# olivesgatech/R3D

Hardware: AMD Instinct MI355X
Metric: training clips/sec (RGB+Depth fusion, DARai) at 1/2/4/8 GPUs; effective-rank match (higher is better)
Workload: dtype f32 (depth products: bf16x3 split on the bf16 matrix cores, fp32 accumulate)

## Files before the change

r3d_amd/csrc/decoder_chain.hip:

```cpp
#include "chain_bf3.h"
#include "mha_small.h"
#include "losses_dev.h"

namespace r3d {

constexpr int kDcBufA = 0;
constexpr int kDcBufB = kDcBufA + kFcRows * kFcP1;
constexpr int kDcBufF = kDcBufB + kFcRows * kFcP1;
constexpr int kDcWl = kDcBufF + kFcRows * kFcP4;
constexpr int kDcWlWave = 128 * kFbWP;
constexpr int kDcRed = kDcWl + 8 * kDcWlWave;
constexpr int kDcLdsFloats = kDcRed + 2 * 2 * 8 * kFcRows;
constexpr int kDcLdsBytes = kDcLdsFloats * 4;
static_assert(16 * kFcWP <= kDcWlWave && mha_small_lds_floats(16, 8) <= kDcWlWave && mha_small_bwd_lds_floats(16, 8) <= kDcWlWave,
              "wave region");
static_assert(kDcLdsBytes + (2 * 8 * (kTLHeads + 8) + 8 * 4 * 128 + 64) * 4 <= 160 * 1024, "LDS (dynamic + the tail's static arrays)");

typedef r3d_decoder_chain_args DcArgs;

__device__ __forceinline__ void dc_stage_rows(float* buf, const float* src, int row0, int tid) {
    const int r = tid >> 5, c4 = tid & 31;
    const f32x4 z = {0.f, 0.f, 0.f, 0.f};
    const f32x4 v = *reinterpret_cast<const f32x4*>(src + (size_t)(row0 + (r & 7)) * kFcH + 4 * c4);
    *reinterpret_cast<f32x4*>(buf + r * kFcP1 + 4 * c4) = r < 8 ? v : z;
}

__device__ __forceinline__ void dc_fwd(const DcArgs& D, const int b, float* lds) {
    const int tid = threadIdx.x, lane = tid & 63, wave = tid >> 6;
    const int li = lane & 15, q = lane >> 4;
    float* bufA = lds + kDcBufA;
    float* bufB = lds + kDcBufB;
    float* bufF = lds + kDcBufF;
    float* wl = lds + kDcWl + wave * kDcWlWave;
    float (*red)[8][kFcRows] = reinterpret_cast<float (*)[8][kFcRows]>(lds + kDcRed);
    constexpr int H = kFcH;
    const int row0 = b * 8;
    const int c = wave * 16 + li;
    const bool live = q < 2;
    const f32x4 zero = {0.f, 0.f, 0.f, 0.f};
    R3D_CHAIN_MARK(D.timeline, b == 0, 0);
    FcW s0, s1;
    fc_wload(s0, D.wo + (size_t)(wave * 16) * H, H, 16, lane);
    fc_wload(s1, D.w1 + (size_t)((4 * wave + 0) * 16) * H, H, 16, lane);
    const FcMaskSrc md2(D.drop_d2, D.g2, H), md3(D.drop_d3, D.g2, H), mff(D.drop_ff, D.g2, 4 * H);
    float t1v[4];
    uint8_t kb2[4], kb3[4], kbf[4][4];
#pragma unroll
    for (int i = 0; i < 4; ++i) {
        const size_t r = (size_t)(row0 + ((4 * q + i) & 7));
        t1v[i] = D.t1[r * H + c];
        kb2[i] = md2.raw(r, c);
        kb3[i] = md3.raw(r, c);
#pragma unroll
        for (int t = 0; t < 4; ++t) kbf[t][i] = mff.raw(r, (4 * wave + t) * 16 + li);
    }
    const float b_o = D.bo[c], g2 = D.g2[c], be2 = D.be2[c], b_2 = D.b2[c];
    float b_1[4];
#pragma unroll
    for (int t = 0; t < 4; ++t) b_1[t] = D.b1[(4 * wave + t) * 16 + li];
    R3D_CHAIN_MARK(D.timeline, b == 0, 1);
    {
        MhaArgs m{};
        m.q = D.caq; m.ldq = H; m.k = D.cakv; m.ldk = 2 * H; m.v = D.cakv + H; m.ldv = 2 * H;
        m.key_label = D.key_label; m.pad_idx = D.pad_idx; m.probs = D.p_ca; m.drop = D.drop_ca; m.drop_scale = D.drop_scale;
        m.o = D.ca_o; m.ldo = H; m.B = D.B; m.heads = 8; m.Lq = 8; m.Lk = D.S; m.dh = 16; m.scale = 0.25f;
        mha_fwd_small_unit<16, 8, false>(m, b * 8 + wave, wl);
    }
    R3D_CHAIN_MARK(D.timeline, b == 0, 2);
    __syncthreads();
    dc_stage_rows(bufA, D.ca_o, row0, tid);
    fc_wstore(s0, wl, lane);
    fc_wload(s0, D.w1 + (size_t)((4 * wave + 1) * 16) * H, H, 16, lane);
    __syncthreads();
    const float* wr = wl + li * kFcWP + 4 * q;
    FcOp a;
    f32x4 acc0 = zero, acc1 = zero;
    R3D_CHAIN_MARK(D.timeline, b == 0, 3);
    fc_opload(a, bufA + li * kFcP1 + 4 * q);
    fc_chunk(a, wr, acc0, acc1);
    __builtin_amdgcn_sched_barrier(0);
    fc_wstore(s1, wl, lane);
    fc_wload(s1, D.w1 + (size_t)((4 * wave + 2) * 16) * H, H, 16, lane);
    __builtin_amdgcn_sched_barrier(0);
    float t2p[4], mean[4], rstd[4], t2v[4];
#pragma unroll
    for (int i = 0; i < 4; ++i) {
        t2p[i] = ((acc0[i] + acc1[i]) + b_o) * md2.keep(kb2[i], D.drop_scale) + t1v[i];
        if (live) D.t2_pre[(size_t)(row0 + 4 * q + i) * H + c] = t2p[i];
    }
    fc_layernorm(t2p, red, wave, li, q, mean, rstd);
#pragma unroll
    for (int i = 0; i < 4; ++i) {
        t2v[i] = (t2p[i] - mean[i]) * rstd[i] * g2 + be2;
        const int r = 4 * q + i;
        if (live) {
            D.t2[(size_t)(row0 + r) * H + c] = t2v[i];
            if (wave == 0 && li == 0) { D.m2[row0 + r] = mean[i]; D.r2[row0 + r] = rstd[i]; }
        }
        bufB[r * kFcP1 + c] = live ? t2v[i] : 0.f;
    }
    __syncthreads();
    R3D_CHAIN_MARK(D.timeline, b == 0, 4);
    fc_opload(a, bufB + li * kFcP1 + 4 * q);
#pragma unroll
    for (int t = 0; t < 4; ++t) {
        acc0 = zero; acc1 = zero;
        fc_chunk(a, wr, acc0, acc1);
        __builtin_amdgcn_sched_barrier(0);
        if (t == 0) { fc_wstore(s0, wl, lane); fc_wload(s0, D.w1 + (size_t)((4 * wave + 3) * 16) * H, H, 16, lane); }
        if (t == 1) { fc_wstore(s1, wl, lane); fc_wload(s1, D.w2 + (size_t)(wave * 16) * (4 * H) + 0, 4 * H, 16, lane); }
        if (t == 2) { fc_wstore(s0, wl, lane); fc_wload(s0, D.w2 + (size_t)(wave * 16) * (4 * H) + 128, 4 * H, 16, lane); }
        if (t == 3) { fc_wstore(s1, wl, lane); fc_wload(s1, D.w2 + (size_t)(wave * 16) * (4 * H) + 256, 4 * H, 16, lane); }
        __builtin_amdgcn_sched_barrier(0);
        const int cu = (4 * wave + t) * 16 + li;
#pragma unroll
        for (int i = 0; i < 4; ++i) {
            const float f = fmaxf((acc0[i] + acc1[i]) + b_1[t], 0.f) * mff.keep(kbf[t][i], D.drop_scale);
            if (live) D.ff1[(size_t)(row0 + 4 * q + i) * (4 * H) + cu] = f;
            bufF[(4 * q + i) * kFcP4 + cu] = live ? f : 0.f;
        }
    }
    __syncthreads();
    R3D_CHAIN_MARK(D.timeline, b == 0, 5);
    acc0 = zero; acc1 = zero;
    const float* ar = bufF + li * kFcP4 + 4 * q;
    fc_opload(a, ar);
    fc_chunk(a, wr, acc0, acc1);
    __builtin_amdgcn_sched_barrier(0);
    fc_wstore(s0, wl, lane);
    fc_wload(s0, D.w2 + (size_t)(wave * 16) * (4 * H) + 384, 4 * H, 16, lane);
    __builtin_amdgcn_sched_barrier(0);
    fc_opload(a, ar + 128);
    fc_chunk(a, wr, acc0, acc1);
    __builtin_amdgcn_sched_barrier(0);
    fc_wstore(s1, wl, lane);
    __builtin_amdgcn_sched_barrier(0);
    fc_opload(a, ar + 256);
    fc_chunk(a, wr, acc0, acc1);
    __builtin_amdgcn_sched_barrier(0);
    fc_wstore(s0, wl, lane);
    __builtin_amdgcn_sched_barrier(0);
    fc_opload(a, ar + 384);
    fc_chunk(a, wr, acc0, acc1);
    if (live) {
#pragma unroll
        for (int i = 0; i < 4; ++i)
            D.t3_pre[(size_t)(row0 + 4 * q + i) * H + c] = ((acc0[i] + acc1[i]) + b_2) * md3.keep(kb3[i], D.drop_scale) + t2v[i];
    }
}

__device__ __forceinline__ void dc_bwd(const DcArgs& D, const int b, float* lds) {
    const int tid = threadIdx.x, lane = tid & 63, wave = tid >> 6;
    const int li = lane & 15, q = lane >> 4;
    float* bufA = lds + kDcBufA;
    float* bufF = lds + kDcBufF;
    float* wl = lds + kDcWl + wave * kDcWlWave;
    float* redA = lds + kDcRed;
    constexpr int H = kFcH;
    const int row0 = b * 8;
    const int c = wave * 16 + li, n0 = wave * 16;
    const bool live = q < 2;
    const f32x4 zero = {0.f, 0.f, 0.f, 0.f};
    R3D_CHAIN_MARK(D.timeline, b == 0, 10);
    FcW s0, s1;
    fb_wload(s0, D.w2 + (4 * wave + 0) * 16, 4 * H, 128, lane);
    fb_wload(s1, D.w2 + (4 * wave + 1) * 16, 4 * H, 128, lane);
    dc_stage_rows(bufA, D.d_ff2, row0, tid);
    const FcMaskSrc md2(D.drop_d2, D.g2, H), mff(D.drop_ff, D.g2, 4 * H);
    float ffv[4][4], res[4], t2pv[4], m2v[4], r2v[4];
    uint8_t kb2[4], kbf[4][4];
#pragma unroll
    for (int i = 0; i < 4; ++i) {
        const size_t r = (size_t)(row0 + ((4 * q + i) & 7));
#pragma unroll
        for (int t = 0; t < 4; ++t) {
            ffv[t][i] = D.ff1[r * (4 * H) + (4 * wave + t) * 16 + li];
            kbf[t][i] = mff.raw(r, (4 * wave + t) * 16 + li);
        }
        res[i] = D.d_t3pre[r * H + c];
        t2pv[i] = D.t2_pre[r * H + c];
        m2v[i] = D.m2[r]; r2v[i] = D.r2[r];
        kb2[i] = md2.raw(r, c);
    }
    const float g2 = D.g2[c];
    __builtin_amdgcn_sched_barrier(0);
    fb_wstore(s0, wl, lane);
    fb_wload(s0, D.w2 + (4 * wave + 2) * 16, 4 * H, 128, lane);
    __syncthreads();
    FcOp a;
    f32x4 acc0, acc1;
    R3D_CHAIN_MARK(D.timeline, b == 0, 11);
    fc_opload(a, bufA + li * kFcP1 + 4 * q);
#pragma unroll
    for (int t = 0; t < 4; ++t) {
        acc0 = zero; acc1 = zero;
        fb_chunk(a, wl, li, q, acc0, acc1);
        __builtin_amdgcn_sched_barrier(0);
        if (t == 0) { fb_wstore(s1, wl, lane); fb_wload(s1, D.w2 + (4 * wave + 3) * 16, 4 * H, 128, lane); }
        if (t == 1) { fb_wstore(s0, wl, lane); fb_wload(s0, D.w1 + n0, H, 128, lane); }
        if (t == 2) { fb_wstore(s1, wl, lane); fb_wload(s1, D.w1 + (size_t)128 * H + n0, H, 128, lane); }
        if (t == 3) { fb_wstore(s0, wl, lane); fb_wload(s0, D.w1 + (size_t)256 * H + n0, H, 128, lane); }
        __builtin_amdgcn_sched_barrier(0);
        const int cu = (4 * wave + t) * 16 + li;
#pragma unroll
        for (int i = 0; i < 4; ++i) {
            const float gv = ffv[t][i] > 0.f ? (acc0[i] + acc1[i]) * mff.keep(kbf[t][i], D.drop_scale) : 0.f;
            if (live) D.d_ff1[(size_t)(row0 + 4 * q + i) * (4 * H) + cu] = gv;
            bufF[(4 * q + i) * kFcP4 + cu] = live ? gv : 0.f;
        }
    }
    __syncthreads();
    R3D_CHAIN_MARK(D.timeline, b == 0, 12);
    acc0 = zero; acc1 = zero;
    const float* ar = bufF + li * kFcP4 + 4 * q;
    fc_opload(a, ar);
    fb_chunk(a, wl, li, q, acc0, acc1);
    __builtin_amdgcn_sched_barrier(0);
    fb_wstore(s1, wl, lane);
    fb_wload(s1, D.w1 + (size_t)384 * H + n0, H, 128, lane);
    __builtin_amdgcn_sched_barrier(0);
    fc_opload(a, ar + 128);
    fb_chunk(a, wl, li, q, acc0, acc1);
    __builtin_amdgcn_sched_barrier(0);
    fb_wstore(s0, wl, lane);
    fb_wload(s0, D.wo + n0, H, 128, lane);
    __builtin_amdgcn_sched_barrier(0);
    fc_opload(a, ar + 256);
    fb_chunk(a, wl, li, q, acc0, acc1);
    __builtin_amdgcn_sched_barrier(0);
    fb_wstore(s1, wl, lane);
    __builtin_amdgcn_sched_barrier(0);
    fc_opload(a, ar + 384);
    fb_chunk(a, wl, li, q, acc0, acc1);
    __builtin_amdgcn_sched_barrier(0);
    fb_wstore(s0, wl, lane);
    __builtin_amdgcn_sched_barrier(0);
    {
        float d[4], xh[4], g[4], gx[4], s1v[4], s2v[4];
#pragma unroll
        for (int i = 0; i < 4; ++i) {
            d[i] = live ? (acc0[i] + acc1[i]) + res[i] : 0.f;
            xh[i] = (t2pv[i] - m2v[i]) * r2v[i];
            g[i] = d[i] * g2;
            gx[i] = g[i] * xh[i];
        }
        if (live) {
            float* pp = D.part_d2 + (size_t)(2 * b + q) * (2 * H);
            pp[c] = (d[0] * xh[0] + d[1] * xh[1]) + (d[2] * xh[2] + d[3] * xh[3]);
            pp[H + c] = (d[0] + d[1]) + (d[2] + d[3]);
        }
        fb_rowsum2<4>(g, gx, redA, wave, li, q, s1v, s2v);
#pragma unroll
        for (int i = 0; i < 4; ++i) {
            const float o = r2v[i] * (g[i] - s1v[i] - xh[i] * s2v[i]);
            const size_t e = (size_t)(row0 + 4 * q + i) * H + c;
            const float ok = o * md2.keep(kb2[i], D.drop_scale);
            if (live) { D.d_t2pre[e] = o; D.d_cap[e] = ok; }
            bufA[(4 * q + i) * kFcP1 + c] = live ? ok : 0.f;
        }
    }
    __syncthreads();
    R3D_CHAIN_MARK(D.timeline, b == 0, 13);
    fc_opload(a, bufA + li * kFcP1 + 4 * q);
    acc0 = zero; acc1 = zero;
    fb_chunk(a, wl, li, q, acc0, acc1);
    if (live) {
#pragma unroll
        for (int i = 0; i < 4; ++i) D.d_cao[(size_t)(row0 + 4 * q + i) * H + c] = acc0[i] + acc1[i];
    }
    R3D_CHAIN_MARK(D.timeline, b == 0, 14);
    __syncthreads();
    {
        MhaArgs m{};
        m.q = D.caq; m.ldq = H; m.k = D.cakv; m.ldk = 2 * H; m.v = D.cakv + H; m.ldv = 2 * H;
        m.probs = D.p_ca; m.drop = D.drop_ca; m.drop_scale = D.drop_scale; m.d_o = D.d_cao; m.lddo = H;
        m.dq = D.d_caq; m.lddq = H; m.dk = D.d_cakv; m.lddk = 2 * H; m.dv = D.d_cakv + H; m.lddv = 2 * H;
        m.B = D.B; m.heads = 8; m.Lq = 8; m.Lk = D.S; m.dh = 16; m.scale = 0.25f;
        mha_bwd_small_unit<16, 8, false>(m, b * 8 + wave, wl);
    }
    R3D_CHAIN_MARK(D.timeline, b == 0, 15);
}

constexpr int kD3P1 = kFcH + 8, kD3P4 = 4 * kFcH + 8;
constexpr int kD3ImgA = 0;
constexpr int kD3ImgB = kD3ImgA + 3 * 16 * kD3P1;
constexpr int kD3ImgF = kD3ImgB + 3 * 16 * kD3P1;
constexpr int kD3ScrBytes = (kD3ImgF + 3 * 16 * kD3P4) * 2;
constexpr int kD3ScrWave = 1856;
constexpr int kD3RedBytes = kD3ScrBytes + 8 * kD3ScrWave * 4;
constexpr int kD3LdsBytes = kD3RedBytes + 2 * 2 * 8 * kFcRows * 4;
static_assert(mha_small_lds_floats(16, 8) <= kD3ScrWave && mha_small_bwd_lds_floats(16, 8) <= kD3ScrWave, "attention scratch");
static_assert(kD3LdsBytes + (2 * 8 * (kTLHeads + 8) + 8 * 4 * 128 + 64) * 4 <= 160 * 1024, "LDS (dynamic + the tail's static arrays)");

__device__ __forceinline__ void dc3_stage_rows(unsigned short* img, const float* src, int row0, int tid) {
    const int r = tid >> 5, c4 = tid & 31;
    const f32x4 z = {0.f, 0.f, 0.f, 0.f};
    const f32x4 v = *reinterpret_cast<const f32x4*>(src + (size_t)(row0 + (r & 7)) * kFcH + 4 * c4);
    bf3_store4(img, kD3P1, r, 4 * c4, r < 8 ? v : z);
}

__device__ __forceinline__ void dc3_fwd(const DcArgs& D, const int b, float* lds) {
    const int tid = threadIdx.x, lane = tid & 63, wave = tid >> 6;
    const int li = lane & 15, q = lane >> 4;
    unsigned short* img = reinterpret_cast<unsigned short*>(lds);
    unsigned short* imgA = img + kD3ImgA;
    unsigned short* imgB = img + kD3ImgB;
    unsigned short* imgF = img + kD3ImgF;
    float* scr = reinterpret_cast<float*>(reinterpret_cast<unsigned char*>(lds) + kD3ScrBytes) + wave * kD3ScrWave;
    float (*red)[8][kFcRows] = reinterpret_cast<float (*)[8][kFcRows]>(reinterpret_cast<unsigned char*>(lds) + kD3RedBytes);
    constexpr int H = kFcH;
    const int row0 = b * 8;
    const int c = wave * 16 + li;
    const bool live = q < 2;
    const f32x4 zero = {0.f, 0.f, 0.f, 0.f};
    R3D_CHAIN_MARK(D.timeline, b == 0, 0);
    Bf3B b0, b1, b2;
    bf3_bload<4>(b0, D.pl_wo, 4, wave, 0, lane);
    bf3_bload<4>(b1, D.pl_w1, 4, 4 * wave + 0, 0, lane);
    bf3_bload<4>(b2, D.pl_w1, 4, 4 * wave + 1, 0, lane);
    const FcMaskSrc md2(D.drop_d2, D.g2, H), md3(D.drop_d3, D.g2, H), mff(D.drop_ff, D.g2, 4 * H);
    float t1v[4];
    uint8_t kb2[4], kb3[4], kbf[4][4];
#pragma unroll
    for (int i = 0; i < 4; ++i) {
        const size_t r = (size_t)(row0 + ((4 * q + i) & 7));
        t1v[i] = D.t1[r * H + c];
        kb2[i] = md2.raw(r, c);
        kb3[i] = md3.raw(r, c);
#pragma unroll
        for (int t = 0; t < 4; ++t) kbf[t][i] = mff.raw(r, (4 * wave + t) * 16 + li);
    }
    const float b_o = D.bo[c], g2 = D.g2[c], be2 = D.be2[c], b_2 = D.b2[c];
    float b_1[4];
#pragma unroll
    for (int t = 0; t < 4; ++t) b_1[t] = D.b1[(4 * wave + t) * 16 + li];
    R3D_CHAIN_MARK(D.timeline, b == 0, 1);
    {
        MhaArgs m{};
        m.q = D.caq; m.ldq = H; m.k = D.cakv; m.ldk = 2 * H; m.v = D.cakv + H; m.ldv = 2 * H;
        m.key_label = D.key_label; m.pad_idx = D.pad_idx; m.probs = D.p_ca; m.drop = D.drop_ca; m.drop_scale = D.drop_scale;
        m.o = D.ca_o; m.ldo = H; m.B = D.B; m.heads = 8; m.Lq = 8; m.Lk = D.S; m.dh = 16; m.scale = 0.25f;
        mha_fwd_small_unit<16, 8, false>(m, b * 8 + wave, scr);
    }
    R3D_CHAIN_MARK(D.timeline, b == 0, 2);
    __syncthreads();
    dc3_stage_rows(imgA, D.ca_o, row0, tid);
    __syncthreads();
    R3D_CHAIN_MARK(D.timeline, b == 0, 3);
    f32x4 acc0 = zero, acc1 = zero;
    bf3_chunk<4>(imgA, kD3P1, li, q, 0, b0, acc0, acc1);
    __builtin_amdgcn_sched_barrier(0);
    bf3_bload<4>(b0, D.pl_w1, 4, 4 * wave + 2, 0, lane);
    __builtin_amdgcn_sched_barrier(0);
    float t2p[4], mean[4], rstd[4], t2v[4];
#pragma unroll
    for (int i = 0; i < 4; ++i) {
        t2p[i] = ((acc0[i] + acc1[i]) + b_o) * md2.keep(kb2[i], D.drop_scale) + t1v[i];
        if (live) D.t2_pre[(size_t)(row0 + 4 * q + i) * H + c] = t2p[i];
    }
    fc_layernorm(t2p, red, wave, li, q, mean, rstd);
#pragma unroll
    for (int i = 0; i < 4; ++i) {
        t2v[i] = (t2p[i] - mean[i]) * rstd[i] * g2 + be2;
        const int r = 4 * q + i;
        if (live) {
            D.t2[(size_t)(row0 + r) * H + c] = t2v[i];
            if (wave == 0 && li == 0) { D.m2[row0 + r] = mean[i]; D.r2[row0 + r] = rstd[i]; }
        }
        bf3_store1(imgB, kD3P1, r, c, live ? t2v[i] : 0.f);
    }
    __syncthreads();
    R3D_CHAIN_MARK(D.timeline, b == 0, 4);
#pragma unroll
    for (int t = 0; t < 4; ++t) {
        acc0 = zero; acc1 = zero;
        if (t == 0) bf3_chunk<4>(imgB, kD3P1, li, q, 0, b1, acc0, acc1);
        if (t == 1) bf3_chunk<4>(imgB, kD3P1, li, q, 0, b2, acc0, acc1);
        if (t == 2) bf3_chunk<4>(imgB, kD3P1, li, q, 0, b0, acc0, acc1);
        if (t == 3) bf3_chunk<4>(imgB, kD3P1, li, q, 0, b1, acc0, acc1);
        __builtin_amdgcn_sched_barrier(0);
        if (t == 0) bf3_bload<4>(b1, D.pl_w1, 4, 4 * wave + 3, 0, lane);
        if (t == 1) bf3_bload<4>(b2, D.pl_w2, 16, wave, 0, lane);
        if (t == 2) bf3_bload<4>(b0, D.pl_w2, 16, wave, 4, lane);
        if (t == 3) bf3_bload<4>(b1, D.pl_w2, 16, wave, 8, lane);
        __builtin_amdgcn_sched_barrier(0);
        const int cu = (4 * wave + t) * 16 + li;
#pragma unroll
        for (int i = 0; i < 4; ++i) {
            const float f = fmaxf((acc0[i] + acc1[i]) + b_1[t], 0.f) * mff.keep(kbf[t][i], D.drop_scale);
            if (live) D.ff1[(size_t)(row0 + 4 * q + i) * (4 * H) + cu] = f;
            bf3_store1(imgF, kD3P4, 4 * q + i, cu, live ? f : 0.f);
        }
    }
    __syncthreads();
    R3D_CHAIN_MARK(D.timeline, b == 0, 5);
    acc0 = zero; acc1 = zero;
    bf3_chunk<4>(imgF, kD3P4, li, q, 0, b2, acc0, acc1);
    __builtin_amdgcn_sched_barrier(0);
    bf3_bload<4>(b2, D.pl_w2, 16, wave, 12, lane);
    __builtin_amdgcn_sched_barrier(0);
    bf3_chunk<4>(imgF, kD3P4, li, q, 4, b0, acc0, acc1);
    bf3_chunk<4>(imgF, kD3P4, li, q, 8, b1, acc0, acc1);
    bf3_chunk<4>(imgF, kD3P4, li, q, 12, b2, acc0, acc1);
    if (live) {
#pragma unroll
        for (int i = 0; i < 4; ++i)
            D.t3_pre[(size_t)(row0 + 4 * q + i) * H + c] =
                ((acc0[i] + acc1[i]) + b_2) * md3.keep(kb3[i], D.drop_scale) + t2v[i];
    }
}

__device__ __forceinline__ void dc3_bwd(const DcArgs& D, const int b, float* lds) {
    const int tid = threadIdx.x, lane = tid & 63, wave = tid >> 6;
    const int li = lane & 15, q = lane >> 4;
    unsigned short* img = reinterpret_cast<unsigned short*>(lds);
    unsigned short* imgA = img + kD3ImgA;
    unsigned short* imgF = img + kD3ImgF;
    float* scr = reinterpret_cast<float*>(reinterpret_cast<unsigned char*>(lds) + kD3ScrBytes) + wave * kD3ScrWave;
    float* redA = reinterpret_cast<float*>(reinterpret_cast<unsigned char*>(lds) + kD3RedBytes);
    constexpr int H = kFcH;
    const int row0 = b * 8;
    const int c = wave * 16 + li;
    const bool live = q < 2;
    const f32x4 zero = {0.f, 0.f, 0.f, 0.f};
    R3D_CHAIN_MARK(D.timeline, b == 0, 10);
    Bf3B b0, b1, b2;
    bf3_bload<4>(b0, D.pl_w2_t, 4, 4 * wave + 0, 0, lane);
    bf3_bload<4>(b1, D.pl_w2_t, 4, 4 * wave + 1, 0, lane);
    bf3_bload<4>(b2, D.pl_w2_t, 4, 4 * wave + 2, 0, lane);
    dc3_stage_rows(imgA, D.d_ff2, row0, tid);
    const FcMaskSrc md2(D.drop_d2, D.g2, H), mff(D.drop_ff, D.g2, 4 * H);
    float ffv[4][4], res[4], t2pv[4], m2v[4], r2v[4];
    uint8_t kb2[4], kbf[4][4];
#pragma unroll
    for (int i = 0; i < 4; ++i) {
        const size_t r = (size_t)(row0 + ((4 * q + i) & 7));
#pragma unroll
        for (int t = 0; t < 4; ++t) {
            ffv[t][i] = D.ff1[r * (4 * H) + (4 * wave + t) * 16 + li];
            kbf[t][i] = mff.raw(r, (4 * wave + t) * 16 + li);
        }
        res[i] = D.d_t3pre[r * H + c];
        t2pv[i] = D.t2_pre[r * H + c];
        m2v[i] = D.m2[r]; r2v[i] = D.r2[r];
        kb2[i] = md2.raw(r, c);
    }
    const float g2 = D.g2[c];
    __syncthreads();
    R3D_CHAIN_MARK(D.timeline, b == 0, 11);
    f32x4 acc0, acc1;
#pragma unroll
    for (int t = 0; t < 4; ++t) {
        acc0 = zero; acc1 = zero;
        if (t == 0) bf3_chunk<4>(imgA, kD3P1, li, q, 0, b0, acc0, acc1);
        if (t == 1) bf3_chunk<4>(imgA, kD3P1, li, q, 0, b1, acc0, acc1);
        if (t == 2) bf3_chunk<4>(imgA, kD3P1, li, q, 0, b2, acc0, acc1);
        if (t == 3) bf3_chunk<4>(imgA, kD3P1, li, q, 0, b0, acc0, acc1);
        __builtin_amdgcn_sched_barrier(0);
        if (t == 0) bf3_bload<4>(b0, D.pl_w2_t, 4, 4 * wave + 3, 0, lane);
        if (t == 1) bf3_bload<4>(b1, D.pl_w1_t, 16, wave, 0, lane);
        if (t == 2) bf3_bload<4>(b2, D.pl_w1_t, 16, wave, 4, lane);
        if (t == 3) bf3_bload<4>(b0, D.pl_w1_t, 16, wave, 8, lane);
        __builtin_amdgcn_sched_barrier(0);
        const int cu = (4 * wave + t) * 16 + li;
#pragma unroll
        for (int i = 0; i < 4; ++i) {
            const float gv = ffv[t][i] > 0.f ? (acc0[i] + acc1[i]) * mff.keep(kbf[t][i], D.drop_scale) : 0.f;
            if (live) D.d_ff1[(size_t)(row0 + 4 * q + i) * (4 * H) + cu] = gv;
            bf3_store1(imgF, kD3P4, 4 * q + i, cu, live ? gv : 0.f);
        }
    }
    __syncthreads();
    R3D_CHAIN_MARK(D.timeline, b == 0, 12);
    acc0 = zero; acc1 = zero;
    bf3_chunk<4>(imgF, kD3P4, li, q, 0, b1, acc0, acc1);
    __builtin_amdgcn_sched_barrier(0);
    bf3_bload<4>(b1, D.pl_w1_t, 16, wave, 12, lane);
    __builtin_amdgcn_sched_barrier(0);
    bf3_chunk<4>(imgF, kD3P4, li, q, 4, b2, acc0, acc1);
    __builtin_amdgcn_sched_barrier(0);
    bf3_bload<4>(b2, D.pl_wo_t, 4, wave, 0, lane);
    __builtin_amdgcn_sched_barrier(0);
    bf3_chunk<4>(imgF, kD3P4, li, q, 8, b0, acc0, acc1);
    bf3_chunk<4>(imgF, kD3P4, li, q, 12, b1, acc0, acc1);
    {
        float d[4], xh[4], g[4], gx[4], s1v[4], s2v[4];
#pragma unroll
        for (int i = 0; i < 4; ++i) {
            d[i] = live ? (acc0[i] + acc1[i]) + res[i] : 0.f;
            xh[i] = (t2pv[i] - m2v[i]) * r2v[i];
            g[i] = d[i] * g2;
            gx[i] = g[i] * xh[i];
        }
        if (live) {
            float* pp = D.part_d2 + (size_t)(2 * b + q) * (2 * H);
            pp[c] = (d[0] * xh[0] + d[1] * xh[1]) + (d[2] * xh[2] + d[3] * xh[3]);
            pp[H + c] = (d[0] + d[1]) + (d[2] + d[3]);
        }
        fb_rowsum2<4>(g, gx, redA, wave, li, q, s1v, s2v);
#pragma unroll
        for (int i = 0; i < 4; ++i) {
            const float o = r2v[i] * (g[i] - s1v[i] - xh[i] * s2v[i]);
            const size_t e = (size_t)(row0 + 4 * q + i) * H + c;
            const float ok = o * md2.keep(kb2[i], D.drop_scale);
            if (live) { D.d_t2pre[e] = o; D.d_cap[e] = ok; }
            bf3_store1(imgA, kD3P1, 4 * q + i, c, live ? ok : 0.f);
        }
    }
    __syncthreads();
    R3D_CHAIN_MARK(D.timeline, b == 0, 13);
    acc0 = zero; acc1 = zero;
    bf3_chunk<4>(imgA, kD3P1, li, q, 0, b2, acc0, acc1);
    if (live) {
#pragma unroll
        for (int i = 0; i < 4; ++i) D.d_cao[(size_t)(row0 + 4 * q + i) * H + c] = acc0[i] + acc1[i];
    }
    R3D_CHAIN_MARK(D.timeline, b == 0, 14);
    __syncthreads();
    {
        MhaArgs m{};
        m.q = D.caq; m.ldq = H; m.k = D.cakv; m.ldk = 2 * H; m.v = D.cakv + H; m.ldv = 2 * H;
        m.probs = D.p_ca; m.drop = D.drop_ca; m.drop_scale = D.drop_scale; m.d_o = D.d_cao; m.lddo = H;
        m.dq = D.d_caq; m.lddq = H; m.dk = D.d_cakv; m.lddk = 2 * H; m.dv = D.d_cakv + H; m.lddv = 2 * H;
        m.B = D.B; m.heads = 8; m.Lq = 8; m.Lk = D.S; m.dh = 16; m.scale = 0.25f;
        mha_bwd_small_unit<16, 8, false>(m, b * 8 + wave, scr);
    }
    R3D_CHAIN_MARK(D.timeline, b == 0, 15);
}

__global__ __launch_bounds__(512) void decoder_chain_bf3_kernel(const DcArgs D, const r3d_tail_losses_args t, const LossArgs a,
                                                                float* part, unsigned* arrivals) {
    extern __shared__ __attribute__((aligned(16))) float lds[];
    __shared__ float lg[8][kTLHeads + 8];
    __shared__ float dl[8][kTLHeads + 8];
    __shared__ float red[8][4][128];
    __shared__ int is_last;
    if (threadIdx.x >= 256) __builtin_amdgcn_s_setprio(0); else __builtin_amdgcn_s_setprio(2);
    const int lane = threadIdx.x & 63, wave = threadIdx.x >> 6;
    if ((int)blockIdx.x < D.B) {
        const int b = (int)blockIdx.x;
        if (D.phases & 1) dc3_fwd(D, b, lds);
        R3D_CHAIN_MARK(D.timeline, b == 0, 6);
        if (D.phases & 2) {
            __syncthreads();
            tail_clip_body(t, a, part, b, lg, dl, red);
        }
        R3D_CHAIN_MARK(D.timeline, b == 0, 7);
        if (D.phases & 4) {
            __syncthreads();
            dc3_bwd(D, b, lds);
        }
    } else if (D.phases & 2) {
        const int u = ((int)blockIdx.x - D.B) * 8 + wave;
        if (u < a.B * a.S) losses_unit(a, part, u, lane);
    }
    if (D.phases & 2) tail_losses_finish(t, a, part, arrivals, &is_last);
}

__global__ __launch_bounds__(512) void decoder_chain_kernel(const DcArgs D, const r3d_tail_losses_args t, const LossArgs a,
                                                            float* part, unsigned* arrivals) {
    extern __shared__ __attribute__((aligned(16))) float lds[];
    if (threadIdx.x >= 256) __builtin_amdgcn_s_setprio(0); else __builtin_amdgcn_s_setprio(2);
    __shared__ float lg[8][kTLHeads + 8];
    __shared__ float dl[8][kTLHeads + 8];
    __shared__ float red[8][4][128];
    __shared__ int is_last;
    const int lane = threadIdx.x & 63, wave = threadIdx.x >> 6;
    if ((int)blockIdx.x < D.B) {
        const int b = (int)blockIdx.x;
        if (D.phases & 1) dc_fwd(D, b, lds);
        R3D_CHAIN_MARK(D.timeline, b == 0, 6);
        if (D.phases & 2) {
            __syncthreads();
            tail_clip_body(t, a, part, b, lg, dl, red);
        }
        R3D_CHAIN_MARK(D.timeline, b == 0, 7);
        if (D.phases & 4) {
            __syncthreads();
            dc_bwd(D, b, lds);
        }
    } else if (D.phases & 2) {
        const int u = ((int)blockIdx.x - D.B) * 8 + wave;
        if (u < a.B * a.S) losses_unit(a, part, u, lane);
    }
    if (D.phases & 2) tail_losses_finish(t, a, part, arrivals, &is_last);
}

}

using namespace r3d;

R3D_EXPORT int r3d_decoder_tail_losses_supported(int H, int n_head, int Q, int rows);

R3D_EXPORT int r3d_decoder_chain_supported(int H, int Q, int heads, int S) {
    return (H == kFcH && Q == 8 && heads == 8 && S > 0 && S <= 64) ? 1 : 0;
}

R3D_EXPORT int r3d_decoder_chain(const r3d_decoder_chain_args* d, const r3d_tail_losses_args* tail, float* ws, void* stream) {
    R3D_REQUIRE(d && (d->phases & 7) && !(d->phases & ~7));
    R3D_REQUIRE(r3d_decoder_chain_supported(d->H, d->Q, d->heads, d->S) && d->B > 0);
    R3D_REQUIRE(d->caq && d->cakv && d->p_ca && d->wo && d->w1 && d->w2 && d->t2_pre && d->m2 && d->r2 && d->g2 && d->ff1);
    if (d->phases & 1)
        R3D_REQUIRE(d->ca_o && d->bo && d->t1 && d->be2 && d->t2 && d->b1 && d->b2 && d->t3_pre);
    if (d->phases & 4)
        R3D_REQUIRE(d->d_t3pre && d->d_ff2 && d->d_ff1 && d->d_t2pre && d->d_cap && d->d_cao && d->d_caq && d->d_cakv && d->part_d2);
    const void* al[] = {d->caq, d->cakv, d->wo, d->w1, d->w2, d->ca_o, d->d_ff2, d->d_cao, d->d_cakv};
    for (const void* p : al)
        if (p && !r3d_aligned16(p)) return R3D_EALIGN;
    r3d_tail_losses_args t{};
    LossArgs a{};
    int grid = d->B;
    unsigned* arrivals = nullptr;
    if (d->phases & 2) {
        R3D_REQUIRE(tail && ws);
        t = *tail;
        R3D_REQUIRE(t.x && t.g3 && t.b3 && t.gF && t.bF && t.w_head && t.b_head && t.t3 && t.m3 && t.r3 && t.tgtF && t.mF && t.rF);
        R3D_REQUIRE(t.out && t.seg && t.past_label && t.target && t.target_dur && t.d_seg && t.d_out && t.loss_out && t.counts);
        R3D_REQUIRE(t.dx && t.dx2 && t.wsF && t.ws3);
        R3D_REQUIRE(t.B == d->B && t.S == d->S && t.Q == d->Q && t.H == d->H && t.K > 0 && t.n_head == t.K + 1);
        R3D_REQUIRE(t.ld_out >= t.n_head && t.ld_dout >= t.n_head && t.ld_seg >= t.K && t.ld_dseg >= t.K);
        if (!r3d_decoder_tail_losses_supported(t.H, t.n_head, t.Q, t.B * t.Q)) return R3D_EINVAL;
        if (!r3d_aligned16(ws)) return R3D_EALIGN;
        if (d->phases & 1) R3D_REQUIRE(t.x == d->t3_pre);
        if (d->phases & 4) R3D_REQUIRE(t.dx == d->d_t3pre && t.dx2 == d->d_ff2);
        a = LossArgs{t.seg, t.ld_seg, t.out, t.ld_out, t.out + t.K, t.ld_out, t.past_label, t.target, t.target_dur, t.B, t.S, t.Q,
                     t.K, t.pad_idx, t.exclude_idx, 0, t.dur_den, t.grad_scale, t.d_seg, t.ld_dseg, t.d_out, t.ld_dout,
                     t.d_out + t.K, t.ld_dout, t.loss_out, t.counts, t.tick_a, t.tick_b};
        const int units = t.B * t.S + t.B * t.Q + t.B;
        grid = t.B + r3d_cdiv(t.B * t.S, 8);
        arrivals = reinterpret_cast<unsigned*>(ws + 4 * (size_t)units);
    }
    if (d->pl_wo) {
        R3D_REQUIRE(d->pl_w1 && d->pl_w2 && d->pl_w2_t && d->pl_w1_t && d->pl_wo_t);
        hipError_t e3 = hipFuncSetAttribute((const void*)decoder_chain_bf3_kernel, hipFuncAttributeMaxDynamicSharedMemorySize,
                                            kD3LdsBytes);
        if (e3 != hipSuccess) return (int)e3;
        hipLaunchKernelGGL(decoder_chain_bf3_kernel, dim3(grid), dim3(512), (size_t)kD3LdsBytes, (hipStream_t)stream, *d, t, a, ws,
                           arrivals);
        R3D_LAUNCH_CHECK();
        return R3D_OK;
    }
    hipError_t e = hipFuncSetAttribute((const void*)decoder_chain_kernel, hipFuncAttributeMaxDynamicSharedMemorySize, kDcLdsBytes);
    if (e != hipSuccess) return (int)e;
    hipLaunchKernelGGL(decoder_chain_kernel, dim3(grid), dim3(512), (size_t)kDcLdsBytes, (hipStream_t)stream, *d, t, a, ws, arrivals);
    R3D_LAUNCH_CHECK();
    return R3D_OK;
}
```

r3d_amd/csrc/fuser_chain.hip:

```cpp
#include "chain_bf3.h"
#include "mha_small.h"
#include "../../include/r3d_hip.h"

namespace r3d {

constexpr int kFcBufH = 0;
constexpr int kFcBufV = kFcBufH + kFcRows * kFcP1;
constexpr int kFcBufF = kFcBufV + kFcRows * kFcP1;
constexpr int kFcWl = kFcBufF + kFcRows * kFcP4;
constexpr int kFcRed = kFcWl + 8 * 16 * kFcWP;
constexpr int kFcLdsFloats = kFcRed + 2 * 8 * kFcRows;
constexpr int kFcLdsBytes = kFcLdsFloats * 4;
static_assert(mha_small_lds_floats(16, 8) <= 16 * kFcWP, "the query role's attention units borrow the wave's weight region");
static_assert(mha_small_bwd_lds_floats(16, 8) <= 16 * kFcWP, "the query role's attention units borrow the wave's weight region");

typedef r3d_fuser_chain_fwd_args FcFwd;

__device__ __forceinline__ void fc_fwd_fuser(const FcFwd& A, const int wg, float* lds) {
    const int tid = threadIdx.x, lane = tid & 63, wave = tid >> 6;
    const int li = lane & 15, q = lane >> 4;
    float* bufH = lds + kFcBufH;
    float* bufV = lds + kFcBufV;
    float* bufF = lds + kFcBufF;
    float* wl = lds + kFcWl + wave * (16 * kFcWP);
    float (*red)[8][kFcRows] = reinterpret_cast<float (*)[8][kFcRows]>(lds + kFcRed);
    const int row0 = wg * kFcRows;
    const int c = wave * 16 + li;
    constexpr int H = kFcH;
    const int nseg_t = (A.K + 15) >> 4;
    R3D_CHAIN_MARK(A.timeline, wg == 0, 0);
    const int nt5 = 16 + nseg_t;

    FcW s0, s1;
    fc_wload(s0, A.wv + (size_t)(wave * 16) * H, H, 16, lane);
    fc_wload(s1, A.wproj + (size_t)(wave * 16) * H, H, 16, lane);
    const f32x4 a_in = *reinterpret_cast<const f32x4*>(A.h1 + (size_t)(row0 + (tid >> 5)) * H + 4 * (tid & 31));
    float x0[4];
#pragma unroll
    for (int i = 0; i < 4; ++i) x0[i] = A.x0[(size_t)(row0 + 4 * q + i) * H + c];
    const float b_proj = A.bproj[c], g2 = A.g2[c], be2 = A.be2[c], b_2 = A.b2[c], gF = A.gf[c], beF = A.bef[c];
    float b_1[4];
#pragma unroll
    for (int t = 0; t < 4; ++t) b_1[t] = A.b1[(4 * wave + t) * 16 + li];
    const int f0 = (row0 >> 1) + 2 * q;
    const float pos0 = A.pos[(size_t)(f0 % A.S) * H + c], pos1 = A.pos[(size_t)((f0 + 1) % A.S) * H + c];
    __builtin_amdgcn_sched_barrier(0);
    *reinterpret_cast<f32x4*>(bufH + (tid >> 5) * kFcP1 + 4 * (tid & 31)) = a_in;
    fc_wstore(s0, wl, lane);
    fc_wload(s0, A.w1 + (size_t)((4 * wave + 0) * 16) * H, H, 16, lane);
    __syncthreads();

    R3D_CHAIN_MARK(A.timeline, wg == 0, 1);
    const float* wr = wl + li * kFcWP + 4 * q;
    FcOp a;
    f32x4 acc0, acc1;
    const f32x4 zero = {0.f, 0.f, 0.f, 0.f};
    fc_opload(a, bufH + li * kFcP1 + 4 * q);
    acc0 = zero; acc1 = zero;
    fc_chunk(a, wr, acc0, acc1);
    __builtin_amdgcn_sched_barrier(0);
    fc_wstore(s1, wl, lane);
    fc_wload(s1, A.w1 + (size_t)((4 * wave + 1) * 16) * H, H, 16, lane);
    __builtin_amdgcn_sched_barrier(0);
#pragma unroll
    for (int i = 0; i < 4; ++i) {
        const float v = acc0[i] + acc1[i];
        const int rs = 4 * q + (i ^ 1);
        A.vsw[(size_t)(row0 + rs) * H + c] = v;
        bufV[rs * kFcP1 + c] = v;
    }
    __syncthreads();
    R3D_CHAIN_MARK(A.timeline, wg == 0, 2);
    fc_opload(a, bufV + li * kFcP1 + 4 * q);
    acc0 = zero; acc1 = zero;
    fc_chunk(a, wr, acc0, acc1);
    __builtin_amdgcn_sched_barrier(0);
    fc_wstore(s0, wl, lane);
    fc_wload(s0, A.w1 + (size_t)((4 * wave + 2) * 16) * H, H, 16, lane);
    __builtin_amdgcn_sched_barrier(0);
    float x1[4], mean[4], rstd[4];
#pragma unroll
    for (int i = 0; i < 4; ++i) {
        x1[i] = (acc0[i] + acc1[i]) + b_proj + x0[i];
        A.x1[(size_t)(row0 + 4 * q + i) * H + c] = x1[i];
    }
    fc_layernorm(x1, red, wave, li, q, mean, rstd);
#pragma unroll
    for (int i = 0; i < 4; ++i) {
        const float h = (x1[i] - mean[i]) * rstd[i] * g2 + be2;
        const int r = 4 * q + i;
        A.h2[(size_t)(row0 + r) * H + c] = h;
        bufH[r * kFcP1 + c] = h;
        if (wave == 0 && li == 0) { A.m2[row0 + r] = mean[i]; A.r2[row0 + r] = rstd[i]; }
    }
    __syncthreads();
    R3D_CHAIN_MARK(A.timeline, wg == 0, 3);
    fc_opload(a, bufH + li * kFcP1 + 4 * q);
#pragma unroll
    for (int t = 0; t < 4; ++t) {
        acc0 = zero; acc1 = zero;
        if (t < 2) R3D_CHAIN_MARK(A.timeline, wg == 0, 8 + 4 * t);
        fc_chunk(a, wr, acc0, acc1);
        __builtin_amdgcn_sched_barrier(0);
        if (t < 2) R3D_CHAIN_MARK(A.timeline, wg == 0, 9 + 4 * t);
#if defined(R3D_FC_PROBE) && (R3D_FC_PROBE & 8)
        if (t == 0) { fc_wstore(s1, wl, lane); }
        if (t == 1) { fc_wstore(s0, wl, lane); }
        if (t == 2) { fc_wstore(s1, wl, lane); }
        if (t == 3) { fc_wstore(s0, wl, lane); }
#elif defined(R3D_FC_PROBE) && (R3D_FC_PROBE & 16)
        if (t == 0) { fc_wload(s1, A.w1 + (size_t)((4 * wave + 3) * 16) * H, H, 16, lane); }
        if (t == 1) { fc_wload(s0, A.w2 + (size_t)(wave * 16) * (4 * H) + 0, 4 * H, 16, lane); }
        if (t == 2) { fc_wload(s1, A.w2 + (size_t)(wave * 16) * (4 * H) + 128, 4 * H, 16, lane); }
        if (t == 3) { fc_wload(s0, A.w2 + (size_t)(wave * 16) * (4 * H) + 256, 4 * H, 16, lane); }
#else
        if (t == 0) { fc_wstore(s1, wl, lane); fc_wload(s1, A.w1 + (size_t)((4 * wave + 3) * 16) * H, H, 16, lane); }
        if (t == 1) { fc_wstore(s0, wl, lane); fc_wload(s0, A.w2 + (size_t)(wave * 16) * (4 * H) + 0, 4 * H, 16, lane); }
        if (t == 2) { fc_wstore(s1, wl, lane); fc_wload(s1, A.w2 + (size_t)(wave * 16) * (4 * H) + 128, 4 * H, 16, lane); }
        if (t == 3) { fc_wstore(s0, wl, lane); fc_wload(s0, A.w2 + (size_t)(wave * 16) * (4 * H) + 256, 4 * H, 16, lane); }
#endif
        __builtin_amdgcn_sched_barrier(0);
        if (t < 2) R3D_CHAIN_MARK(A.timeline, wg == 0, 10 + 4 * t);
        const int cu = (4 * wave + t) * 16 + li;
#pragma unroll
        for (int i = 0; i < 4; ++i) {
            const float u = (acc0[i] + acc1[i]) + b_1[t];
#if defined(R3D_FC_PROBE) && (R3D_FC_PROBE & 4)
            const float f = u;
#else
            const float f = gelu_f(u);
#endif
            const size_t o = (size_t)(row0 + 4 * q + i) * (4 * H) + cu;
#if !(defined(R3D_FC_PROBE) && (R3D_FC_PROBE & 1))
            A.u[o] = u;
            A.f1[o] = f;
#endif
#if !(defined(R3D_FC_PROBE) && (R3D_FC_PROBE & 2))
            bufF[(4 * q + i) * kFcP4 + cu] = f;
#else
            if (u == 123.456f) bufF[(4 * q + i) * kFcP4 + cu] = f;
#endif
        }
        if (t < 2) R3D_CHAIN_MARK(A.timeline, wg == 0, 11 + 4 * t);
    }
    __syncthreads();
    R3D_CHAIN_MARK(A.timeline, wg == 0, 4);
    acc0 = zero; acc1 = zero;
    {
        const float* ar = bufF + li * kFcP4 + 4 * q;
        fc_opload(a, ar);
        fc_chunk(a, wr, acc0, acc1);
        __builtin_amdgcn_sched_barrier(0);
        fc_wstore(s1, wl, lane);
        fc_wload(s1, A.w2 + (size_t)(wave * 16) * (4 * H) + 384, 4 * H, 16, lane);
        __builtin_amdgcn_sched_barrier(0);
        fc_opload(a, ar + 128);
        fc_chunk(a, wr, acc0, acc1);
        __builtin_amdgcn_sched_barrier(0);
        fc_wstore(s0, wl, lane);
        {
            const int t5 = wave;
            fc_wload(s0, A.wkv + (size_t)(t5 * 16) * H, H, 16, lane);
        }
        __builtin_amdgcn_sched_barrier(0);
        fc_opload(a, ar + 256);
        fc_chunk(a, wr, acc0, acc1);
        __builtin_amdgcn_sched_barrier(0);
        fc_wstore(s1, wl, lane);
        {
            const int t5 = wave + 8;
            fc_wload(s1, A.wkv + (size_t)(t5 * 16) * H, H, 16, lane);
        }
        __builtin_amdgcn_sched_barrier(0);
        fc_opload(a, ar + 384);
        fc_chunk(a, wr, acc0, acc1);
        __builtin_amdgcn_sched_barrier(0);
    }
    fc_wstore(s0, wl, lane);
    const int t5c = wave + 16;
    const bool has12 = t5c < nt5;
    {
        const int ts = has12 ? t5c - 16 : 0;
        const int nv = A.K - 16 * ts;
        fc_wload(s0, A.wseg + (size_t)(ts * 16) * H, H, nv < 16 ? nv : 16, lane);
    }
    const float bkv0 = A.bkv[wave * 16 + li], bkv1 = A.bkv[(wave + 8) * 16 + li];
    const int cseg = (has12 ? t5c - 16 : 0) * 16 + li;
    const float bsg = A.bseg[cseg < A.K ? cseg : A.K - 1];
    __builtin_amdgcn_sched_barrier(0);
    R3D_CHAIN_MARK(A.timeline, wg == 0, 5);
    float x3[4];
#pragma unroll
    for (int i = 0; i < 4; ++i) {
        x3[i] = (acc0[i] + acc1[i]) + b_2 + x1[i] + (A.add_xres ? x0[i] : 0.f);
        A.x3[(size_t)(row0 + 4 * q + i) * H + c] = x3[i];
    }
    fc_layernorm(x3, red, wave, li, q, mean, rstd);
    float y[4];
#pragma unroll
    for (int i = 0; i < 4; ++i) {
        y[i] = (x3[i] - mean[i]) * rstd[i] * gF + beF;
        if (A.y) A.y[(size_t)(row0 + 4 * q + i) * H + c] = y[i];
        if (wave == 0 && li == 0) { A.mf[row0 + 4 * q + i] = mean[i]; A.rf[row0 + 4 * q + i] = rstd[i]; }
    }
    {
        const float fu0 = (y[0] + y[1]) * 0.5f, fu1 = (y[2] + y[3]) * 0.5f;
        A.fused[(size_t)f0 * H + c] = fu0;
        A.fused[(size_t)(f0 + 1) * H + c] = fu1;
        bufV[(2 * q) * kFcP1 + c] = fu0;
        bufV[(2 * q + 1) * kFcP1 + c] = fu1;
        bufV[(8 + 2 * q) * kFcP1 + c] = fu0 + pos0;
        bufV[(8 + 2 * q + 1) * kFcP1 + c] = fu1 + pos1;
    }
    __syncthreads();
    R3D_CHAIN_MARK(A.timeline, wg == 0, 6);
    fc_opload(a, bufV + li * kFcP1 + 4 * q);
    const int fr = (row0 >> 1) + ((4 * q) & 7);
    acc0 = zero; acc1 = zero;
    fc_chunk(a, wr, acc0, acc1);
    __builtin_amdgcn_sched_barrier(0);
    fc_wstore(s1, wl, lane);
    __builtin_amdgcn_sched_barrier(0);
    if (q >= 2) {
#pragma unroll
        for (int i = 0; i < 4; ++i) A.cakv[(size_t)(fr + i) * (2 * H) + wave * 16 + li] = (acc0[i] + acc1[i]) + bkv0;
    }
    acc0 = zero; acc1 = zero;
    fc_chunk(a, wr, acc0, acc1);
    __builtin_amdgcn_sched_barrier(0);
    fc_wstore(s0, wl, lane);
    __builtin_amdgcn_sched_barrier(0);
    if (q >= 2) {
#pragma unroll
        for (int i = 0; i < 4; ++i) A.cakv[(size_t)(fr + i) * (2 * H) + (wave + 8) * 16 + li] = (acc0[i] + acc1[i]) + bkv1;
    }
    if (has12) {
        acc0 = zero; acc1 = zero;
        fc_chunk(a, wr, acc0, acc1);
        if (q < 2 && cseg < A.K) {
#pragma unroll
            for (int i = 0; i < 4; ++i) A.seg[(size_t)(fr + i) * A.K + cseg] = (acc0[i] + acc1[i]) + bsg;
        }
    }
    R3D_CHAIN_MARK(A.timeline, wg == 0, 7);
}

__device__ __forceinline__ void fc_fwd_query(const FcFwd& A, const int wgq, float* lds) {
    const int tid = threadIdx.x, lane = tid & 63, wave = tid >> 6;
    const int li = lane & 15, q = lane >> 4;
    float* bufH = lds + kFcBufH;
    float* bufV = lds + kFcBufV;
    float* wl = lds + kFcWl + wave * (16 * kFcWP);
    float (*red)[8][kFcRows] = reinterpret_cast<float (*)[8][kFcRows]>(lds + kFcRed);
    constexpr int H = kFcH;
    const int row0 = wgq * kFcRows;
    const int c = wave * 16 + li;
    R3D_CHAIN_MARK(A.timeline, wgq == 0, 16);
    FcW s0, s1;
    fc_wload(s0, A.w_in + (size_t)(wave * 16) * H, H, 16, lane);
    fc_wload(s1, A.w_in + (size_t)((wave + 8) * 16) * H, H, 16, lane);
    const f32x4 a_in = *reinterpret_cast<const f32x4*>(A.qpos + (size_t)((tid >> 5) & 7) * H + 4 * (tid & 31));
    float b_in[3];
#pragma unroll
    for (int t = 0; t < 3; ++t) b_in[t] = A.b_in[(wave + 8 * t) * 16 + li];
    const float b_out = A.b_out[c], g1 = A.g1[c], be1 = A.be1[c], b_q = A.bq[c];
    const FcMaskSrc md1(A.drop_d1, A.g1, H);
    uint8_t kb[4];
    float qp[4];
#pragma unroll
    for (int i = 0; i < 4; ++i) {
        const int r = row0 + 4 * q + i;
        kb[i] = md1.raw(r, c);
        qp[i] = A.qpos[(size_t)((4 * q + i) & 7) * H + c];
    }
    __builtin_amdgcn_sched_barrier(0);
    *reinterpret_cast<f32x4*>(bufH + (tid >> 5) * kFcP1 + 4 * (tid & 31)) = a_in;
    fc_wstore(s0, wl, lane);
    fc_wload(s0, A.w_in + (size_t)((wave + 16) * 16) * H, H, 16, lane);
    __syncthreads();
    const float* wr = wl + li * kFcWP + 4 * q;
    FcOp a;
    f32x4 acc0, acc1;
    const f32x4 zero = {0.f, 0.f, 0.f, 0.f};
    fc_opload(a, bufH + li * kFcP1 + 4 * q);
#pragma unroll
    for (int t = 0; t < 3; ++t) {
        acc0 = zero; acc1 = zero;
        fc_chunk(a, wr, acc0, acc1);
        __builtin_amdgcn_sched_barrier(0);
        if (t == 0) { fc_wstore(s1, wl, lane); fc_wload(s1, A.w_out + (size_t)(wave * 16) * H, H, 16, lane); }
        if (t == 1) { fc_wstore(s0, wl, lane); fc_wload(s0, A.wq + (size_t)(wave * 16) * H, H, 16, lane); }
        __builtin_amdgcn_sched_barrier(0);
#pragma unroll
        for (int i = 0; i < 4; ++i)
            A.sa_qkv[(size_t)(row0 + 4 * q + i) * (3 * H) + (wave + 8 * t) * 16 + li] = (acc0[i] + acc1[i]) + b_in[t];
    }
    R3D_CHAIN_MARK(A.timeline, wgq == 0, 17);
    __syncthreads();
    {
        MhaArgs m{};
        m.q = A.sa_qkv; m.ldq = 3 * H; m.k = A.sa_qkv + H; m.ldk = 3 * H; m.v = A.sa_qkv + 2 * H; m.ldv = 3 * H;
        m.probs = A.p_sa; m.drop = A.drop_sa; m.drop_scale = A.drop_scale; m.o = A.sa_o; m.ldo = H;
        m.B = A.B; m.heads = 8; m.Lq = 8; m.Lk = 8; m.dh = 16; m.scale = 0.25f;
        mha_fwd_small_unit<16, 8, false>(m, (2 * wgq) * 8 + wave, wl);
        __builtin_amdgcn_wave_barrier();
        mha_fwd_small_unit<16, 8, false>(m, (2 * wgq + 1) * 8 + wave, wl);
    }
    __syncthreads();
    {
        const f32x4 so = *reinterpret_cast<const f32x4*>(A.sa_o + (size_t)(row0 + (tid >> 5)) * H + 4 * (tid & 31));
        *reinterpret_cast<f32x4*>(bufV + (tid >> 5) * kFcP1 + 4 * (tid & 31)) = so;
    }
    R3D_CHAIN_MARK(A.timeline, wgq == 0, 18);
    fc_wstore(s1, wl, lane);
    __syncthreads();
    R3D_CHAIN_MARK(A.timeline, wgq == 0, 19);
    fc_opload(a, bufV + li * kFcP1 + 4 * q);
    acc0 = zero; acc1 = zero;
    fc_chunk(a, wr, acc0, acc1);
    __builtin_amdgcn_sched_barrier(0);
    fc_wstore(s0, wl, lane);
    __builtin_amdgcn_sched_barrier(0);
    float t1p[4], mean[4], rstd[4];
#pragma unroll
    for (int i = 0; i < 4; ++i) {
        t1p[i] = ((acc0[i] + acc1[i]) + b_out) * md1.keep(kb[i], A.drop_scale);
        A.t1_pre[(size_t)(row0 + 4 * q + i) * H + c] = t1p[i];
    }
    fc_layernorm(t1p, red, wave, li, q, mean, rstd);
#pragma unroll
    for (int i = 0; i < 4; ++i) {
        const int r = 4 * q + i;
        const float t1 = (t1p[i] - mean[i]) * rstd[i] * g1 + be1;
        A.t1[(size_t)(row0 + r) * H + c] = t1;
        bufH[r * kFcP1 + c] = t1 + qp[i];
        if (wave == 0 && li == 0) { A.m1[row0 + r] = mean[i]; A.r1[row0 + r] = rstd[i]; }
    }
    __syncthreads();
    R3D_CHAIN_MARK(A.timeline, wgq == 0, 20);
    fc_opload(a, bufH + li * kFcP1 + 4 * q);
    acc0 = zero; acc1 = zero;
    fc_chunk(a, wr, acc0, acc1);
#pragma unroll
    for (int i = 0; i < 4; ++i) A.caq[(size_t)(row0 + 4 * q + i) * H + c] = (acc0[i] + acc1[i]) + b_q;
    R3D_CHAIN_MARK(A.timeline, wgq == 0, 21);
}

constexpr int kF3P1 = kFcH + 8;
constexpr int kF3P4 = 4 * kFcH + 8;
constexpr int kF3ImgH = 0;
constexpr int kF3ImgV = kF3ImgH + 3 * 16 * kF3P1;
constexpr int kF3ImgF = kF3ImgV + 3 * 16 * kF3P1;
constexpr int kF3RedBytes = (kF3ImgF + 3 * 16 * kF3P4) * 2;
constexpr int kF3LdsBytes = kF3RedBytes + 2 * 2 * 8 * kFcRows * 4;

__device__ __forceinline__ void fc3_fwd_fuser(const FcFwd& A, const int wg, float* lds) {
    const int tid = threadIdx.x, lane = tid & 63, wave = tid >> 6;
    const int li = lane & 15, q = lane >> 4;
    unsigned short* img = reinterpret_cast<unsigned short*>(lds);
    unsigned short* imgH = img + kF3ImgH;
    unsigned short* imgV = img + kF3ImgV;
    unsigned short* imgF = img + kF3ImgF;
    float (*red)[8][kFcRows] = reinterpret_cast<float (*)[8][kFcRows]>(reinterpret_cast<unsigned char*>(lds) + kF3RedBytes);
    const int row0 = wg * kFcRows;
    const int c = wave * 16 + li;
    constexpr int H = kFcH;
    const int nseg_t = (A.K + 15) >> 4;
    const bool has12 = wave < nseg_t;
    R3D_CHAIN_MARK(A.timeline, wg == 0, 0);
    Bf3B b0, b1, b2;
    bf3_bload<4>(b0, A.pl_wv, 4, wave, 0, lane);
    bf3_bload<4>(b1, A.pl_wproj, 4, wave, 0, lane);
    bf3_bload<4>(b2, A.pl_w1, 4, 4 * wave + 0, 0, lane);
    const f32x4 a_in = *reinterpret_cast<const f32x4*>(A.h1 + (size_t)(row0 + (tid >> 5)) * H + 4 * (tid & 31));
    float x0[4];
#pragma unroll
    for (int i = 0; i < 4; ++i) x0[i] = A.x0[(size_t)(row0 + 4 * q + i) * H + c];
    const float b_proj = A.bproj[c], g2 = A.g2[c], be2 = A.be2[c], b_2 = A.b2[c], gF = A.gf[c], beF = A.bef[c];
    float b_1[4];
#pragma unroll
    for (int t = 0; t < 4; ++t) b_1[t] = A.b1[(4 * wave + t) * 16 + li];
    const int f0 = (row0 >> 1) + 2 * q;
    const float pos0 = A.pos[(size_t)(f0 % A.S) * H + c], pos1 = A.pos[(size_t)((f0 + 1) % A.S) * H + c];
    const float bkv0 = A.bkv[wave * 16 + li], bkv1 = A.bkv[(wave + 8) * 16 + li];
    const int cseg = (has12 ? wave : 0) * 16 + li;
    const float bsg = A.bseg[cseg < A.K ? cseg : A.K - 1];
    __builtin_amdgcn_sched_barrier(0);
    bf3_stage_tile(imgH, kF3P1, 0, a_in, tid);
    __syncthreads();
    R3D_CHAIN_MARK(A.timeline, wg == 0, 1);
    const f32x4 zero = {0.f, 0.f, 0.f, 0.f};
    f32x4 acc0 = zero, acc1 = zero;
    bf3_chunk<4>(imgH, kF3P1, li, q, 0, b0, acc0, acc1);
    __builtin_amdgcn_sched_barrier(0);
    bf3_bload<4>(b0, A.pl_w1, 4, 4 * wave + 1, 0, lane);
    __builtin_amdgcn_sched_barrier(0);
#pragma unroll
    for (int i = 0; i < 4; ++i) {
        const float v = acc0[i] + acc1[i];
        const int rs = 4 * q + (i ^ 1);
        A.vsw[(size_t)(row0 + rs) * H + c] = v;
        bf3_store1(imgV, kF3P1, rs, c, v);
    }
    __syncthreads();
    R3D_CHAIN_MARK(A.timeline, wg == 0, 2);
    acc0 = zero; acc1 = zero;
    bf3_chunk<4>(imgV, kF3P1, li, q, 0, b1, acc0, acc1);
    __builtin_amdgcn_sched_barrier(0);
    bf3_bload<4>(b1, A.pl_w1, 4, 4 * wave + 2, 0, lane);
    __builtin_amdgcn_sched_barrier(0);
    float x1[4], mean[4], rstd[4];
#pragma unroll
    for (int i = 0; i < 4; ++i) {
        x1[i] = (acc0[i] + acc1[i]) + b_proj + x0[i];
        A.x1[(size_t)(row0 + 4 * q + i) * H + c] = x1[i];
    }
    fc_layernorm(x1, red, wave, li, q, mean, rstd);
#pragma unroll
    for (int i = 0; i < 4; ++i) {
        const float h = (x1[i] - mean[i]) * rstd[i] * g2 + be2;
        const int r = 4 * q + i;
        A.h2[(size_t)(row0 + r) * H + c] = h;
        bf3_store1(imgH, kF3P1, r, c, h);
        if (wave == 0 && li == 0) { A.m2[row0 + r] = mean[i]; A.r2[row0 + r] = rstd[i]; }
    }
    __syncthreads();
    R3D_CHAIN_MARK(A.timeline, wg == 0, 3);
#pragma unroll
    for (int t = 0; t < 4; ++t) {
        acc0 = zero; acc1 = zero;
        if (t == 0) bf3_chunk<4>(imgH, kF3P1, li, q, 0, b2, acc0, acc1);
        if (t == 1) bf3_chunk<4>(imgH, kF3P1, li, q, 0, b0, acc0, acc1);
        if (t == 2) bf3_chunk<4>(imgH, kF3P1, li, q, 0, b1, acc0, acc1);
        if (t == 3) bf3_chunk<4>(imgH, kF3P1, li, q, 0, b2, acc0, acc1);
        __builtin_amdgcn_sched_barrier(0);
        if (t == 0) bf3_bload<4>(b2, A.pl_w1, 4, 4 * wave + 3, 0, lane);
        if (t == 1) bf3_bload<4>(b0, A.pl_w2, 16, wave, 0, lane);
        if (t == 2) bf3_bload<4>(b1, A.pl_w2, 16, wave, 4, lane);
        if (t == 3) bf3_bload<4>(b2, A.pl_w2, 16, wave, 8, lane);
        __builtin_amdgcn_sched_barrier(0);
        const int cu = (4 * wave + t) * 16 + li;
#pragma unroll
        for (int i = 0; i < 4; ++i) {
            const float u = (acc0[i] + acc1[i]) + b_1[t];
            const float f = gelu_f(u);
            const size_t o = (size_t)(row0 + 4 * q + i) * (4 * H) + cu;
            A.u[o] = u;
            A.f1[o] = f;
            bf3_store1(imgF, kF3P4, 4 * q + i, cu, f);
        }
    }
    __syncthreads();
    R3D_CHAIN_MARK(A.timeline, wg == 0, 4);
    acc0 = zero; acc1 = zero;
    bf3_chunk<4>(imgF, kF3P4, li, q, 0, b0, acc0, acc1);
    __builtin_amdgcn_sched_barrier(0);
    bf3_bload<4>(b0, A.pl_w2, 16, wave, 12, lane);
    __builtin_amdgcn_sched_barrier(0);
    bf3_chunk<4>(imgF, kF3P4, li, q, 4, b1, acc0, acc1);
    __builtin_amdgcn_sched_barrier(0);
    bf3_bload<4>(b1, A.pl_wkv, 4, wave, 0, lane);
    __builtin_amdgcn_sched_barrier(0);
    bf3_chunk<4>(imgF, kF3P4, li, q, 8, b2, acc0, acc1);
    __builtin_amdgcn_sched_barrier(0);
    bf3_bload<4>(b2, A.pl_wkv, 4, wave + 8, 0, lane);
    __builtin_amdgcn_sched_barrier(0);
    bf3_chunk<4>(imgF, kF3P4, li, q, 12, b0, acc0, acc1);
    __builtin_amdgcn_sched_barrier(0);
    bf3_bload<4>(b0, A.pl_wseg, 4, has12 ? wave : 0, 0, lane);
    __builtin_amdgcn_sched_barrier(0);
    R3D_CHAIN_MARK(A.timeline, wg == 0, 5);
    float x3[4];
#pragma unroll
    for (int i = 0; i < 4; ++i) {
        x3[i] = (acc0[i] + acc1[i]) + b_2 + x1[i] + (A.add_xres ? x0[i] : 0.f);
        A.x3[(size_t)(row0 + 4 * q + i) * H + c] = x3[i];
    }
    fc_layernorm(x3, red, wave, li, q, mean, rstd);
    float y[4];
#pragma unroll
    for (int i = 0; i < 4; ++i) {
        y[i] = (x3[i] - mean[i]) * rstd[i] * gF + beF;
        if (A.y) A.y[(size_t)(row0 + 4 * q + i) * H + c] = y[i];
        if (wave == 0 && li == 0) { A.mf[row0 + 4 * q + i] = mean[i]; A.rf[row0 + 4 * q + i] = rstd[i]; }
    }
    {
        const float fu0 = (y[0] + y[1]) * 0.5f, fu1 = (y[2] + y[3]) * 0.5f;
        A.fused[(size_t)f0 * H + c] = fu0;
        A.fused[(size_t)(f0 + 1) * H + c] = fu1;
        bf3_store1(imgV, kF3P1, 2 * q, c, fu0);
        bf3_store1(imgV, kF3P1, 2 * q + 1, c, fu1);
        bf3_store1(imgV, kF3P1, 8 + 2 * q, c, fu0 + pos0);
        bf3_store1(imgV, kF3P1, 8 + 2 * q + 1, c, fu1 + pos1);
    }
    __syncthreads();
    R3D_CHAIN_MARK(A.timeline, wg == 0, 6);
    const int fr = (row0 >> 1) + ((4 * q) & 7);
    acc0 = zero; acc1 = zero;
    bf3_chunk<4>(imgV, kF3P1, li, q, 0, b1, acc0, acc1);
    if (q >= 2) {
#pragma unroll
        for (int i = 0; i < 4; ++i) A.cakv[(size_t)(fr + i) * (2 * H) + wave * 16 + li] = (acc0[i] + acc1[i]) + bkv0;
    }
    acc0 = zero; acc1 = zero;
    bf3_chunk<4>(imgV, kF3P1, li, q, 0, b2, acc0, acc1);
    if (q >= 2) {
#pragma unroll
        for (int i = 0; i < 4; ++i) A.cakv[(size_t)(fr + i) * (2 * H) + (wave + 8) * 16 + li] = (acc0[i] + acc1[i]) + bkv1;
    }
    if (has12) {
        acc0 = zero; acc1 = zero;
        bf3_chunk<4>(imgV, kF3P1, li, q, 0, b0, acc0, acc1);
        if (q < 2 && cseg < A.K) {
#pragma unroll
            for (int i = 0; i < 4; ++i) A.seg[(size_t)(fr + i) * A.K + cseg] = (acc0[i] + acc1[i]) + bsg;
        }
    }
    R3D_CHAIN_MARK(A.timeline, wg == 0, 7);
}

__global__ __launch_bounds__(512) void fuser_chain_fwd_bf3_kernel(const FcFwd A) {
    extern __shared__ __attribute__((aligned(16))) float lds[];
    if (threadIdx.x >= 256) __builtin_amdgcn_s_setprio(0); else __builtin_amdgcn_s_setprio(2);
    const int nf = (2 * A.N) / kFcRows;
    if ((int)blockIdx.x < nf) fc3_fwd_fuser(A, (int)blockIdx.x, lds);
    else fc_fwd_query(A, (int)blockIdx.x - nf, lds);
}

__global__ __launch_bounds__(256) void weight_planes_kernel(const r3d_plane_job* __restrict__ jobs, int njobs, int total) {
    weight_planes_block(jobs, njobs, total, (int)blockIdx.x * 4 + (threadIdx.x >> 6), threadIdx.x & 63);
}

__global__ __launch_bounds__(512) void fuser_chain_fwd_kernel(const FcFwd A) {
    extern __shared__ __attribute__((aligned(16))) float lds[];
    if (threadIdx.x >= 256) __builtin_amdgcn_s_setprio(0); else __builtin_amdgcn_s_setprio(2);
    const int nf = (2 * A.N) / kFcRows;
    if ((int)blockIdx.x < nf) fc_fwd_fuser(A, (int)blockIdx.x, lds);
    else fc_fwd_query(A, (int)blockIdx.x - nf, lds);
}


constexpr int kFbWl = kFcBufF + kFcRows * kFcP4;
constexpr int kFbRed = kFbWl + 8 * 128 * kFbWP;
constexpr int kFbLdsFloats = kFbRed + 2 * 2 * 8 * kFcRows;
constexpr int kFbLdsBytes = kFbLdsFloats * 4;
static_assert(mha_small_bwd_lds_floats(16, 8) <= 128 * kFbWP, "attention units borrow the wave's weight region");
static_assert(kFbLdsBytes <= 160 * 1024, "LDS");

typedef r3d_fuser_chain_bwd_args FcBwd;

__device__ __forceinline__ void fc_bwd_fuser(const FcBwd& A, const int wg, float* lds) {
    const int tid = threadIdx.x, lane = tid & 63, wave = tid >> 6;
    const int li = lane & 15, q = lane >> 4;
    float* bufH = lds + kFcBufH;
    float* bufV = lds + kFcBufV;
    float* bufF = lds + kFcBufF;
    float* wl = lds + kFbWl + wave * (128 * kFbWP);
    float* redA = lds + kFbRed;
    float* redB = redA + 2 * 8 * kFcRows;
    constexpr int H = kFcH;
    const int row0 = wg * kFcRows;
    const int c = wave * 16 + li;
    const int n0 = wave * 16;
    const int f0 = (row0 >> 1) + 2 * q;
    const f32x4 zero = {0.f, 0.f, 0.f, 0.f};

    R3D_CHAIN_MARK(A.timeline, wg == 0, 0);
    FcW s0, s1;
    fb_wload(s0, A.wkv + n0, H, 128, lane);
    fb_wload(s1, A.wkv + (size_t)128 * H + n0, H, 128, lane);
    {
        const int r = tid >> 5, c4 = tid & 31, fr = (row0 >> 1) + (r >> 1);
        const f32x4 v0 = *reinterpret_cast<const f32x4*>(A.d_cakv + (size_t)fr * (2 * H) + 4 * c4);
        const f32x4 v1 = *reinterpret_cast<const f32x4*>(A.d_cakv + (size_t)fr * (2 * H) + 128 + 4 * c4);
        f32x4 v2;
#pragma unroll
        for (int e = 0; e < 4; ++e) {
            const int k = 4 * c4 + e;
            const float t = A.d_seg[(size_t)fr * A.K + (k < A.K ? k : A.K - 1)];
            v2[e] = k < A.K ? t : 0.f;
        }
        float* dst = bufF + r * kFcP4 + 4 * c4;
        *reinterpret_cast<f32x4*>(dst) = v0;
        *reinterpret_cast<f32x4*>(dst + 128) = v1;
        *reinterpret_cast<f32x4*>(dst + 256) = v2;
    }
    float x3v[4], mfv[4], rfv[4], dex[2];
#pragma unroll
    for (int i = 0; i < 4; ++i) {
        const int r = row0 + 4 * q + i;
        x3v[i] = A.x3[(size_t)r * H + c]; mfv[i] = A.mf[r]; rfv[i] = A.rf[r];
    }
    const float gF = A.gf[c];
    {
        const float* ex = A.d_extra ? A.d_extra : A.gf;
        const int ld = A.d_extra ? H : 0;
        dex[0] = ex[(size_t)f0 * ld + c]; dex[1] = ex[(size_t)(f0 + 1) * ld + c];
        if (!A.d_extra) { dex[0] = 0.f; dex[1] = 0.f; }
    }
    __builtin_amdgcn_sched_barrier(0);
    fb_wstore(s0, wl, lane);
    fb_wload(s0, A.wseg + n0, H, A.K, lane);
    __syncthreads();
    FcOp a;
    f32x4 acc0 = zero, acc1 = zero;
    const float* ar = bufF + li * kFcP4 + 4 * q;
    R3D_CHAIN_MARK(A.timeline, wg == 0, 1);
    fc_opload(a, ar);
    fb_chunk(a, wl, li, q, acc0, acc1);
    __builtin_amdgcn_sched_barrier(0);
    fb_wstore(s1, wl, lane);
    fb_wload(s1, A.w2 + (4 * wave + 0) * 16, 4 * H, 128, lane);
    __builtin_amdgcn_sched_barrier(0);
    fc_opload(a, ar + 128);
    fb_chunk(a, wl, li, q, acc0, acc1);
    __builtin_amdgcn_sched_barrier(0);
    fb_wstore(s0, wl, lane);
    fb_wload(s0, A.w2 + (4 * wave + 1) * 16, 4 * H, 128, lane);
    __builtin_amdgcn_sched_barrier(0);
    A.d_fused[(size_t)f0 * H + c] = acc0[0] + acc1[0];
    A.d_fused[(size_t)(f0 + 1) * H + c] = acc0[2] + acc1[2];
    fc_opload(a, ar + 256);
    fb_chunk(a, wl, li, q, acc0, acc1);
    __builtin_amdgcn_sched_barrier(0);
    fb_wstore(s1, wl, lane);
    fb_wload(s1, A.w2 + (4 * wave + 2) * 16, 4 * H, 128, lane);
    __builtin_amdgcn_sched_barrier(0);
    R3D_CHAIN_MARK(A.timeline, wg == 0, 2);
    float dx3[4];
    {
        float d[4], xh[4], g[4], gx[4], s1v[4], s2v[4];
#pragma unroll
        for (int i = 0; i < 4; ++i) {
            d[i] = 0.5f * ((acc0[i] + acc1[i]) + dex[i >> 1]);
            xh[i] = (x3v[i] - mfv[i]) * rfv[i];
            g[i] = d[i] * gF;
            gx[i] = g[i] * xh[i];
        }
        float* pp = A.part_nf + (size_t)(wg * 4 + q) * (2 * H);
        pp[c] = (d[0] * xh[0] + d[1] * xh[1]) + (d[2] * xh[2] + d[3] * xh[3]);
        pp[H + c] = (d[0] + d[1]) + (d[2] + d[3]);
        fb_rowsum2<4>(g, gx, redA, wave, li, q, s1v, s2v);
#pragma unroll
        for (int i = 0; i < 4; ++i) {
            dx3[i] = rfv[i] * (g[i] - s1v[i] - xh[i] * s2v[i]);
            A.d_x3[(size_t)(row0 + 4 * q + i) * H + c] = dx3[i];
            bufH[(4 * q + i) * kFcP1 + c] = dx3[i];
        }
    }
    float uv[4][4];
#pragma unroll
    for (int t = 0; t < 4; ++t) {
#pragma unroll
        for (int i = 0; i < 4; ++i) uv[t][i] = A.u[(size_t)(row0 + 4 * q + i) * (4 * H) + (4 * wave + t) * 16 + li];
    }
    __syncthreads();
    R3D_CHAIN_MARK(A.timeline, wg == 0, 3);
    fc_opload(a, bufH + li * kFcP1 + 4 * q);
#pragma unroll
    for (int t = 0; t < 4; ++t) {
        acc0 = zero; acc1 = zero;
        fb_chunk(a, wl, li, q, acc0, acc1);
        __builtin_amdgcn_sched_barrier(0);
        if (t == 0) { fb_wstore(s0, wl, lane); fb_wload(s0, A.w2 + (4 * wave + 3) * 16, 4 * H, 128, lane); }
        if (t == 1) { fb_wstore(s1, wl, lane); fb_wload(s1, A.w1 + n0, H, 128, lane); }
        if (t == 2) { fb_wstore(s0, wl, lane); fb_wload(s0, A.w1 + (size_t)128 * H + n0, H, 128, lane); }
        if (t == 3) { fb_wstore(s1, wl, lane); fb_wload(s1, A.w1 + (size_t)256 * H + n0, H, 128, lane); }
        __builtin_amdgcn_sched_barrier(0);
        const int cu = (4 * wave + t) * 16 + li;
#pragma unroll
        for (int i = 0; i < 4; ++i) {
            const float du = (acc0[i] + acc1[i]) * gelu_grad_f(uv[t][i]);
            A.d_u[(size_t)(row0 + 4 * q + i) * (4 * H) + cu] = du;
            bufF[(4 * q + i) * kFcP4 + cu] = du;
        }
    }
    float x1v[4], m2v[4], r2v[4];
#pragma unroll
    for (int i = 0; i < 4; ++i) {
        const int r = row0 + 4 * q + i;
        x1v[i] = A.x1[(size_t)r * H + c]; m2v[i] = A.m2[r]; r2v[i] = A.r2[r];
    }
    const float g2 = A.g2[c];
    __syncthreads();
    R3D_CHAIN_MARK(A.timeline, wg == 0, 4);
    acc0 = zero; acc1 = zero;
    fc_opload(a, ar);
    fb_chunk(a, wl, li, q, acc0, acc1);
    __builtin_amdgcn_sched_barrier(0);
    fb_wstore(s0, wl, lane);
    fb_wload(s0, A.w1 + (size_t)384 * H + n0, H, 128, lane);
    __builtin_amdgcn_sched_barrier(0);
    fc_opload(a, ar + 128);
    fb_chunk(a, wl, li, q, acc0, acc1);
    __builtin_amdgcn_sched_barrier(0);
    fb_wstore(s1, wl, lane);
    fb_wload(s1, A.wproj + n0, H, 128, lane);
    __builtin_amdgcn_sched_barrier(0);
    fc_opload(a, ar + 256);
    fb_chunk(a, wl, li, q, acc0, acc1);
    __builtin_amdgcn_sched_barrier(0);
    fb_wstore(s0, wl, lane);
    fb_wload(s0, A.wv + n0, H, 128, lane);
    __builtin_amdgcn_sched_barrier(0);
    fc_opload(a, ar + 384);
    fb_chunk(a, wl, li, q, acc0, acc1);
    __builtin_amdgcn_sched_barrier(0);
    fb_wstore(s1, wl, lane);
    __builtin_amdgcn_sched_barrier(0);
    float dx1[4];
    {
        float d[4], xh[4], g[4], gx[4], s1v[4], s2v[4];
#pragma unroll
        for (int i = 0; i < 4; ++i) {
            d[i] = acc0[i] + acc1[i];
            if (A.d_h2) A.d_h2[(size_t)(row0 + 4 * q + i) * H + c] = d[i];
            xh[i] = (x1v[i] - m2v[i]) * r2v[i];
            g[i] = d[i] * g2;
            gx[i] = g[i] * xh[i];
        }
        float* pp = A.part_n2 + (size_t)(wg * 4 + q) * (2 * H);
        pp[c] = (d[0] * xh[0] + d[1] * xh[1]) + (d[2] * xh[2] + d[3] * xh[3]);
        pp[H + c] = (d[0] + d[1]) + (d[2] + d[3]);
        fb_rowsum2<4>(g, gx, redB, wave, li, q, s1v, s2v);
#pragma unroll
        for (int i = 0; i < 4; ++i) {
            dx1[i] = r2v[i] * (g[i] - s1v[i] - xh[i] * s2v[i]) + dx3[i];
            A.d_x1[(size_t)(row0 + 4 * q + i) * H + c] = dx1[i];
            bufV[(4 * q + i) * kFcP1 + c] = dx1[i];
        }
    }
    const FcMaskSrc mx0(A.drop_x0, A.g1n, H);
    float x0v[4], m1v[4], r1v[4];
    uint8_t kb[4];
#pragma unroll
    for (int i = 0; i < 4; ++i) {
        const int r = row0 + 4 * q + i;
        x0v[i] = A.x0[(size_t)r * H + c]; m1v[i] = A.m1[r]; r1v[i] = A.r1[r];
        kb[i] = mx0.raw(r, c);
    }
    const float g1n = A.g1n[c], mr = A.m_rgb[c], md = A.m_dep[c], gd = A.lnd_g[c], bd = A.lnd_b[c];
    float rgbv[2], dpv[2], mdv[2], rdv[2];
#pragma unroll
    for (int j = 0; j < 2; ++j) {
        rgbv[j] = A.rgb[(size_t)(f0 + j) * H + c]; dpv[j] = A.dep_pre[(size_t)(f0 + j) * H + c];
        mdv[j] = A.mean_d[f0 + j]; rdv[j] = A.rstd_d[f0 + j];
    }
    __syncthreads();
    R3D_CHAIN_MARK(A.timeline, wg == 0, 5);
    fc_opload(a, bufV + li * kFcP1 + 4 * q);
    acc0 = zero; acc1 = zero;
    fb_chunk(a, wl, li, q, acc0, acc1);
    __builtin_amdgcn_sched_barrier(0);
    fb_wstore(s0, wl, lane);
    __builtin_amdgcn_sched_barrier(0);
#pragma unroll
    for (int i = 0; i < 4; ++i) {
        const float v = acc0[i] + acc1[i];
        const int rs = 4 * q + (i ^ 1);
        A.d_v[(size_t)(row0 + rs) * H + c] = v;
        bufH[rs * kFcP1 + c] = v;
    }
    __syncthreads();
    R3D_CHAIN_MARK(A.timeline, wg == 0, 6);
    fc_opload(a, bufH + li * kFcP1 + 4 * q);
    acc0 = zero; acc1 = zero;
    fb_chunk(a, wl, li, q, acc0, acc1);
    float gx0[4];
    {
        float d[4], xh[4], g[4], gx[4], s1v[4], s2v[4];
#pragma unroll
        for (int i = 0; i < 4; ++i) {
            d[i] = acc0[i] + acc1[i];
            if (A.d_h1) A.d_h1[(size_t)(row0 + 4 * q + i) * H + c] = d[i];
            xh[i] = (x0v[i] - m1v[i]) * r1v[i];
            g[i] = d[i] * g1n;
            gx[i] = g[i] * xh[i];
        }
#pragma unroll
        for (int j = 0; j < 2; ++j) {
            float* pp = A.part_n1 + (size_t)(f0 + j) * (2 * H);
            pp[c] = d[2 * j] * xh[2 * j] + d[2 * j + 1] * xh[2 * j + 1];
            pp[H + c] = d[2 * j] + d[2 * j + 1];
        }
        fb_rowsum2<4>(g, gx, redA, wave, li, q, s1v, s2v);
#pragma unroll
        for (int i = 0; i < 4; ++i)
            gx0[i] = (r1v[i] * (g[i] - s1v[i] - xh[i] * s2v[i]) + dx1[i] + (A.add_xres ? dx3[i] : 0.f)) *
                     mx0.keep(kb[i], A.drop_scale);
    }
    {
        float g[2], gx[2], xh[2], s1v[2], s2v[2];
#pragma unroll
        for (int j = 0; j < 2; ++j) {
            const float g0 = gx0[2 * j], g1 = gx0[2 * j + 1];
            const float drgb = ((mr != 0.f ? 0.f : g0) + (md != 0.f ? g1 : 0.f)) * (rgbv[j] > 0.f ? 1.f : 0.f);
            A.d_rgb_pre[(size_t)(f0 + j) * H + c] = drgb;
            float dd = (mr != 0.f ? g0 : 0.f) + (md != 0.f ? 0.f : g1);
            xh[j] = (dpv[j] - mdv[j]) * rdv[j];
            if (!(xh[j] * gd + bd > 0.f)) dd = 0.f;
            float* pp = A.part_dep + (size_t)(f0 + j) * (2 * H);
            pp[c] = dd * xh[j];
            pp[H + c] = dd;
            g[j] = dd * gd;
            gx[j] = g[j] * xh[j];
        }
        fb_rowsum2<2>(g, gx, redB, wave, li, q, s1v, s2v);
#pragma unroll
        for (int j = 0; j < 2; ++j)
            A.d_dep_pre[(size_t)(f0 + j) * H + c] = rdv[j] * (g[j] - s1v[j] - xh[j] * s2v[j]);
    }
    R3D_CHAIN_MARK(A.timeline, wg == 0, 7);
}

__device__ __forceinline__ void fc_bwd_query(const FcBwd& A, const int wgq, float* lds) {
    const int tid = threadIdx.x, lane = tid & 63, wave = tid >> 6;
    const int li = lane & 15, q = lane >> 4;
    float* bufH = lds + kFcBufH;
    float* bufV = lds + kFcBufV;
    float* bufF = lds + kFcBufF;
    float* wl = lds + kFbWl + wave * (128 * kFbWP);
    float* redA = lds + kFbRed;
    constexpr int H = kFcH;
    const int row0 = wgq * kFcRows;
    const int c = wave * 16 + li, n0 = wave * 16;
    const f32x4 zero = {0.f, 0.f, 0.f, 0.f};
    FcW s0, s1;
    fb_wload(s0, A.wq + n0, H, 128, lane);
    fb_wload(s1, A.w_out + n0, H, 128, lane);
    const f32x4 a_in = *reinterpret_cast<const f32x4*>(A.d_caq + (size_t)(row0 + (tid >> 5)) * H + 4 * (tid & 31));
    const FcMaskSrc md1(A.drop_d1, A.g1d, H);
    float t2p[4], tpre[4], m1v[4], r1v[4];
    uint8_t kb[4];
#pragma unroll
    for (int i = 0; i < 4; ++i) {
        const int r = row0 + 4 * q + i;
        t2p[i] = A.d_t1_res[(size_t)r * H + c];
        tpre[i] = A.t1_pre[(size_t)r * H + c];
        m1v[i] = A.m1d[r]; r1v[i] = A.r1d[r];
        kb[i] = md1.raw(r, c);
    }
    const float g1 = A.g1d[c];
    __builtin_amdgcn_sched_barrier(0);
    *reinterpret_cast<f32x4*>(bufH + (tid >> 5) * kFcP1 + 4 * (tid & 31)) = a_in;
    fb_wstore(s0, wl, lane);
    fb_wload(s0, A.w_in + n0, H, 128, lane);
    __syncthreads();
    FcOp a;
    f32x4 acc0 = zero, acc1 = zero;
    fc_opload(a, bufH + li * kFcP1 + 4 * q);
    fb_chunk(a, wl, li, q, acc0, acc1);
    __builtin_amdgcn_sched_barrier(0);
    fb_wstore(s1, wl, lane);
    fb_wload(s1, A.w_in + (size_t)128 * H + n0, H, 128, lane);
    __builtin_amdgcn_sched_barrier(0);
    {
        float d[4], xh[4], g[4], gx[4], s1v[4], s2v[4];
#pragma unroll
        for (int i = 0; i < 4; ++i) {
            const float cq = acc0[i] + acc1[i];
            A.caqin[(size_t)(row0 + 4 * q + i) * H + c] = cq;
            d[i] = cq + t2p[i];
            xh[i] = (tpre[i] - m1v[i]) * r1v[i];
            g[i] = d[i] * g1;
            gx[i] = g[i] * xh[i];
        }
        float* pp = A.part_d1 + (size_t)(wgq * 4 + q) * (2 * H);
        pp[c] = (d[0] * xh[0] + d[1] * xh[1]) + (d[2] * xh[2] + d[3] * xh[3]);
        pp[H + c] = (d[0] + d[1]) + (d[2] + d[3]);
        fb_rowsum2<4>(g, gx, redA, wave, li, q, s1v, s2v);
#pragma unroll
        for (int i = 0; i < 4; ++i) {
            const float o = r1v[i] * (g[i] - s1v[i] - xh[i] * s2v[i]);
            const size_t e = (size_t)(row0 + 4 * q + i) * H + c;
            const float ok = o * md1.keep(kb[i], A.drop_scale);
            if (A.t1pre_out) A.t1pre_out[e] = o;
            A.sap[e] = ok;
            bufV[(4 * q + i) * kFcP1 + c] = ok;
        }
    }
    __syncthreads();
    fc_opload(a, bufV + li * kFcP1 + 4 * q);
    acc0 = zero; acc1 = zero;
    fb_chunk(a, wl, li, q, acc0, acc1);
#pragma unroll
    for (int i = 0; i < 4; ++i) A.sao[(size_t)(row0 + 4 * q + i) * H + c] = acc0[i] + acc1[i];
    __syncthreads();
    {
        MhaArgs m{};
        m.q = A.sa_qkv; m.ldq = 3 * H; m.k = A.sa_qkv + H; m.ldk = 3 * H; m.v = A.sa_qkv + 2 * H; m.ldv = 3 * H;
        m.probs = const_cast<float*>(A.p_sa); m.drop = A.drop_sa; m.drop_scale = A.drop_scale; m.d_o = A.sao; m.lddo = H;
        m.dq = A.saqkv; m.lddq = 3 * H; m.dk = A.saqkv + H; m.lddk = 3 * H; m.dv = A.saqkv + 2 * H; m.lddv = 3 * H;
        m.B = A.B; m.heads = 8; m.Lq = 8; m.Lk = 8; m.dh = 16; m.scale = 0.25f;
        mha_bwd_small_unit<16, 8, false>(m, (2 * wgq) * 8 + wave, wl);
        __builtin_amdgcn_wave_barrier();
        mha_bwd_small_unit<16, 8, false>(m, (2 * wgq + 1) * 8 + wave, wl);
    }
    __syncthreads();
    {
        const int r = tid >> 5, c4 = tid & 31;
        const float* src = A.saqkv + (size_t)(row0 + r) * (3 * H) + 4 * c4;
        const f32x4 v0 = *reinterpret_cast<const f32x4*>(src), v1 = *reinterpret_cast<const f32x4*>(src + 128),
                    v2 = *reinterpret_cast<const f32x4*>(src + 256);
        float* dst = bufF + r * kFcP4 + 4 * c4;
        *reinterpret_cast<f32x4*>(dst) = v0;
        *reinterpret_cast<f32x4*>(dst + 128) = v1;
        *reinterpret_cast<f32x4*>(dst + 256) = v2;
    }
    fb_wstore(s0, wl, lane);
    fb_wload(s0, A.w_in + (size_t)256 * H + n0, H, 128, lane);
    __syncthreads();
    const float* ar = bufF + li * kFcP4 + 4 * q;
    acc0 = zero; acc1 = zero;
    fc_opload(a, ar);
    fb_chunk(a, wl, li, q, acc0, acc1);
    __builtin_amdgcn_sched_barrier(0);
    fb_wstore(s1, wl, lane);
    __builtin_amdgcn_sched_barrier(0);
    fc_opload(a, ar + 128);
    fb_chunk(a, wl, li, q, acc0, acc1);
    __builtin_amdgcn_sched_barrier(0);
    fb_wstore(s0, wl, lane);
    __builtin_amdgcn_sched_barrier(0);
    fc_opload(a, ar + 256);
    fb_chunk(a, wl, li, q, acc0, acc1);
#pragma unroll
    for (int i = 0; i < 4; ++i) A.sain[(size_t)(row0 + 4 * q + i) * H + c] = acc0[i] + acc1[i];
}

__device__ __forceinline__ void fc3_bwd_fuser(const FcBwd& A, const int wg, float* lds) {
    const int tid = threadIdx.x, lane = tid & 63, wave = tid >> 6;
    const int li = lane & 15, q = lane >> 4;
    unsigned short* img = reinterpret_cast<unsigned short*>(lds);
    unsigned short* imgH = img + kF3ImgH;
    unsigned short* imgV = img + kF3ImgV;
    unsigned short* imgF = img + kF3ImgF;
    float* redA = reinterpret_cast<float*>(reinterpret_cast<unsigned char*>(lds) + kF3RedBytes);
    float* redB = redA + 2 * 8 * kFcRows;
    constexpr int H = kFcH;
    const int row0 = wg * kFcRows;
    const int c = wave * 16 + li;
    const int f0 = (row0 >> 1) + 2 * q;
    const f32x4 zero = {0.f, 0.f, 0.f, 0.f};
    R3D_CHAIN_MARK(A.timeline, wg == 0, 0);
    Bf3B b0, b1, b2;
    bf3_bload<4>(b0, A.pl_wkv_t, 8, wave, 0, lane);
    bf3_bload<4>(b1, A.pl_wkv_t, 8, wave, 4, lane);
    bf3_bload<1>(b2, A.pl_wseg_t, 1, wave, 0, lane);
    {
        const int r = tid >> 5, c4 = tid & 31, fr = (row0 >> 1) + (r >> 1);
        const f32x4 v0 = *reinterpret_cast<const f32x4*>(A.d_cakv + (size_t)fr * (2 * H) + 4 * c4);
        const f32x4 v1 = *reinterpret_cast<const f32x4*>(A.d_cakv + (size_t)fr * (2 * H) + 128 + 4 * c4);
        f32x4 v2;
#pragma unroll
        for (int e = 0; e < 4; ++e) {
            const int k = 4 * (c4 & 7) + e;
            const float t = A.d_seg[(size_t)fr * A.K + (k < A.K ? k : A.K - 1)];
            v2[e] = k < A.K ? t : 0.f;
        }
        bf3_store4(imgF, kF3P4, r, 4 * c4, v0);
        bf3_store4(imgF, kF3P4, r, 128 + 4 * c4, v1);
        if (c4 < 8) bf3_store4(imgF, kF3P4, r, 256 + 4 * c4, v2);
    }
    float x3v[4], mfv[4], rfv[4], dex[2];
#pragma unroll
    for (int i = 0; i < 4; ++i) {
        const int r = row0 + 4 * q + i;
        x3v[i] = A.x3[(size_t)r * H + c]; mfv[i] = A.mf[r]; rfv[i] = A.rf[r];
    }
    const float gF = A.gf[c];
    {
        const float* ex = A.d_extra ? A.d_extra : A.gf;
        const int ld = A.d_extra ? H : 0;
        dex[0] = ex[(size_t)f0 * ld + c]; dex[1] = ex[(size_t)(f0 + 1) * ld + c];
        if (!A.d_extra) { dex[0] = 0.f; dex[1] = 0.f; }
    }
    __syncthreads();
    R3D_CHAIN_MARK(A.timeline, wg == 0, 1);
    f32x4 acc0 = zero, acc1 = zero;
    bf3_chunk<4>(imgF, kF3P4, li, q, 0, b0, acc0, acc1);
    __builtin_amdgcn_sched_barrier(0);
    bf3_bload<4>(b0, A.pl_w2_t, 4, 4 * wave + 0, 0, lane);
    __builtin_amdgcn_sched_barrier(0);
    bf3_chunk<4>(imgF, kF3P4, li, q, 4, b1, acc0, acc1);
    __builtin_amdgcn_sched_barrier(0);
    bf3_bload<4>(b1, A.pl_w2_t, 4, 4 * wave + 1, 0, lane);
    __builtin_amdgcn_sched_barrier(0);
    A.d_fused[(size_t)f0 * H + c] = acc0[0] + acc1[0];
    A.d_fused[(size_t)(f0 + 1) * H + c] = acc0[2] + acc1[2];
    bf3_chunk<1>(imgF, kF3P4, li, q, 8, b2, acc0, acc1);
    __builtin_amdgcn_sched_barrier(0);
    bf3_bload<4>(b2, A.pl_w2_t, 4, 4 * wave + 2, 0, lane);
    __builtin_amdgcn_sched_barrier(0);
    R3D_CHAIN_MARK(A.timeline, wg == 0, 2);
    float dx3[4];
    {
        float d[4], xh[4], g[4], gx[4], s1v[4], s2v[4];
#pragma unroll
        for (int i = 0; i < 4; ++i) {
            d[i] = 0.5f * ((acc0[i] + acc1[i]) + dex[i >> 1]);
            xh[i] = (x3v[i] - mfv[i]) * rfv[i];
            g[i] = d[i] * gF;
            gx[i] = g[i] * xh[i];
        }
        float* pp = A.part_nf + (size_t)(wg * 4 + q) * (2 * H);
        pp[c] = (d[0] * xh[0] + d[1] * xh[1]) + (d[2] * xh[2] + d[3] * xh[3]);
        pp[H + c] = (d[0] + d[1]) + (d[2] + d[3]);
        fb_rowsum2<4>(g, gx, redA, wave, li, q, s1v, s2v);
#pragma unroll
        for (int i = 0; i < 4; ++i) {
            dx3[i] = rfv[i] * (g[i] - s1v[i] - xh[i] * s2v[i]);
            A.d_x3[(size_t)(row0 + 4 * q + i) * H + c] = dx3[i];
            bf3_store1(imgH, kF3P1, 4 * q + i, c, dx3[i]);
        }
    }
    float uv[4][4];
#pragma unroll
    for (int t = 0; t < 4; ++t) {
#pragma unroll
        for (int i = 0; i < 4; ++i) uv[t][i] = A.u[(size_t)(row0 + 4 * q + i) * (4 * H) + (4 * wave + t) * 16 + li];
    }
    __syncthreads();
    R3D_CHAIN_MARK(A.timeline, wg == 0, 3);
#pragma unroll
    for (int t = 0; t < 4; ++t) {
        acc0 = zero; acc1 = zero;
        if (t == 0) bf3_chunk<4>(imgH, kF3P1, li, q, 0, b0, acc0, acc1);
        if (t == 1) bf3_chunk<4>(imgH, kF3P1, li, q, 0, b1, acc0, acc1);
        if (t == 2) bf3_chunk<4>(imgH, kF3P1, li, q, 0, b2, acc0, acc1);
        if (t == 3) bf3_chunk<4>(imgH, kF3P1, li, q, 0, b0, acc0, acc1);
        __builtin_amdgcn_sched_barrier(0);
        if (t == 0) bf3_bload<4>(b0, A.pl_w2_t, 4, 4 * wave + 3, 0, lane);
        if (t == 1) bf3_bload<4>(b1, A.pl_w1_t, 16, wave, 0, lane);
        if (t == 2) bf3_bload<4>(b2, A.pl_w1_t, 16, wave, 4, lane);
        if (t == 3) bf3_bload<4>(b0, A.pl_w1_t, 16, wave, 8, lane);
        __builtin_amdgcn_sched_barrier(0);
        const int cu = (4 * wave + t) * 16 + li;
#pragma unroll
        for (int i = 0; i < 4; ++i) {
            const float du = (acc0[i] + acc1[i]) * gelu_grad_f(uv[t][i]);
            A.d_u[(size_t)(row0 + 4 * q + i) * (4 * H) + cu] = du;
            bf3_store1(imgF, kF3P4, 4 * q + i, cu, du);
        }
    }
    float x1v[4], m2v[4], r2v[4];
#pragma unroll
    for (int i = 0; i < 4; ++i) {
        const int r = row0 + 4 * q + i;
        x1v[i] = A.x1[(size_t)r * H + c]; m2v[i] = A.m2[r]; r2v[i] = A.r2[r];
    }
    const float g2 = A.g2[c];
    __syncthreads();
    R3D_CHAIN_MARK(A.timeline, wg == 0, 4);
    acc0 = zero; acc1 = zero;
    bf3_chunk<4>(imgF, kF3P4, li, q, 0, b1, acc0, acc1);
    __builtin_amdgcn_sched_barrier(0);
    bf3_bload<4>(b1, A.pl_w1_t, 16, wave, 12, lane);
    __builtin_amdgcn_sched_barrier(0);
    bf3_chunk<4>(imgF, kF3P4, li, q, 4, b2, acc0, acc1);
    __builtin_amdgcn_sched_barrier(0);
    bf3_bload<4>(b2, A.pl_wproj_t, 4, wave, 0, lane);
    __builtin_amdgcn_sched_barrier(0);
    bf3_chunk<4>(imgF, kF3P4, li, q, 8, b0, acc0, acc1);
    __builtin_amdgcn_sched_barrier(0);
    bf3_bload<4>(b0, A.pl_wv_t, 4, wave, 0, lane);
    __builtin_amdgcn_sched_barrier(0);
    bf3_chunk<4>(imgF, kF3P4, li, q, 12, b1, acc0, acc1);
    __builtin_amdgcn_sched_barrier(0);
    float dx1[4];
    {
        float d[4], xh[4], g[4], gx[4], s1v[4], s2v[4];
#pragma unroll
        for (int i = 0; i < 4; ++i) {
            d[i] = acc0[i] + acc1[i];
            if (A.d_h2) A.d_h2[(size_t)(row0 + 4 * q + i) * H + c] = d[i];
            xh[i] = (x1v[i] - m2v[i]) * r2v[i];
            g[i] = d[i] * g2;
            gx[i] = g[i] * xh[i];
        }
        float* pp = A.part_n2 + (size_t)(wg * 4 + q) * (2 * H);
        pp[c] = (d[0] * xh[0] + d[1] * xh[1]) + (d[2] * xh[2] + d[3] * xh[3]);
        pp[H + c] = (d[0] + d[1]) + (d[2] + d[3]);
        fb_rowsum2<4>(g, gx, redB, wave, li, q, s1v, s2v);
#pragma unroll
        for (int i = 0; i < 4; ++i) {
            dx1[i] = r2v[i] * (g[i] - s1v[i] - xh[i] * s2v[i]) + dx3[i];
            A.d_x1[(size_t)(row0 + 4 * q + i) * H + c] = dx1[i];
            bf3_store1(imgV, kF3P1, 4 * q + i, c, dx1[i]);
        }
    }
    const FcMaskSrc mx0(A.drop_x0, A.g1n, H);
    float x0v[4], m1v[4], r1v[4];
    uint8_t kb[4];
#pragma unroll
    for (int i = 0; i < 4; ++i) {
        const int r = row0 + 4 * q + i;
        x0v[i] = A.x0[(size_t)r * H + c]; m1v[i] = A.m1[r]; r1v[i] = A.r1[r];
        kb[i] = mx0.raw(r, c);
    }
    const float g1n = A.g1n[c], mr = A.m_rgb[c], md = A.m_dep[c], gd = A.lnd_g[c], bd = A.lnd_b[c];
    float rgbv[2], dpv[2], mdv[2], rdv[2];
#pragma unroll
    for (int j = 0; j < 2; ++j) {
        rgbv[j] = A.rgb[(size_t)(f0 + j) * H + c]; dpv[j] = A.dep_pre[(size_t)(f0 + j) * H + c];
        mdv[j] = A.mean_d[f0 + j]; rdv[j] = A.rstd_d[f0 + j];
    }
    __syncthreads();
    R3D_CHAIN_MARK(A.timeline, wg == 0, 5);
    acc0 = zero; acc1 = zero;
    bf3_chunk<4>(imgV, kF3P1, li, q, 0, b2, acc0, acc1);
#pragma unroll
    for (int i = 0; i < 4; ++i) {
        const float v = acc0[i] + acc1[i];
        const int rs = 4 * q + (i ^ 1);
        A.d_v[(size_t)(row0 + rs) * H + c] = v;
        bf3_store1(imgH, kF3P1, rs, c, v);
    }
    __syncthreads();
    R3D_CHAIN_MARK(A.timeline, wg == 0, 6);
    acc0 = zero; acc1 = zero;
    bf3_chunk<4>(imgH, kF3P1, li, q, 0, b0, acc0, acc1);
    float gx0[4];
    {
        float d[4], xh[4], g[4], gx[4], s1v[4], s2v[4];
#pragma unroll
        for (int i = 0; i < 4; ++i) {
            d[i] = acc0[i] + acc1[i];
            if (A.d_h1) A.d_h1[(size_t)(row0 + 4 * q + i) * H + c] = d[i];
            xh[i] = (x0v[i] - m1v[i]) * r1v[i];
            g[i] = d[i] * g1n;
            gx[i] = g[i] * xh[i];
        }
#pragma unroll
        for (int j = 0; j < 2; ++j) {
            float* pp = A.part_n1 + (size_t)(f0 + j) * (2 * H);
            pp[c] = d[2 * j] * xh[2 * j] + d[2 * j + 1] * xh[2 * j + 1];
            pp[H + c] = d[2 * j] + d[2 * j + 1];
        }
        fb_rowsum2<4>(g, gx, redA, wave, li, q, s1v, s2v);
#pragma unroll
        for (int i = 0; i < 4; ++i)
            gx0[i] = (r1v[i] * (g[i] - s1v[i] - xh[i] * s2v[i]) + dx1[i] + (A.add_xres ? dx3[i] : 0.f)) *
                     mx0.keep(kb[i], A.drop_scale);
    }
    {
        float g[2], gx[2], xh[2], s1v[2], s2v[2];
#pragma unroll
        for (int j = 0; j < 2; ++j) {
            const float g0 = gx0[2 * j], g1 = gx0[2 * j + 1];
            const float drgb = ((mr != 0.f ? 0.f : g0) + (md != 0.f ? g1 : 0.f)) * (rgbv[j] > 0.f ? 1.f : 0.f);
            A.d_rgb_pre[(size_t)(f0 + j) * H + c] = drgb;
            float dd = (mr != 0.f ? g0 : 0.f) + (md != 0.f ? 0.f : g1);
            xh[j] = (dpv[j] - mdv[j]) * rdv[j];
            if (!(xh[j] * gd + bd > 0.f)) dd = 0.f;
            float* pp = A.part_dep + (size_t)(f0 + j) * (2 * H);
            pp[c] = dd * xh[j];
            pp[H + c] = dd;
            g[j] = dd * gd;
            gx[j] = g[j] * xh[j];
        }
        fb_rowsum2<2>(g, gx, redB, wave, li, q, s1v, s2v);
#pragma unroll
        for (int j = 0; j < 2; ++j)
            A.d_dep_pre[(size_t)(f0 + j) * H + c] = rdv[j] * (g[j] - s1v[j] - xh[j] * s2v[j]);
    }
    R3D_CHAIN_MARK(A.timeline, wg == 0, 7);
}

__global__ __launch_bounds__(512) void fuser_chain_bwd_bf3_kernel(const FcBwd A) {
    extern __shared__ __attribute__((aligned(16))) float lds[];
    if (threadIdx.x >= 256) __builtin_amdgcn_s_setprio(0); else __builtin_amdgcn_s_setprio(2);
    const int nf = (2 * A.N) / kFcRows;
    if ((int)blockIdx.x < nf) fc3_bwd_fuser(A, (int)blockIdx.x, lds);
    else fc_bwd_query(A, (int)blockIdx.x - nf, lds);
}

__global__ __launch_bounds__(512) void fuser_chain_bwd_kernel(const FcBwd A) {
    extern __shared__ __attribute__((aligned(16))) float lds[];
    if (threadIdx.x >= 256) __builtin_amdgcn_s_setprio(0); else __builtin_amdgcn_s_setprio(2);
    const int nf = (2 * A.N) / kFcRows;
    if ((int)blockIdx.x < nf) fc_bwd_fuser(A, (int)blockIdx.x, lds);
    else fc_bwd_query(A, (int)blockIdx.x - nf, lds);
}

}

R3D_EXPORT int r3d_fuser_chain_supported(int N, int H, int K, int B, int Q, int heads) {
    return (H == r3d::kFcH && N > 0 && (2 * N) % r3d::kFcRows == 0 && K > 0 && K <= 128 && B > 0 && Q == 8 && heads == 8 &&
            (B * Q) % r3d::kFcRows == 0) ? 1 : 0;
}

R3D_EXPORT int r3d_fuser_chain_fwd(const r3d_fuser_chain_fwd_args* a, void* stream) {
    R3D_REQUIRE(a);
    R3D_REQUIRE(r3d_fuser_chain_supported(a->N, a->H, a->K, a->B, a->Q, a->heads));
    R3D_REQUIRE(a->S > 0 && a->N % a->S == 0);
    R3D_REQUIRE(a->x0 && a->h1 && a->wv && a->wproj && a->bproj && a->g2 && a->be2 && a->w1 && a->b1 && a->w2 && a->b2 && a->gf &&
                a->bef && a->pos && a->wkv && a->bkv && a->wseg && a->bseg);
    R3D_REQUIRE(a->vsw && a->x1 && a->h2 && a->m2 && a->r2 && a->u && a->f1 && a->x3 && a->mf && a->rf && a->fused && a->seg &&
                a->cakv);
    R3D_REQUIRE(a->qpos && a->w_in && a->b_in && a->w_out && a->b_out && a->g1 && a->be1 && a->wq && a->bq);
    R3D_REQUIRE(a->sa_qkv && a->p_sa && a->sa_o && a->t1_pre && a->t1 && a->m1 && a->r1 && a->caq);
    const void* al[] = {a->h1, a->wv, a->wproj, a->w1, a->w2, a->wkv, a->wseg, a->qpos, a->w_in, a->w_out, a->wq, a->sa_o,
                        a->sa_qkv};
    for (const void* p : al)
        if (!r3d_aligned16(p)) return R3D_EALIGN;
    hipError_t e = hipFuncSetAttribute((const void*)r3d::fuser_chain_fwd_kernel, hipFuncAttributeMaxDynamicSharedMemorySize,
                                       r3d::kFcLdsBytes);
    if (e != hipSuccess) return (int)e;
    const int grid = (2 * a->N) / r3d::kFcRows + (a->B * a->Q) / r3d::kFcRows;
    if (a->pl_wv) {
        R3D_REQUIRE(a->pl_wproj && a->pl_w1 && a->pl_w2 && a->pl_wkv && a->pl_wseg);
        const int ldsb = r3d::kFcLdsBytes > r3d::kF3LdsBytes ? r3d::kFcLdsBytes : r3d::kF3LdsBytes;
        e = hipFuncSetAttribute((const void*)r3d::fuser_chain_fwd_bf3_kernel, hipFuncAttributeMaxDynamicSharedMemorySize, ldsb);
        if (e != hipSuccess) return (int)e;
        hipLaunchKernelGGL(r3d::fuser_chain_fwd_bf3_kernel, dim3(grid), dim3(512), (size_t)ldsb, (hipStream_t)stream, *a);
        R3D_LAUNCH_CHECK();
        return R3D_OK;
    }
    hipLaunchKernelGGL(r3d::fuser_chain_fwd_kernel, dim3(grid), dim3(512), (size_t)r3d::kFcLdsBytes, (hipStream_t)stream, *a);
    R3D_LAUNCH_CHECK();
    return R3D_OK;
}

R3D_EXPORT int64_t r3d_weight_plane_elems(int N, int K) { return N > 0 && K > 0 ? (int64_t)r3d::bf3_plane_elems(N, K) : 0; }

R3D_EXPORT int r3d_weight_planes(const r3d_plane_job* jobs_device, int njobs, int total_blocks, void* stream) {
    R3D_REQUIRE(jobs_device && njobs > 0 && total_blocks > 0);
    hipLaunchKernelGGL(r3d::weight_planes_kernel, dim3(r3d_cdiv(total_blocks, 4)), dim3(256), 0, (hipStream_t)stream, jobs_device,
                       njobs, total_blocks);
    R3D_LAUNCH_CHECK();
    return R3D_OK;
}

R3D_EXPORT int r3d_fuser_chain_bwd(const r3d_fuser_chain_bwd_args* a, void* stream) {
    R3D_REQUIRE(a);
    R3D_REQUIRE(r3d_fuser_chain_supported(a->N, a->H, a->K, a->B, a->Q, a->heads));
    R3D_REQUIRE(a->d_cakv && a->d_seg && a->wkv && a->wseg && a->x3 && a->mf && a->rf && a->gf && a->w2 && a->u && a->w1 && a->x1 &&
                a->m2 && a->r2 && a->g2 && a->wproj && a->wv && a->x0 && a->m1 && a->r1 && a->g1n && a->m_rgb && a->m_dep &&
                a->rgb && a->dep_pre && a->mean_d && a->rstd_d && a->lnd_g && a->lnd_b);
    R3D_REQUIRE(a->d_fused && a->d_x3 && a->d_u && a->d_x1 && a->d_v && a->d_rgb_pre && a->d_dep_pre && a->part_nf && a->part_n2 &&
                a->part_n1 && a->part_dep);
    R3D_REQUIRE(a->d_caq && a->d_t1_res && a->wq && a->t1_pre && a->m1d && a->r1d && a->g1d && a->w_out && a->sa_qkv && a->p_sa &&
                a->w_in && a->caqin && a->sap && a->sao && a->saqkv && a->sain && a->part_d1);
    const void* al[] = {a->d_cakv, a->wkv, a->wseg, a->w2, a->w1, a->wproj, a->wv, a->d_caq, a->wq, a->w_out, a->w_in, a->saqkv,
                        a->sa_qkv, a->sao};
    for (const void* p : al)
        if (!r3d_aligned16(p)) return R3D_EALIGN;
    hipError_t e = hipFuncSetAttribute((const void*)r3d::fuser_chain_bwd_kernel, hipFuncAttributeMaxDynamicSharedMemorySize,
                                       r3d::kFbLdsBytes);
    if (e != hipSuccess) return (int)e;
    const int grid = (2 * a->N) / r3d::kFcRows + (a->B * a->Q) / r3d::kFcRows;
    if (a->pl_wkv_t) {
        R3D_REQUIRE(a->pl_wseg_t && a->pl_w2_t && a->pl_w1_t && a->pl_wproj_t && a->pl_wv_t && a->K <= 32);
        const int ldsb = r3d::kFbLdsBytes > r3d::kF3LdsBytes ? r3d::kFbLdsBytes : r3d::kF3LdsBytes;
        e = hipFuncSetAttribute((const void*)r3d::fuser_chain_bwd_bf3_kernel, hipFuncAttributeMaxDynamicSharedMemorySize, ldsb);
        if (e != hipSuccess) return (int)e;
        hipLaunchKernelGGL(r3d::fuser_chain_bwd_bf3_kernel, dim3(grid), dim3(512), (size_t)ldsb, (hipStream_t)stream, *a);
        R3D_LAUNCH_CHECK();
        return R3D_OK;
    }
    hipLaunchKernelGGL(r3d::fuser_chain_bwd_kernel, dim3(grid), dim3(512), (size_t)r3d::kFbLdsBytes, (hipStream_t)stream, *a);
    R3D_LAUNCH_CHECK();
    return R3D_OK;
}
```

r3d_amd/csrc/losses_dev.h:

```cpp
#pragma once
#include "common.h"
#include "../../include/r3d_hip.h"

namespace r3d {

struct LossArgs {
    const float* seg; int ld_seg; const float* act; int ld_act; const float* dur; int ld_dur;
    const int64_t* past_label; const int64_t* target; const float* target_dur;
    int B, S, Q, K, pad_idx, exclude_idx; int val_mode;
    const float* dur_den; float grad_scale;
    float* d_seg; int ld_dseg; float* d_act; int ld_dact; float* d_dur; int ld_ddur;
    float* loss_out; int64_t* counts;
    int64_t* tick_a; int64_t* tick_b;
    int Kseg = 0;
};

__device__ __forceinline__ float ce_row(const float* logit, int K, int64_t label, bool valid, int pad_idx,
                                        float gscale, float* dl, int lane, int* argmax_out) {
    float m = -INFINITY;
    int am = 0x7fffffff;
    if (K <= 64) {
        const float x = lane < K ? logit[lane] : -INFINITY;
        m = wave_max(x);
        const unsigned long long hit = __ballot(lane < K && x == m);
        am = hit ? __builtin_ctzll(hit) : 0x7fffffff;
    } else {
        for (int c = lane; c < K; c += 64) {
            const float x = logit[c];
            if (x > m || (x == m && c < am)) { m = x; am = c; }
        }
#pragma unroll
        for (int off = 32; off > 0; off >>= 1) {
            const float om = __shfl_xor(m, off, 64);
            const int oa = __shfl_xor(am, off, 64);
            if (om > m || (om == m && oa < am)) { m = om; am = oa; }
        }
    }
    *argmax_out = am;
    float se = 0.f;
    for (int c = lane; c < K; c += 64) se += expf(logit[c] - m);
    se = wave_sum(se);
    const float lse = m + logf(se);
    float loss = 0.f;
    if (valid) loss = lse - logit[label];
    if (dl) {
        for (int c = lane; c < K; c += 64) {
            float g = 0.f;
            if (valid) g = (expf(logit[c] - lse) - ((int64_t)c == label ? 1.f : 0.f)) * gscale;
            dl[c] = g;
        }
    }
    return loss;
}

__device__ __forceinline__ void losses_unit(const LossArgs& a, float* part, int u, int lane) {
    const int N = a.B * a.S, BQ = a.B * a.Q;
    float out_l = 0.f, out_c = 0.f, out_v = 0.f;
    if (u < N) {
        if (a.seg) {
            const int64_t lab = a.past_label[u];
            const int Ks = a.Kseg > 0 ? a.Kseg : a.K;
            const bool valid = (lab != (int64_t)a.pad_idx) && (lab != (int64_t)a.exclude_idx) && lab >= 0 && lab < Ks;
            int am;
            float l = ce_row(a.seg + (size_t)u * a.ld_seg, Ks, lab, valid, a.pad_idx, a.grad_scale / (float)N,
                             a.d_seg ? a.d_seg + (size_t)u * a.ld_dseg : nullptr, lane, &am);
            if (valid && am == a.pad_idx) l += 2.0f;
            out_l = l; out_v = valid ? 1.f : 0.f; out_c = (valid && (int64_t)am == lab) ? 1.f : 0.f;
        }
    } else if (u < N + BQ) {
        const int r = u - N, b = r / a.Q;
        int last = -1;
        for (int s = lane; s < a.S; s += 64)
            if (a.past_label[(size_t)b * a.S + s] != (int64_t)a.pad_idx) last = s;
#pragma unroll
        for (int off = 32; off > 0; off >>= 1) last = max(last, __shfl_xor(last, off, 64));
        const int64_t ref = (last >= 0) ? a.past_label[(size_t)b * a.S + last] : (int64_t)a.pad_idx;
        const float w = (ref == a.target[(size_t)b * a.Q]) ? 1.0f : 10.0f;
        const int64_t lab = a.target[r];
        const bool valid = (lab != (int64_t)a.pad_idx) && (lab != (int64_t)a.exclude_idx) && lab >= 0 && lab < a.K;
        int am;
        const float l = ce_row(a.act + (size_t)r * a.ld_act, a.K, lab, valid, a.pad_idx, w * a.grad_scale / (float)BQ,
                               a.d_act ? a.d_act + (size_t)r * a.ld_dact : nullptr, lane, &am);
        out_l = l * w; out_v = valid ? 1.f : 0.f; out_c = (valid && (int64_t)am == lab) ? 1.f : 0.f;
    } else {
        const int b = u - N - BQ;
        float mc = 0.f;
        for (int e = lane; e < BQ; e += 64) mc += (a.target_dur[e] != (float)a.pad_idx) ? 1.f : 0.f;
        mc = wave_sum(mc);
        const float dur_den = a.dur_den ? *a.dur_den : mc;
        float ssum = 0.f;
        for (int q = lane; q < a.Q; q += 64) {
            const float td = a.target_dur[(size_t)b * a.Q + q];
            const float mk = (td != (float)a.pad_idx) ? 1.f : 0.f;
            ssum += fabsf(expf(a.dur[((size_t)b * a.Q + q) * a.ld_dur]) * mk);
        }
        ssum = wave_sum(ssum);
        const float den = fmaxf(ssum, 1e-12f);
        float sq = 0.f, gp = 0.f;
        for (int q = lane; q < a.Q; q += 64) {
            const float td = a.target_dur[(size_t)b * a.Q + q];
            const float mk = (td != (float)a.pad_idx) ? 1.f : 0.f;
            const float p = expf(a.dur[((size_t)b * a.Q + q) * a.ld_dur]) * mk / den;
            const float t = a.val_mode ? td : td * mk * mk;
            const float diff = p - t;
            sq += diff * diff;
            gp += (2.f * diff / dur_den) * p;
        }
        sq = wave_sum(sq);
        gp = wave_sum(gp);
        if (a.d_dur) {
            for (int q = lane; q < a.Q; q += 64) {
                const float td = a.target_dur[(size_t)b * a.Q + q];
                const float mk = (td != (float)a.pad_idx) ? 1.f : 0.f;
                const float p = expf(a.dur[((size_t)b * a.Q + q) * a.ld_dur]) * mk / den;
                const float t = a.val_mode ? td : td * mk * mk;
                const float g = 2.f * (p - t) / dur_den;
                const float dd = (ssum >= 1e-12f) ? p * (g - gp) : 0.f;
                a.d_dur[((size_t)b * a.Q + q) * a.ld_ddur] = dd * a.grad_scale;
            }
        }
        out_l = sq; out_v = mc;
    }
    if (lane == 0) {
        __hip_atomic_store(part + 4 * (size_t)u + 0, out_l, __ATOMIC_RELAXED, __HIP_MEMORY_SCOPE_AGENT);
        __hip_atomic_store(part + 4 * (size_t)u + 1, out_c, __ATOMIC_RELAXED, __HIP_MEMORY_SCOPE_AGENT);
        __hip_atomic_store(part + 4 * (size_t)u + 2, out_v, __ATOMIC_RELAXED, __HIP_MEMORY_SCOPE_AGENT);
    }
}

__device__ __forceinline__ void losses_finalize(const LossArgs& a, const float* part) {
    __shared__ double red[4][3][3];
    const int lane = threadIdx.x & 63, wave = threadIdx.x >> 6;
    const int N = a.B * a.S, BQ = a.B * a.Q;
    double acc[3][3] = {{0, 0, 0}, {0, 0, 0}, {0, 0, 0}};
    for (int u = threadIdx.x; u < N + BQ + a.B; u += 256) {
        float4 v;
        v.x = __hip_atomic_load(part + 4 * (size_t)u + 0, __ATOMIC_RELAXED, __HIP_MEMORY_SCOPE_AGENT);
        v.y = __hip_atomic_load(part + 4 * (size_t)u + 1, __ATOMIC_RELAXED, __HIP_MEMORY_SCOPE_AGENT);
        v.z = __hip_atomic_load(part + 4 * (size_t)u + 2, __ATOMIC_RELAXED, __HIP_MEMORY_SCOPE_AGENT);
        const int g = u < N ? 0 : (u < N + BQ ? 1 : 2);
        acc[g][0] += v.x; acc[g][1] += v.y; acc[g][2] += v.z;
    }
#pragma unroll
    for (int g = 0; g < 3; ++g)
#pragma unroll
        for (int k = 0; k < 3; ++k) {
            const double t = wave_sum_d(acc[g][k]);
            if (lane == 0) red[wave][g][k] = t;
        }
    __syncthreads();
    if (threadIdx.x == 0) {
        double t[3][3];
        for (int g = 0; g < 3; ++g)
            for (int k = 0; k < 3; ++k) t[g][k] = (red[0][g][k] + red[1][g][k]) + (red[2][g][k] + red[3][g][k]);
        const double msum = t[2][2] / (double)a.B;
        const double dur_den = a.dur_den ? (double)*a.dur_den : msum;
        const float ls = a.seg ? (float)(t[0][0] / (double)N) : 0.f;
        const float la = (float)(t[1][0] / (double)BQ);
        const float ld = (float)(t[2][0] / dur_den);
        a.loss_out[0] = ls; a.loss_out[1] = la; a.loss_out[2] = ld; a.loss_out[3] = ls + la + ld;
        a.counts[0] = (int64_t)(t[0][1] + 0.5); a.counts[1] = (int64_t)(t[0][2] + 0.5);
        a.counts[2] = (int64_t)(t[1][1] + 0.5); a.counts[3] = (int64_t)(t[1][2] + 0.5);
        if (a.tick_a) *a.tick_a += 1;
        if (a.tick_b) *a.tick_b += 1;
    }
}

constexpr float kLnEpsTL = 1e-5f;

__device__ __forceinline__ void ln2_apply(const float (&x)[2], const float (&g)[2], const float (&b)[2], int H, int lane,
                                          float (&y)[2], float& mean, float& rstd) {
    float s = 0.f;
#pragma unroll
    for (int e = 0; e < 2; ++e) s += (lane + 64 * e < H) ? x[e] : 0.f;
    mean = wave_sum(s) / (float)H;
    float q = 0.f;
#pragma unroll
    for (int e = 0; e < 2; ++e) {
        const float dl = (lane + 64 * e < H) ? x[e] - mean : 0.f;
        q += dl * dl;
    }
    rstd = 1.0f / sqrtf(wave_sum(q) / (float)H + kLnEpsTL);
#pragma unroll
    for (int e = 0; e < 2; ++e) y[e] = (lane + 64 * e < H) ? (x[e] - mean) * rstd * g[e] + b[e] : 0.f;
}

__device__ __forceinline__ void losses_finalize8(const LossArgs& a, const float* part) {
    __shared__ double red8[8][3][3];
    const int lane = threadIdx.x & 63, wave = threadIdx.x >> 6;
    const int N = a.B * a.S, BQ = a.B * a.Q;
    double acc[3][3] = {{0, 0, 0}, {0, 0, 0}, {0, 0, 0}};
    for (int u = threadIdx.x; u < N + BQ + a.B; u += 512) {
        const float vx = __hip_atomic_load(part + 4 * (size_t)u + 0, __ATOMIC_RELAXED, __HIP_MEMORY_SCOPE_AGENT);
        const float vy = __hip_atomic_load(part + 4 * (size_t)u + 1, __ATOMIC_RELAXED, __HIP_MEMORY_SCOPE_AGENT);
        const float vz = __hip_atomic_load(part + 4 * (size_t)u + 2, __ATOMIC_RELAXED, __HIP_MEMORY_SCOPE_AGENT);
        const int g = u < N ? 0 : (u < N + BQ ? 1 : 2);
        acc[g][0] += vx; acc[g][1] += vy; acc[g][2] += vz;
    }
#pragma unroll
    for (int g = 0; g < 3; ++g)
#pragma unroll
        for (int k = 0; k < 3; ++k) {
            const double t = wave_sum_d(acc[g][k]);
            if (lane == 0) red8[wave][g][k] = t;
        }
    __syncthreads();
    if (threadIdx.x == 0) {
        double t[3][3];
        for (int g = 0; g < 3; ++g)
            for (int k = 0; k < 3; ++k)
                t[g][k] = ((red8[0][g][k] + red8[1][g][k]) + (red8[2][g][k] + red8[3][g][k])) +
                          ((red8[4][g][k] + red8[5][g][k]) + (red8[6][g][k] + red8[7][g][k]));
        const double msum = t[2][2] / (double)a.B;
        const double dur_den = a.dur_den ? (double)*a.dur_den : msum;
        const float ls = a.seg ? (float)(t[0][0] / (double)N) : 0.f;
        const float la = (float)(t[1][0] / (double)BQ);
        const float ld = (float)(t[2][0] / dur_den);
        a.loss_out[0] = ls; a.loss_out[1] = la; a.loss_out[2] = ld; a.loss_out[3] = ls + la + ld;
        a.counts[0] = (int64_t)(t[0][1] + 0.5); a.counts[1] = (int64_t)(t[0][2] + 0.5);
        a.counts[2] = (int64_t)(t[1][1] + 0.5); a.counts[3] = (int64_t)(t[1][2] + 0.5);
        if (a.tick_a) *a.tick_a += 1;
        if (a.tick_b) *a.tick_b += 1;
    }
}

constexpr int kTLHeads = 24;

__device__ __forceinline__ void tail_clip_body(const r3d_tail_losses_args& t, const LossArgs& a, float* part, const int b,
                                               float (*lg)[kTLHeads + 8], float (*dl)[kTLHeads + 8], float (*red)[4][128]) {
    const int lane = threadIdx.x & 63, wave = threadIdx.x >> 6;
    const int H = t.H, K = a.K, Q = a.Q, NH = t.n_head, N = a.B * a.S, BQ = a.B * a.Q;
    const int row = b * Q + wave;
    int cc[2];
    float x[2], g3[2], b3[2], gF[2], bF[2];
#pragma unroll
    for (int e = 0; e < 2; ++e) {
        const int c = lane + 64 * e;
        cc[e] = c < H ? c : H - 1;
        x[e] = t.x[(size_t)row * H + cc[e]];
        g3[e] = t.g3[cc[e]]; b3[e] = t.b3[cc[e]]; gF[e] = t.gF[cc[e]]; bF[e] = t.bF[cc[e]];
    }
    float wh[kTLHeads][2];
#pragma unroll
    for (int k = 0; k < kTLHeads; ++k) {
        const int kc = k < NH ? k : NH - 1;
#pragma unroll
        for (int e = 0; e < 2; ++e) wh[k][e] = t.w_head[(size_t)kc * H + cc[e]];
    }
    float keep[2];
#pragma unroll
    for (int e = 0; e < 2; ++e) keep[e] = t.drop ? t.drop_scale * (float)t.drop[(size_t)row * H + cc[e]] : 1.f;
    const bool small = a.S <= 64 && BQ <= 64;
    const int64_t pl_pre = a.past_label[(size_t)b * a.S + (lane < a.S ? lane : 0)];
    const int64_t tgt_first = a.target[(size_t)b * Q];
    const int64_t tgt_row = a.target[row];
    const float td_all = a.target_dur[lane < BQ ? lane : 0];
    const float td_clip = a.target_dur[(size_t)b * Q + (lane < Q ? lane : 0)];
    const float dden_pre = a.dur_den ? *a.dur_den : 0.f;
    float y3[2], yF[2], m3, r3, mF, rF;
    ln2_apply(x, g3, b3, H, lane, y3, m3, r3);
    ln2_apply(y3, gF, bF, H, lane, yF, mF, rF);
    if (lane == 0) { t.m3[row] = m3; t.r3[row] = r3; t.mF[row] = mF; t.rF[row] = rF; }
#pragma unroll
    for (int e = 0; e < 2; ++e)
        if (lane + 64 * e < H) {
            t.t3[(size_t)row * H + lane + 64 * e] = y3[e];
            t.tgtF[(size_t)row * H + lane + 64 * e] = yF[e];
        }
    {
        float p[kTLHeads];
#pragma unroll
        for (int k = 0; k < kTLHeads; ++k) p[k] = yF[0] * wh[k][0] + yF[1] * wh[k][1];
#pragma unroll
        for (int k = 0; k < kTLHeads; ++k) {
            if (k < NH) {
                const float v = wave_sum(p[k]) + t.b_head[k];
                if (lane == 0) { t.out[(size_t)row * t.ld_out + k] = v; lg[wave][k] = v; }
            }
        }
    }
    __syncthreads();
    float out_l, out_c, out_v;
    {
        int last = -1;
        int64_t ref = (int64_t)a.pad_idx;
        if (small) {
            const unsigned long long obs = __ballot(lane < a.S && pl_pre != (int64_t)a.pad_idx);
            last = obs ? 63 - __builtin_clzll(obs) : -1;
            const int lsel = __builtin_amdgcn_readfirstlane(last < 0 ? 0 : last);
            const unsigned rlo = __builtin_amdgcn_readlane((unsigned)(unsigned long long)pl_pre, lsel);
            const unsigned rhi = __builtin_amdgcn_readlane((unsigned)((unsigned long long)pl_pre >> 32), lsel);
            if (last >= 0) ref = (int64_t)(((unsigned long long)rhi << 32) | rlo);
        } else {
            for (int s = lane; s < a.S; s += 64)
                if (a.past_label[(size_t)b * a.S + s] != (int64_t)a.pad_idx) last = s;
#pragma unroll
            for (int off = 32; off > 0; off >>= 1) last = max(last, __shfl_xor(last, off, 64));
            if (last >= 0) ref = a.past_label[(size_t)b * a.S + last];
        }
        const float w = (ref == tgt_first) ? 1.0f : 10.0f;
        const int64_t lab = tgt_row;
        const bool valid = (lab != (int64_t)a.pad_idx) && (lab != (int64_t)a.exclude_idx) && lab >= 0 && lab < K;
        int am;
        const float l = ce_row(&lg[wave][0], K, lab, valid, a.pad_idx, w * a.grad_scale / (float)BQ, &dl[wave][0], lane, &am);
        out_l = l * w; out_v = valid ? 1.f : 0.f; out_c = (valid && (int64_t)am == lab) ? 1.f : 0.f;
        if (lane == 0) {
            __hip_atomic_store(part + 4 * (size_t)(N + row) + 0, out_l, __ATOMIC_RELAXED, __HIP_MEMORY_SCOPE_AGENT);
            __hip_atomic_store(part + 4 * (size_t)(N + row) + 1, out_c, __ATOMIC_RELAXED, __HIP_MEMORY_SCOPE_AGENT);
            __hip_atomic_store(part + 4 * (size_t)(N + row) + 2, out_v, __ATOMIC_RELAXED, __HIP_MEMORY_SCOPE_AGENT);
        }
    }
    {
        float mc = 0.f;
        if (small) mc = (lane < BQ && td_all != (float)a.pad_idx) ? 1.f : 0.f;
        else
            for (int e = lane; e < BQ; e += 64) mc += (a.target_dur[e] != (float)a.pad_idx) ? 1.f : 0.f;
        mc = wave_sum(mc);
        const float dur_den = a.dur_den ? dden_pre : mc;
        const float mkq = (lane < Q && td_clip != (float)a.pad_idx) ? 1.f : 0.f;
        const float eq = lane < Q ? expf(lg[lane < Q ? lane : 0][K]) * mkq : 0.f;
        const float ssum = wave_sum(fabsf(eq));
        const float den = fmaxf(ssum, 1e-12f);
        float sq = 0.f, gp = 0.f;
        if (lane < Q) {
            const float p = eq / den;
            const float tt = td_clip * mkq * mkq;
            const float diff = p - tt;
            sq = diff * diff;
            gp = (2.f * diff / dur_den) * p;
        }
        sq = wave_sum(sq);
        gp = wave_sum(gp);
        const float td_w = __builtin_bit_cast(float, __builtin_amdgcn_readlane(__builtin_bit_cast(unsigned, td_clip),
                                                                               __builtin_amdgcn_readfirstlane(wave)));
        if (lane == 0) {
            const float td = td_w;
            const float mk = (td != (float)a.pad_idx) ? 1.f : 0.f;
            const float p = expf(lg[wave][K]) * mk / den;
            const float g = 2.f * (p - td * mk * mk) / dur_den;
            dl[wave][K] = ((ssum >= 1e-12f) ? p * (g - gp) : 0.f) * a.grad_scale;
            if (wave == 0) {
                const size_t u = (size_t)N + BQ + b;
                __hip_atomic_store(part + 4 * u + 0, sq, __ATOMIC_RELAXED, __HIP_MEMORY_SCOPE_AGENT);
                __hip_atomic_store(part + 4 * u + 1, 0.f, __ATOMIC_RELAXED, __HIP_MEMORY_SCOPE_AGENT);
                __hip_atomic_store(part + 4 * u + 2, mc, __ATOMIC_RELAXED, __HIP_MEMORY_SCOPE_AGENT);
            }
        }
    }
    for (int k = lane; k < NH; k += 64) t.d_out[(size_t)row * t.ld_dout + k] = dl[wave][k];
    float d[2] = {0.f, 0.f};
#pragma unroll
    for (int k = 0; k < kTLHeads; ++k) {
        if (k < NH) {
            const float dk = dl[wave][k];
            d[0] += dk * wh[k][0]; d[1] += dk * wh[k][1];
        }
    }
    float agF[2], abF[2], ag3[2], ab3[2], xh[2], gg[2], s1 = 0.f, s2 = 0.f;
#pragma unroll
    for (int e = 0; e < 2; ++e) {
        const bool in = lane + 64 * e < H;
        xh[e] = in ? (y3[e] - mF) * rF : 0.f;
        const float dd = in ? d[e] : 0.f;
        agF[e] = dd * xh[e]; abF[e] = dd;
        gg[e] = dd * gF[e];
        s1 += gg[e]; s2 += gg[e] * xh[e];
    }
    s1 = wave_sum(s1) / (float)H; s2 = wave_sum(s2) / (float)H;
    float dt[2], u1 = 0.f, u2 = 0.f;
#pragma unroll
    for (int e = 0; e < 2; ++e) dt[e] = rF * (gg[e] - s1 - xh[e] * s2);
#pragma unroll
    for (int e = 0; e < 2; ++e) {
        const bool in = lane + 64 * e < H;
        xh[e] = in ? (x[e] - m3) * r3 : 0.f;
        const float dd = in ? dt[e] : 0.f;
        ag3[e] = dd * xh[e]; ab3[e] = dd;
        gg[e] = dd * g3[e];
        u1 += gg[e]; u2 += gg[e] * xh[e];
    }
    u1 = wave_sum(u1) / (float)H; u2 = wave_sum(u2) / (float)H;
#pragma unroll
    for (int e = 0; e < 2; ++e) {
        const int c = lane + 64 * e;
        if (c < H) {
            const float o = r3 * (gg[e] - u1 - xh[e] * u2);
            t.dx[(size_t)row * H + c] = o;
            t.dx2[(size_t)row * H + c] = o * keep[e];
            red[wave][0][c] = agF[e]; red[wave][1][c] = abF[e]; red[wave][2][c] = ag3[e]; red[wave][3][c] = ab3[e];
        }
    }
    __syncthreads();
    for (int i = threadIdx.x; i < 2 * 4 * H; i += 512) {
        const int half = i / (4 * H), j = i - half * 4 * H, which = j / H, c = j - which * H;
        const int w0 = 4 * half;
        const float s = (red[w0][which][c] + red[w0 + 1][which][c]) + (red[w0 + 2][which][c] + red[w0 + 3][which][c]);
        float* ws = which < 2 ? t.wsF : t.ws3;
        ws[((size_t)(2 * b + half) * 2 + (which & 1)) * H + c] = s;
    }
}

template <int EPL>
__device__ __forceinline__ void lnw_apply(const float (&x)[EPL], const float (&g)[EPL], const float (&b)[EPL], int H, int lane,
                                          float (&y)[EPL], float& mean, float& rstd) {
    float s = 0.f;
#pragma unroll
    for (int e = 0; e < EPL; ++e) s += (lane + 64 * e < H) ? x[e] : 0.f;
    mean = wave_sum(s) / (float)H;
    float q = 0.f;
#pragma unroll
    for (int e = 0; e < EPL; ++e) {
        const float dl = (lane + 64 * e < H) ? x[e] - mean : 0.f;
        q += dl * dl;
    }
    rstd = 1.0f / sqrtf(wave_sum(q) / (float)H + kLnEpsTL);
#pragma unroll
    for (int e = 0; e < EPL; ++e) y[e] = (lane + 64 * e < H) ? (x[e] - mean) * rstd * g[e] + b[e] : 0.f;
}

template <int EPL>
__device__ __forceinline__ void tail_clip_body_wide(const r3d_tail_losses_args& t, const LossArgs& a, float* part, const int b,
                                                    float (*lg)[kTLHeads + 8], float (*dl)[kTLHeads + 8], const float* whs,
                                                    float* red) {
    const int lane = threadIdx.x & 63, wave = threadIdx.x >> 6;
    const int H = t.H, K = a.K, Q = a.Q, NH = t.n_head, N = a.B * a.S, BQ = a.B * a.Q;
    const int row = b * Q + wave;
    int cc[EPL];
    float x[EPL], g3[EPL], b3[EPL], gF[EPL], bF[EPL];
#pragma unroll
    for (int e = 0; e < EPL; ++e) {
        const int c = lane + 64 * e;
        cc[e] = c < H ? c : H - 1;
        x[e] = t.x[(size_t)row * H + cc[e]];
        g3[e] = t.g3[cc[e]]; b3[e] = t.b3[cc[e]]; gF[e] = t.gF[cc[e]]; bF[e] = t.bF[cc[e]];
    }
    float keep[EPL];
#pragma unroll
    for (int e = 0; e < EPL; ++e) keep[e] = t.drop ? t.drop_scale * (float)t.drop[(size_t)row * H + cc[e]] : 1.f;
    const bool small = a.S <= 64 && BQ <= 64;
    const int64_t pl_pre = a.past_label[(size_t)b * a.S + (lane < a.S ? lane : 0)];
    const int64_t tgt_first = a.target[(size_t)b * Q];
    const int64_t tgt_row = a.target[row];
    const float td_all = a.target_dur[lane < BQ ? lane : 0];
    const float td_clip = a.target_dur[(size_t)b * Q + (lane < Q ? lane : 0)];
    const float dden_pre = a.dur_den ? *a.dur_den : 0.f;
    float y3[EPL], yF[EPL], m3, r3, mF, rF;
    lnw_apply<EPL>(x, g3, b3, H, lane, y3, m3, r3);
    lnw_apply<EPL>(y3, gF, bF, H, lane, yF, mF, rF);
    if (lane == 0) { t.m3[row] = m3; t.r3[row] = r3; t.mF[row] = mF; t.rF[row] = rF; }
#pragma unroll
    for (int e = 0; e < EPL; ++e)
        if (lane + 64 * e < H) {
            t.t3[(size_t)row * H + lane + 64 * e] = y3[e];
            t.tgtF[(size_t)row * H + lane + 64 * e] = yF[e];
        }
    {
        float p[kTLHeads];
#pragma unroll
        for (int k = 0; k < kTLHeads; ++k) {
            const int kc = k < NH ? k : NH - 1;
            float s = 0.f;
#pragma unroll
            for (int e = 0; e < EPL; ++e) s += yF[e] * whs[(size_t)kc * H + cc[e]];
            p[k] = s;
        }
#pragma unroll
        for (int k = 0; k < kTLHeads; ++k) {
            if (k < NH) {
                const float v = wave_sum(p[k]) + t.b_head[k];
                if (lane == 0) { t.out[(size_t)row * t.ld_out + k] = v; lg[wave][k] = v; }
            }
        }
    }
    __syncthreads();
    float out_l, out_c, out_v;
    {
        int last = -1;
        int64_t ref = (int64_t)a.pad_idx;
        if (small) {
            const unsigned long long obs = __ballot(lane < a.S && pl_pre != (int64_t)a.pad_idx);
            last = obs ? 63 - __builtin_clzll(obs) : -1;
            const int lsel = __builtin_amdgcn_readfirstlane(last < 0 ? 0 : last);
            const unsigned rlo = __builtin_amdgcn_readlane((unsigned)(unsigned long long)pl_pre, lsel);
            const unsigned rhi = __builtin_amdgcn_readlane((unsigned)((unsigned long long)pl_pre >> 32), lsel);
            if (last >= 0) ref = (int64_t)(((unsigned long long)rhi << 32) | rlo);
        } else {
            for (int s = lane; s < a.S; s += 64)
                if (a.past_label[(size_t)b * a.S + s] != (int64_t)a.pad_idx) last = s;
#pragma unroll
            for (int off = 32; off > 0; off >>= 1) last = max(last, __shfl_xor(last, off, 64));
            if (last >= 0) ref = a.past_label[(size_t)b * a.S + last];
        }
        const float w = (ref == tgt_first) ? 1.0f : 10.0f;
        const int64_t lab = tgt_row;
        const bool valid = (lab != (int64_t)a.pad_idx) && (lab != (int64_t)a.exclude_idx) && lab >= 0 && lab < K;
        int am;
        const float l = ce_row(&lg[wave][0], K, lab, valid, a.pad_idx, w * a.grad_scale / (float)BQ, &dl[wave][0], lane, &am);
        out_l = l * w; out_v = valid ? 1.f : 0.f; out_c = (valid && (int64_t)am == lab) ? 1.f : 0.f;
        if (lane == 0) {
            __hip_atomic_store(part + 4 * (size_t)(N + row) + 0, out_l, __ATOMIC_RELAXED, __HIP_MEMORY_SCOPE_AGENT);
            __hip_atomic_store(part + 4 * (size_t)(N + row) + 1, out_c, __ATOMIC_RELAXED, __HIP_MEMORY_SCOPE_AGENT);
            __hip_atomic_store(part + 4 * (size_t)(N + row) + 2, out_v, __ATOMIC_RELAXED, __HIP_MEMORY_SCOPE_AGENT);
        }
    }
    {
        float mc = 0.f;
        if (small) mc = (lane < BQ && td_all != (float)a.pad_idx) ? 1.f : 0.f;
        else
            for (int e = lane; e < BQ; e += 64) mc += (a.target_dur[e] != (float)a.pad_idx) ? 1.f : 0.f;
        mc = wave_sum(mc);
        const float dur_den = a.dur_den ? dden_pre : mc;
        const float mkq = (lane < Q && td_clip != (float)a.pad_idx) ? 1.f : 0.f;
        const float eq = lane < Q ? expf(lg[lane < Q ? lane : 0][K]) * mkq : 0.f;
        const float ssum = wave_sum(fabsf(eq));
        const float den = fmaxf(ssum, 1e-12f);
        float sq = 0.f, gp = 0.f;
        if (lane < Q) {
            const float p = eq / den;
            const float tt = td_clip * mkq * mkq;
            const float diff = p - tt;
            sq = diff * diff;
            gp = (2.f * diff / dur_den) * p;
        }
        sq = wave_sum(sq);
        gp = wave_sum(gp);
        const float td_w = __builtin_bit_cast(float, __builtin_amdgcn_readlane(__builtin_bit_cast(unsigned, td_clip),
                                                                               __builtin_amdgcn_readfirstlane(wave)));
        if (lane == 0) {
            const float td = td_w;
            const float mk = (td != (float)a.pad_idx) ? 1.f : 0.f;
            const float p = expf(lg[wave][K]) * mk / den;
            const float g = 2.f * (p - td * mk * mk) / dur_den;
            dl[wave][K] = ((ssum >= 1e-12f) ? p * (g - gp) : 0.f) * a.grad_scale;
            if (wave == 0) {
                const size_t u = (size_t)N + BQ + b;
                __hip_atomic_store(part + 4 * u + 0, sq, __ATOMIC_RELAXED, __HIP_MEMORY_SCOPE_AGENT);
                __hip_atomic_store(part + 4 * u + 1, 0.f, __ATOMIC_RELAXED, __HIP_MEMORY_SCOPE_AGENT);
                __hip_atomic_store(part + 4 * u + 2, mc, __ATOMIC_RELAXED, __HIP_MEMORY_SCOPE_AGENT);
            }
        }
    }
    for (int k = lane; k < NH; k += 64) t.d_out[(size_t)row * t.ld_dout + k] = dl[wave][k];
    float d[EPL];
#pragma unroll
    for (int e = 0; e < EPL; ++e) d[e] = 0.f;
#pragma unroll
    for (int k = 0; k < kTLHeads; ++k) {
        if (k < NH) {
            const float dk = dl[wave][k];
#pragma unroll
            for (int e = 0; e < EPL; ++e) d[e] += dk * whs[(size_t)k * H + cc[e]];
        }
    }
    float agF[EPL], abF[EPL], ag3[EPL], ab3[EPL], xh[EPL], gg[EPL], s1 = 0.f, s2 = 0.f;
#pragma unroll
    for (int e = 0; e < EPL; ++e) {
        const bool in = lane + 64 * e < H;
        xh[e] = in ? (y3[e] - mF) * rF : 0.f;
        const float dd = in ? d[e] : 0.f;
        agF[e] = dd * xh[e]; abF[e] = dd;
        gg[e] = dd * gF[e];
        s1 += gg[e]; s2 += gg[e] * xh[e];
    }
    s1 = wave_sum(s1) / (float)H; s2 = wave_sum(s2) / (float)H;
    float dt[EPL], u1 = 0.f, u2 = 0.f;
#pragma unroll
    for (int e = 0; e < EPL; ++e) dt[e] = rF * (gg[e] - s1 - xh[e] * s2);
#pragma unroll
    for (int e = 0; e < EPL; ++e) {
        const bool in = lane + 64 * e < H;
        xh[e] = in ? (x[e] - m3) * r3 : 0.f;
        const float dd = in ? dt[e] : 0.f;
        ag3[e] = dd * xh[e]; ab3[e] = dd;
        gg[e] = dd * g3[e];
        u1 += gg[e]; u2 += gg[e] * xh[e];
    }
    u1 = wave_sum(u1) / (float)H; u2 = wave_sum(u2) / (float)H;
#pragma unroll
    for (int e = 0; e < EPL; ++e) {
        const int c = lane + 64 * e;
        if (c < H) {
            const float o = r3 * (gg[e] - u1 - xh[e] * u2);
            t.dx[(size_t)row * H + c] = o;
            t.dx2[(size_t)row * H + c] = o * keep[e];
            red[(wave * 4 + 0) * H + c] = agF[e]; red[(wave * 4 + 1) * H + c] = abF[e];
            red[(wave * 4 + 2) * H + c] = ag3[e]; red[(wave * 4 + 3) * H + c] = ab3[e];
        }
    }
    __syncthreads();
    for (int i = threadIdx.x; i < 2 * 4 * H; i += 512) {
        const int half = i / (4 * H), j = i - half * 4 * H, which = j / H, c = j - which * H;
        const int w0 = 4 * half;
        const float s = (red[(w0 * 4 + which) * H + c] + red[((w0 + 1) * 4 + which) * H + c]) +
                        (red[((w0 + 2) * 4 + which) * H + c] + red[((w0 + 3) * 4 + which) * H + c]);
        float* ws = which < 2 ? t.wsF : t.ws3;
        ws[((size_t)(2 * b + half) * 2 + (which & 1)) * H + c] = s;
    }
}

__device__ __forceinline__ void tail_losses_finish(const r3d_tail_losses_args& t, const LossArgs& a, float* part,
                                                   unsigned* arrivals, int* is_last) {
    if (t.defer_finalize) {
        if (blockIdx.x == 0 && threadIdx.x == 0) {
            if (a.tick_a) *a.tick_a += 1;
            if (a.tick_b) *a.tick_b += 1;
        }
        return;
    }
    __builtin_amdgcn_s_waitcnt(0);
    __syncthreads();
    if (threadIdx.x == 0)
        *is_last = (__hip_atomic_fetch_add(arrivals, 1u, __ATOMIC_RELAXED, __HIP_MEMORY_SCOPE_AGENT) == gridDim.x - 1) ? 1 : 0;
    __syncthreads();
    if (!*is_last) return;
    losses_finalize8(a, part);
    if (threadIdx.x == 0) *arrivals = 0u;
}

}
```

r3d_amd/csrc/mha_small.h:

```cpp
#pragma once
#include "common.h"

namespace r3d {

struct MhaArgs {
    const float* q; int ldq; const float* k; int ldk; const float* v; int ldv;
    const uint8_t* kpm;
    const int64_t* key_label; int pad_idx;
    float* probs;
    const uint8_t* drop; float drop_scale;
    float* o; int ldo;
    const float* d_o; int lddo;
    float* dq; int lddq; float* dk; int lddk; float* dv; int lddv;
    int B, heads, Lq, Lk, dh; float scale;
};

constexpr int mha_small_lds_floats(int DH, int LQ) { return LQ * DH + LQ * 64 + 64 * (DH + 1); }

template <bool WG> __device__ __forceinline__ void mha_unit_sync() {
    if (WG) __syncthreads();
    else __builtin_amdgcn_wave_barrier();
}

template <int DH, int LQ, bool WG>
__device__ __forceinline__ void mha_fwd_small_unit(const MhaArgs& a, const int unit, float* lds) {
    float* qs = lds;
    float* sc = lds + LQ * DH;
    float* vc = sc + LQ * 64;
    const int b = unit / a.heads, h = unit % a.heads;
    const int lane = threadIdx.x & 63, Lk = a.Lk;
    const int jc = lane < Lk ? lane : Lk - 1;
    const float* qb = a.q + (size_t)b * LQ * a.ldq + h * DH;
    const float4* kr = reinterpret_cast<const float4*>(a.k + ((size_t)b * Lk + jc) * a.ldk + h * DH);
    const float4* vr = reinterpret_cast<const float4*>(a.v + ((size_t)b * Lk + jc) * a.ldv + h * DH);
    const size_t pbase = ((size_t)(b * a.heads + h) * LQ) * Lk;
    float4 k4[DH / 4], v4[DH / 4];
#pragma unroll
    for (int t = 0; t < DH / 4; ++t) { k4[t] = kr[t]; v4[t] = vr[t]; }
    float qv[(LQ * DH + 63) / 64];
#pragma unroll
    for (int t = 0; t < (LQ * DH + 63) / 64; ++t) {
        const int e = lane + 64 * t, ec = e < LQ * DH ? e : LQ * DH - 1;
        qv[t] = qb[(size_t)(ec / DH) * a.ldq + (ec % DH)];
    }
    const bool has_drop = a.drop != nullptr, has_kpm = a.kpm != nullptr, has_lab = a.key_label != nullptr;
    const uint8_t* dp = has_drop ? a.drop + pbase + jc : reinterpret_cast<const uint8_t*>(kr);
    const size_t dst_ = has_drop ? (size_t)Lk : 0;
    uint8_t kraw[LQ];
#pragma unroll
    for (int i = 0; i < LQ; ++i) kraw[i] = dp[(size_t)i * dst_];
    const uint8_t kpm_raw = *(has_kpm ? a.kpm + (size_t)b * Lk + jc : reinterpret_cast<const uint8_t*>(kr));
    const int64_t lab_raw = *(has_lab ? a.key_label + (size_t)b * Lk + jc : reinterpret_cast<const int64_t*>(kr));
#pragma unroll
    for (int t = 0; t < (LQ * DH + 63) / 64; ++t) {
        const int e = lane + 64 * t;
        if (e < LQ * DH) qs[e] = qv[t];
    }
#pragma unroll
    for (int t = 0; t < DH / 4; ++t) {
        vc[lane * (DH + 1) + 4 * t + 0] = v4[t].x; vc[lane * (DH + 1) + 4 * t + 1] = v4[t].y;
        vc[lane * (DH + 1) + 4 * t + 2] = v4[t].z; vc[lane * (DH + 1) + 4 * t + 3] = v4[t].w;
    }
    mha_unit_sync<WG>();
    float keep[LQ];
#pragma unroll
    for (int i = 0; i < LQ; ++i) keep[i] = has_drop ? a.drop_scale * (float)kraw[i] : 1.f;
    const bool masked = lane >= Lk || (has_kpm && kpm_raw != 0) || (has_lab && lab_raw == (int64_t)a.pad_idx);
    float p[LQ];
#pragma unroll
    for (int i = 0; i < LQ; ++i) {
        float s = 0.f;
#pragma unroll
        for (int t = 0; t < DH / 4; ++t) {
            const float4 q4 = *reinterpret_cast<const float4*>(qs + i * DH + 4 * t);
            s += q4.x * k4[t].x + q4.y * k4[t].y + q4.z * k4[t].z + q4.w * k4[t].w;
        }
        s = masked ? -INFINITY : s * a.scale;
        const float m = wave_max(s);
        const float e = expf(s - m);
        const float sum = wave_sum(e);
        p[i] = e / sum;
        if (lane < Lk) a.probs[pbase + (size_t)i * Lk + lane] = p[i];
        sc[i * 64 + lane] = lane < Lk ? p[i] * keep[i] : 0.f;
    }
    mha_unit_sync<WG>();
#pragma unroll
    for (int t = 0; t < (LQ * DH + 63) / 64; ++t) {
        const int e = lane + 64 * t;
        if (e < LQ * DH) {
            const int i = e / DH, d = e % DH;
            float s = 0.f;
            for (int r = 0; r < Lk; ++r) s += sc[i * 64 + r] * vc[r * (DH + 1) + d];
            a.o[((size_t)b * LQ + i) * a.ldo + h * DH + d] = s;
        }
    }
}

constexpr int mha_small_bwd_lds_floats(int DH, int LQ) { return 2 * LQ * DH + LQ * 64 + 64 * (DH + 1); }

template <int DH, int LQ, bool WG>
__device__ __forceinline__ void mha_bwd_small_unit(const MhaArgs& a, const int unit, float* lds) {
    float* qs = lds;
    float* dos = lds + LQ * DH;
    float* ds = dos + LQ * DH;
    float* kc = ds + LQ * 64;
    const int b = unit / a.heads, h = unit % a.heads;
    const int lane = threadIdx.x & 63, Lk = a.Lk;
    const int jc = lane < Lk ? lane : Lk - 1;
    const float* qb = a.q + (size_t)b * LQ * a.ldq + h * DH;
    const float* dob = a.d_o + (size_t)b * LQ * a.lddo + h * DH;
    const float4* kr = reinterpret_cast<const float4*>(a.k + ((size_t)b * Lk + jc) * a.ldk + h * DH);
    const float4* vr = reinterpret_cast<const float4*>(a.v + ((size_t)b * Lk + jc) * a.ldv + h * DH);
    const size_t pbase = ((size_t)(b * a.heads + h) * LQ) * Lk;
    float4 k4[DH / 4], v4[DH / 4];
#pragma unroll
    for (int t = 0; t < DH / 4; ++t) { k4[t] = kr[t]; v4[t] = vr[t]; }
    float qv[(LQ * DH + 63) / 64], dv_[(LQ * DH + 63) / 64];
#pragma unroll
    for (int t = 0; t < (LQ * DH + 63) / 64; ++t) {
        const int e = lane + 64 * t, ec = e < LQ * DH ? e : LQ * DH - 1;
        qv[t] = qb[(size_t)(ec / DH) * a.ldq + (ec % DH)];
        dv_[t] = dob[(size_t)(ec / DH) * a.lddo + (ec % DH)];
    }
    const bool has_drop = a.drop != nullptr;
    const uint8_t* dp = has_drop ? a.drop + pbase + jc : reinterpret_cast<const uint8_t*>(kr);
    const size_t dst_ = has_drop ? (size_t)Lk : 0;
    float P[LQ];
    uint8_t kraw[LQ];
#pragma unroll
    for (int i = 0; i < LQ; ++i) {
        P[i] = a.probs[pbase + (size_t)i * Lk + jc];
        kraw[i] = dp[(size_t)i * dst_];
    }
#pragma unroll
    for (int t = 0; t < (LQ * DH + 63) / 64; ++t) {
        const int e = lane + 64 * t;
        if (e < LQ * DH) { qs[e] = qv[t]; dos[e] = dv_[t]; }
    }
#pragma unroll
    for (int t = 0; t < DH / 4; ++t) {
        kc[lane * (DH + 1) + 4 * t + 0] = k4[t].x; kc[lane * (DH + 1) + 4 * t + 1] = k4[t].y;
        kc[lane * (DH + 1) + 4 * t + 2] = k4[t].z; kc[lane * (DH + 1) + 4 * t + 3] = k4[t].w;
    }
    mha_unit_sync<WG>();
    float keep[LQ];
#pragma unroll
    for (int i = 0; i < LQ; ++i) keep[i] = has_drop ? a.drop_scale * (float)kraw[i] : 1.f;
    float dS[LQ], Pd[LQ];
    const bool live = lane < Lk;
#pragma unroll
    for (int i = 0; i < LQ; ++i) {
        float s = 0.f;
#pragma unroll
        for (int t = 0; t < DH / 4; ++t) {
            const float4 g4 = *reinterpret_cast<const float4*>(dos + i * DH + 4 * t);
            s += g4.x * v4[t].x + g4.y * v4[t].y + g4.z * v4[t].z + g4.w * v4[t].w;
        }
        const float dp = s * keep[i];
        const float pi = live ? P[i] : 0.f;
        const float tsum = wave_sum(pi * dp);
        dS[i] = live ? pi * (dp - tsum) * a.scale : 0.f;
        Pd[i] = pi * keep[i];
        ds[i * 64 + lane] = dS[i];
    }
    mha_unit_sync<WG>();
#pragma unroll
    for (int t = 0; t < (LQ * DH + 63) / 64; ++t) {
        const int e = lane + 64 * t;
        if (e < LQ * DH) {
            const int i = e / DH, d = e % DH;
            float s = 0.f;
            for (int r = 0; r < Lk; ++r) s += ds[i * 64 + r] * kc[r * (DH + 1) + d];
            a.dq[((size_t)b * LQ + i) * a.lddq + h * DH + d] = s;
        }
    }
    if (live) {
        float4* dkr = reinterpret_cast<float4*>(a.dk + ((size_t)b * Lk + lane) * a.lddk + h * DH);
        float4* dvr = reinterpret_cast<float4*>(a.dv + ((size_t)b * Lk + lane) * a.lddv + h * DH);
#pragma unroll
        for (int t = 0; t < DH / 4; ++t) {
            float4 gk = make_float4(0.f, 0.f, 0.f, 0.f), gv = make_float4(0.f, 0.f, 0.f, 0.f);
#pragma unroll
            for (int i = 0; i < LQ; ++i) {
                const float4 q4 = *reinterpret_cast<const float4*>(qs + i * DH + 4 * t);
                const float4 g4 = *reinterpret_cast<const float4*>(dos + i * DH + 4 * t);
                gk.x += dS[i] * q4.x; gk.y += dS[i] * q4.y; gk.z += dS[i] * q4.z; gk.w += dS[i] * q4.w;
                gv.x += Pd[i] * g4.x; gv.y += Pd[i] * g4.y; gv.z += Pd[i] * g4.z; gv.w += Pd[i] * g4.w;
            }
            dkr[t] = gk;
            dvr[t] = gv;
        }
    }
}

}
```

Measured before the change: 44010.

## Chain decoder fwd/tail/bwd through LDS, keep relu/dropout masks in registers

When all three phases run, the fused decoder kernel keeps intermediates on chip. The attention output goes straight into the bf16 image, and t3_pre and the tail gradients are parked in attention scratch. ReLU and dropout bits are packed into registers, so the backward pass no longer reloads ff1, d_t3pre, d_ff2 or d_cao from global memory. Attention loads are split from compute so global loads and tail parameter prefetches are issued earlier and overlap other work. This adds template paths, LDS aliasing and register pressure, and the fallback path is kept for partial phase masks.

```diff
diff --git a/r3d_amd/csrc/decoder_chain.hip b/r3d_amd/csrc/decoder_chain.hip
--- a/r3d_amd/csrc/decoder_chain.hip
+++ b/r3d_amd/csrc/decoder_chain.hip
@@ -299,14 +299,37 @@
     bf3_store4(img, kD3P1, r, 4 * c4, r < 8 ? v : z);
 }
 
-__device__ __forceinline__ void dc3_fwd(const DcArgs& D, const int b, float* lds) {
+constexpr int kD3Par = 0;
+constexpr int kD3ParWh = kD3Par + 4 * kFcH;
+constexpr int kD3ParBh = kD3ParWh + kTLHeads * kFcH;
+constexpr int kD3Xt = kD3ParBh + 32;
+constexpr int kD3Dxt = kD3Xt + 8 * kFcH;
+static_assert(kD3Dxt + 8 * kFcH <= 8 * kD3ScrWave && (kD3Xt % 4) == 0, "parked tiles fit the attention scratch");
+static_assert(8 * kFcH * 4 <= 3 * 16 * kD3P1 * 2, "d ca_o tile fits image B");
+
+struct Dc3Keep {
+    unsigned relu;
+    unsigned kbf[4];
+};
+
+struct Dc3ImgSink {
+    unsigned short* img;
+    __device__ __forceinline__ void operator()(int row, int col, float v) const {
+        asm volatile("" : "+v"(v));
+        bf3_store1(img, kD3P1, row, col, v);
+    }
+};
+
+template <bool CHIP>
+__device__ __forceinline__ void dc3_fwd(const DcArgs& D, const r3d_tail_losses_args& T, const int b, float* lds, Dc3Keep& keep) {
     const int tid = threadIdx.x, lane = tid & 63, wave = tid >> 6;
     const int li = lane & 15, q = lane >> 4;
     unsigned short* img = reinterpret_cast<unsigned short*>(lds);
     unsigned short* imgA = img + kD3ImgA;
     unsigned short* imgB = img + kD3ImgB;
     unsigned short* imgF = img + kD3ImgF;
-    float* scr = reinterpret_cast<float*>(reinterpret_cast<unsigned char*>(lds) + kD3ScrBytes) + wave * kD3ScrWave;
+    float* scr0 = reinterpret_cast<float*>(reinterpret_cast<unsigned char*>(lds) + kD3ScrBytes);
+    float* scr = scr0 + wave * kD3ScrWave;
     float (*red)[8][kFcRows] = reinterpret_cast<float (*)[8][kFcRows]>(reinterpret_cast<unsigned char*>(lds) + kD3RedBytes);
     constexpr int H = kFcH;
     const int row0 = b * 8;
@@ -314,38 +337,74 @@
     const bool live = q < 2;
     const f32x4 zero = {0.f, 0.f, 0.f, 0.f};
     R3D_CHAIN_MARK(D.timeline, b == 0, 0);
+    MhaArgs m{};
+    m.q = D.caq; m.ldq = H; m.k = D.cakv; m.ldk = 2 * H; m.v = D.cakv + H; m.ldv = 2 * H;
+    m.key_label = D.key_label; m.pad_idx = D.pad_idx; m.probs = D.p_ca; m.drop = D.drop_ca; m.drop_scale = D.drop_scale;
+    m.o = D.ca_o; m.ldo = H; m.B = D.B; m.heads = 8; m.Lq = 8; m.Lk = D.S; m.dh = 16; m.scale = 0.25f;
+    MhaFwdRegs<16, 8> mr;
+    mha_fwd_small_load<16, 8>(m, b * 8 + wave, mr);
+    f32x4 pw0 = zero, pw1 = zero;
+    float pln = 0.f, pbh = 0.f;
+    if (CHIP) {
+        pbh = T.b_head[(tid & 31) < T.n_head ? (tid & 31) : T.n_head - 1];
+        const int nw4 = T.n_head * (H / 4);
+        const f32x4* wsrc = reinterpret_cast<const f32x4*>(T.w_head);
+        pw0 = wsrc[tid < nw4 ? tid : nw4 - 1];
+        pw1 = wsrc[tid + 512 < nw4 ? tid + 512 : nw4 - 1];
+        const int wv = __builtin_amdgcn_readfirstlane(wave);
+        const float* lsrc = wv < 2 ? T.g3 : (wv < 4 ? T.b3 : (wv < 6 ? T.gF : T.bF));
+        pln = lsrc[tid & 127];
+    }
+    __builtin_amdgcn_sched_barrier(0);
     Bf3B b0, b1, b2;
     bf3_bload<4>(b0, D.pl_wo, 4, wave, 0, lane);
+    const FcMaskSrc md2(D.drop_d2, D.g2, H), md3(D.drop_d3, D.g2, H), mff(D.drop_ff, D.g2, 4 * H);
+    float t1v[4];
+    uint8_t kb2r[4], kb3r[4], kbfr[4][4];
+#pragma unroll
+    for (int i = 0; i < 4; ++i) {
+        const size_t r = (size_t)(row0 + ((4 * q + i) & 7));
+        t1v[i] = D.t1[r * H + c];
+        kb2r[i] = md2.raw(r, c);
+        kb3r[i] = md3.raw(r, c);
+#pragma unroll
+        for (int t = 0; t < 4; ++t) kbfr[t][i] = mff.raw(r, (4 * wave + t) * 16 + li);
+    }
+    const float b_o = D.bo[c], g2 = D.g2[c], be2 = D.be2[c], b_2 = D.b2[c];
+    float b_1[4];
+#pragma unroll
+    for (int t = 0; t < 4; ++t) b_1[t] = D.b1[(4 * wave + t) * 16 + li];
+    if (CHIP) {
+        for (int i = tid; i < 3 * 8 * (H / 4); i += 512) {
+            const int pl = i / (8 * (H / 4)), r = 8 + (i / (H / 4)) % 8, c4 = i % (H / 4);
+            *reinterpret_cast<uint2*>(imgA + (pl * 16 + r) * kD3P1 + 4 * c4) = make_uint2(0u, 0u);
+        }
+    }
+    R3D_CHAIN_MARK(D.timeline, b == 0, 1);
+    if (CHIP) mha_fwd_small_compute<16, 8, false>(m, b * 8 + wave, scr, mr, Dc3ImgSink{imgA});
+    else mha_fwd_small_compute<16, 8, false>(m, b * 8 + wave, scr, mr);
+    R3D_CHAIN_MARK(D.timeline, b == 0, 2);
     bf3_bload<4>(b1, D.pl_w1, 4, 4 * wave + 0, 0, lane);
     bf3_bload<4>(b2, D.pl_w1, 4, 4 * wave + 1, 0, lane);
-    const FcMaskSrc md2(D.drop_d2, D.g2, H), md3(D.drop_d3, D.g2, H), mff(D.drop_ff, D.g2, 4 * H);
-    float t1v[4];
-    uint8_t kb2[4], kb3[4], kbf[4][4];
-#pragma unroll
-    for (int i = 0; i < 4; ++i) {
-        const size_t r = (size_t)(row0 + ((4 * q + i) & 7));
-        t1v[i] = D.t1[r * H + c];
-        kb2[i] = md2.raw(r, c);
-        kb3[i] = md3.raw(r, c);
-#pragma unroll
-        for (int t = 0; t < 4; ++t) kbf[t][i] = mff.raw(r, (4 * wave + t) * 16 + li);
-    }
-    const float b_o = D.bo[c], g2 = D.g2[c], be2 = D.be2[c], b_2 = D.b2[c];
-    float b_1[4];
-#pragma unroll
-    for (int t = 0; t < 4; ++t) b_1[t] = D.b1[(4 * wave + t) * 16 + li];
-    R3D_CHAIN_MARK(D.timeline, b == 0, 1);
-    {
-        MhaArgs m{};
-        m.q = D.caq; m.ldq = H; m.k = D.cakv; m.ldk = 2 * H; m.v = D.cakv + H; m.ldv = 2 * H;
-        m.key_label = D.key_label; m.pad_idx = D.pad_idx; m.probs = D.p_ca; m.drop = D.drop_ca; m.drop_scale = D.drop_scale;
-        m.o = D.ca_o; m.ldo = H; m.B = D.B; m.heads = 8; m.Lq = 8; m.Lk = D.S; m.dh = 16; m.scale = 0.25f;
-        mha_fwd_small_unit<16, 8, false>(m, b * 8 + wave, scr);
-    }
-    R3D_CHAIN_MARK(D.timeline, b == 0, 2);
-    __syncthreads();
-    dc3_stage_rows(imgA, D.ca_o, row0, tid);
-    __syncthreads();
+    unsigned kb2 = 0u, kb3 = 0u, kbf[4] = {0u, 0u, 0u, 0u};
+#pragma unroll
+    for (int i = 0; i < 4; ++i) {
+        kb2 |= (unsigned)kb2r[i] << (8 * i);
+        kb3 |= (unsigned)kb3r[i] << (8 * i);
+#pragma unroll
+        for (int t = 0; t < 4; ++t) kbf[t] |= (unsigned)kbfr[t][i] << (8 * i);
+    }
+    __syncthreads();
+    if (CHIP) {
+        const int nw4 = T.n_head * (H / 4);
+        if (tid < nw4) *reinterpret_cast<f32x4*>(scr0 + kD3ParWh + 4 * tid) = pw0;
+        if (tid + 512 < nw4) *reinterpret_cast<f32x4*>(scr0 + kD3ParWh + 4 * (tid + 512)) = pw1;
+        if (tid < 32) scr0[kD3ParBh + tid] = pbh;
+        scr0[kD3Par + tid] = pln;
+    } else {
+        dc3_stage_rows(imgA, D.ca_o, row0, tid);
+        __syncthreads();
+    }
     R3D_CHAIN_MARK(D.timeline, b == 0, 3);
     f32x4 acc0 = zero, acc1 = zero;
     bf3_chunk<4>(imgA, kD3P1, li, q, 0, b0, acc0, acc1);
@@ -355,7 +414,7 @@
     float t2p[4], mean[4], rstd[4], t2v[4];
 #pragma unroll
     for (int i = 0; i < 4; ++i) {
-        t2p[i] = ((acc0[i] + acc1[i]) + b_o) * md2.keep(kb2[i], D.drop_scale) + t1v[i];
+        t2p[i] = ((acc0[i] + acc1[i]) + b_o) * md2.keep((uint8_t)(kb2 >> (8 * i)), D.drop_scale) + t1v[i];
         if (live) D.t2_pre[(size_t)(row0 + 4 * q + i) * H + c] = t2p[i];
     }
     fc_layernorm(t2p, red, wave, li, q, mean, rstd);
@@ -371,6 +430,7 @@
     }
     __syncthreads();
     R3D_CHAIN_MARK(D.timeline, b == 0, 4);
+    unsigned relu = 0u;
 #pragma unroll
     for (int t = 0; t < 4; ++t) {
         acc0 = zero; acc1 = zero;
@@ -387,10 +447,17 @@
         const int cu = (4 * wave + t) * 16 + li;
 #pragma unroll
         for (int i = 0; i < 4; ++i) {
-            const float f = fmaxf((acc0[i] + acc1[i]) + b_1[t], 0.f) * mff.keep(kbf[t][i], D.drop_scale);
+            const float f = fmaxf((acc0[i] + acc1[i]) + b_1[t], 0.f) * mff.keep((uint8_t)(kbf[t] >> (8 * i)), D.drop_scale);
             if (live) D.ff1[(size_t)(row0 + 4 * q + i) * (4 * H) + cu] = f;
             bf3_store1(imgF, kD3P4, 4 * q + i, cu, live ? f : 0.f);
-        }
+            if (CHIP) relu |= (f > 0.f ? 1u : 0u) << (4 * t + i);
+        }
+    }
+    if (CHIP) {
+        keep.relu = relu;
+#pragma unroll
+        for (int t = 0; t < 4; ++t)
+            keep.kbf[t] = kbf[t];
     }
     __syncthreads();
     R3D_CHAIN_MARK(D.timeline, b == 0, 5);
@@ -404,19 +471,46 @@
     bf3_chunk<4>(imgF, kD3P4, li, q, 12, b2, acc0, acc1);
     if (live) {
 #pragma unroll
-        for (int i = 0; i < 4; ++i)
-            D.t3_pre[(size_t)(row0 + 4 * q + i) * H + c] =
-                ((acc0[i] + acc1[i]) + b_2) * md3.keep(kb3[i], D.drop_scale) + t2v[i];
-    }
-}
-
-__device__ __forceinline__ void dc3_bwd(const DcArgs& D, const int b, float* lds) {
-    const int tid = threadIdx.x, lane = tid & 63, wave = tid >> 6;
+        for (int i = 0; i < 4; ++i) {
+            const float v = ((acc0[i] + acc1[i]) + b_2) * md3.keep((uint8_t)(kb3 >> (8 * i)), D.drop_scale) + t2v[i];
+            D.t3_pre[(size_t)(row0 + 4 * q + i) * H + c] = v;
+            if (CHIP) scr0[kD3Xt + (4 * q + i) * H + c] = v;
+        }
+    }
+}
+
+struct Dc3TailIo {
+    static constexpr bool kChip = true;
+    float* scr0; unsigned short* imgA; const unsigned short* pl_w2_t; int tid_, wave, lane;
+    Bf3B& w0; Bf3B& w1;
+    __device__ __forceinline__ int tid() const { return tid_; }
+    __device__ __forceinline__ float x(int row, int c) const { return scr0[kD3Xt + row * kFcH + c]; }
+    __device__ __forceinline__ float ln(int which, int c) const { return scr0[kD3Par + which * kFcH + c]; }
+    __device__ __forceinline__ float wh(int k, int c) const { return scr0[kD3ParWh + k * kFcH + c]; }
+    __device__ __forceinline__ float bh(int k) const { return scr0[kD3ParBh + k]; }
+    __device__ __forceinline__ void grads(int row, int c, float dx, float dx2) const {
+        scr0[kD3Dxt + row * kFcH + c] = dx;
+        asm volatile("" : "+v"(dx2));
+        bf3_store1(imgA, kD3P1, row, c, dx2);
+    }
+    __device__ __forceinline__ void loads_requested() const {
+        bf3_bload<4>(w0, pl_w2_t, 4, 4 * wave + 0, 0, lane);
+        bf3_bload<4>(w1, pl_w2_t, 4, 4 * wave + 1, 0, lane);
+    }
+};
+
+template <bool CHIP>
+__device__ __forceinline__ void dc3_bwd(const DcArgs& D, const int b_, float* lds, const Dc3Keep& keep, Bf3B& b0, Bf3B& b1, Bf3B& b2) {
+    int tid = threadIdx.x, b = b_;
+    if (CHIP) { asm volatile("" : "+v"(tid)); asm volatile("" : "+s"(b)); }
+    const int lane = tid & 63, wave = tid >> 6;
     const int li = lane & 15, q = lane >> 4;
     unsigned short* img = reinterpret_cast<unsigned short*>(lds);
     unsigned short* imgA = img + kD3ImgA;
     unsigned short* imgF = img + kD3ImgF;
-    float* scr = reinterpret_cast<float*>(reinterpret_cast<unsigned char*>(lds) + kD3ScrBytes) + wave * kD3ScrWave;
+    float* dct = reinterpret_cast<float*>(img + kD3ImgB);
+    float* scr0 = reinterpret_cast<float*>(reinterpret_cast<unsigned char*>(lds) + kD3ScrBytes);
+    float* scr = scr0 + wave * kD3ScrWave;
     float* redA = reinterpret_cast<float*>(reinterpret_cast<unsigned char*>(lds) + kD3RedBytes);
     constexpr int H = kFcH;
     const int row0 = b * 8;
@@ -424,29 +518,43 @@
     const bool live = q < 2;
     const f32x4 zero = {0.f, 0.f, 0.f, 0.f};
     R3D_CHAIN_MARK(D.timeline, b == 0, 10);
-    Bf3B b0, b1, b2;
-    bf3_bload<4>(b0, D.pl_w2_t, 4, 4 * wave + 0, 0, lane);
-    bf3_bload<4>(b1, D.pl_w2_t, 4, 4 * wave + 1, 0, lane);
-    bf3_bload<4>(b2, D.pl_w2_t, 4, 4 * wave + 2, 0, lane);
-    dc3_stage_rows(imgA, D.d_ff2, row0, tid);
     const FcMaskSrc md2(D.drop_d2, D.g2, H), mff(D.drop_ff, D.g2, 4 * H);
     float ffv[4][4], res[4], t2pv[4], m2v[4], r2v[4];
     uint8_t kb2[4], kbf[4][4];
+    if (!CHIP) {
+        dc3_stage_rows(imgA, D.d_ff2, row0, tid);
+#pragma unroll
+        for (int i = 0; i < 4; ++i) {
+            const size_t r = (size_t)(row0 + ((4 * q + i) & 7));
+#pragma unroll
+            for (int t = 0; t < 4; ++t) {
+                ffv[t][i] = D.ff1[r * (4 * H) + (4 * wave + t) * 16 + li];
+                kbf[t][i] = mff.raw(r, (4 * wave + t) * 16 + li);
+            }
+        }
+        bf3_bload<4>(b0, D.pl_w2_t, 4, 4 * wave + 0, 0, lane);
+        bf3_bload<4>(b1, D.pl_w2_t, 4, 4 * wave + 1, 0, lane);
+        bf3_bload<4>(b2, D.pl_w2_t, 4, 4 * wave + 2, 0, lane);
+    } else {
+        bf3_bload<4>(b2, D.pl_w2_t, 4, 4 * wave + 2, 0, lane);
+#pragma unroll
+        for (int t = 0; t < 4; ++t)
+#pragma unroll
+            for (int i = 0; i < 4; ++i) {
+                ffv[t][i] = ((keep.relu >> (4 * t + i)) & 1u) ? 1.f : 0.f;
+                kbf[t][i] = (uint8_t)(keep.kbf[t] >> (8 * i));
+            }
+    }
 #pragma unroll
     for (int i = 0; i < 4; ++i) {
         const size_t r = (size_t)(row0 + ((4 * q + i) & 7));
-#pragma unroll
-        for (int t = 0; t < 4; ++t) {
-            ffv[t][i] = D.ff1[r * (4 * H) + (4 * wave + t) * 16 + li];
-            kbf[t][i] = mff.raw(r, (4 * wave + t) * 16 + li);
-        }
-        res[i] = D.d_t3pre[r * H + c];
+        if (!CHIP) res[i] = D.d_t3pre[r * H + c];
         t2pv[i] = D.t2_pre[r * H + c];
         m2v[i] = D.m2[r]; r2v[i] = D.r2[r];
         kb2[i] = md2.raw(r, c);
     }
     const float g2 = D.g2[c];
-    __syncthreads();
+    if (!CHIP) __syncthreads();
     R3D_CHAIN_MARK(D.timeline, b == 0, 11);
     f32x4 acc0, acc1;
 #pragma unroll
@@ -483,6 +591,17 @@
     __builtin_amdgcn_sched_barrier(0);
     bf3_chunk<4>(imgF, kD3P4, li, q, 8, b0, acc0, acc1);
     bf3_chunk<4>(imgF, kD3P4, li, q, 12, b1, acc0, acc1);
+    if (CHIP) {
+#pragma unroll
+        for (int i = 0; i < 4; ++i) res[i] = scr0[kD3Dxt + ((4 * q + i) & 7) * H + c];
+    }
+    MhaArgs m{};
+    m.q = D.caq; m.ldq = H; m.k = D.cakv; m.ldk = 2 * H; m.v = D.cakv + H; m.ldv = 2 * H;
+    m.probs = D.p_ca; m.drop = D.drop_ca; m.drop_scale = D.drop_scale; m.d_o = D.d_cao; m.lddo = H;
+    m.dq = D.d_caq; m.lddq = H; m.dk = D.d_cakv; m.lddk = 2 * H; m.dv = D.d_cakv + H; m.lddv = 2 * H;
+    m.B = D.B; m.heads = 8; m.Lq = 8; m.Lk = D.S; m.dh = 16; m.scale = 0.25f;
+    MhaBwdRegs<16, 8> mr;
+    if (CHIP) mha_bwd_small_load<16, 8, true>(m, b * 8 + wave, mr, lane);
     {
         float d[4], xh[4], g[4], gx[4], s1v[4], s2v[4];
 #pragma unroll
@@ -494,7 +613,7 @@
         }
         if (live) {
             float* pp = D.part_d2 + (size_t)(2 * b + q) * (2 * H);
-            pp[c] = (d[0] * xh[0] + d[1] * xh[1]) + (d[2] * xh[2] + d[3] * xh[3]);
+            pp[c] = __builtin_fmaf(d[0], xh[0], d[1] * xh[1]) + __builtin_fmaf(d[2], xh[2], d[3] * xh[3]);
             pp[H + c] = (d[0] + d[1]) + (d[2] + d[3]);
         }
         fb_rowsum2<4>(g, gx, redA, wave, li, q, s1v, s2v);
@@ -513,16 +632,17 @@
     bf3_chunk<4>(imgA, kD3P1, li, q, 0, b2, acc0, acc1);
     if (live) {
 #pragma unroll
-        for (int i = 0; i < 4; ++i) D.d_cao[(size_t)(row0 + 4 * q + i) * H + c] = acc0[i] + acc1[i];
+        for (int i = 0; i < 4; ++i) {
+            const float v = acc0[i] + acc1[i];
+            D.d_cao[(size_t)(row0 + 4 * q + i) * H + c] = v;
+            if (CHIP) dct[(4 * q + i) * H + c] = v;
+        }
     }
     R3D_CHAIN_MARK(D.timeline, b == 0, 14);
     __syncthreads();
-    {
-        MhaArgs m{};
-        m.q = D.caq; m.ldq = H; m.k = D.cakv; m.ldk = 2 * H; m.v = D.cakv + H; m.ldv = 2 * H;
-        m.probs = D.p_ca; m.drop = D.drop_ca; m.drop_scale = D.drop_scale; m.d_o = D.d_cao; m.lddo = H;
-        m.dq = D.d_caq; m.lddq = H; m.dk = D.d_cakv; m.lddk = 2 * H; m.dv = D.d_cakv + H; m.lddv = 2 * H;
-        m.B = D.B; m.heads = 8; m.Lq = 8; m.Lk = D.S; m.dh = 16; m.scale = 0.25f;
+    if (CHIP) {
+        mha_bwd_small_compute<16, 8, false, true>(m, b * 8 + wave, scr, mr, dct, H, lane);
+    } else {
         mha_bwd_small_unit<16, 8, false>(m, b * 8 + wave, scr);
     }
     R3D_CHAIN_MARK(D.timeline, b == 0, 15);
@@ -539,16 +659,32 @@
     const int lane = threadIdx.x & 63, wave = threadIdx.x >> 6;
     if ((int)blockIdx.x < D.B) {
         const int b = (int)blockIdx.x;
-        if (D.phases & 1) dc3_fwd(D, b, lds);
-        R3D_CHAIN_MARK(D.timeline, b == 0, 6);
-        if (D.phases & 2) {
+        Dc3Keep keep{};
+        Bf3B w0, w1, w2;
+        if (D.phases == 7) {
+            dc3_fwd<true>(D, t, b, lds, keep);
+            R3D_CHAIN_MARK(D.timeline, b == 0, 6);
             __syncthreads();
-            tail_clip_body(t, a, part, b, lg, dl, red);
-        }
-        R3D_CHAIN_MARK(D.timeline, b == 0, 7);
-        if (D.phases & 4) {
-            __syncthreads();
-            dc3_bwd(D, b, lds);
+            float* scr0 = reinterpret_cast<float*>(reinterpret_cast<unsigned char*>(lds) + kD3ScrBytes);
+            int tid2 = threadIdx.x;
+            asm volatile("" : "+v"(tid2));
+            tail_clip_body(t, a, part, b, lg, dl, red,
+                           Dc3TailIo{scr0, reinterpret_cast<unsigned short*>(lds) + kD3ImgA, D.pl_w2_t, tid2, tid2 >> 6, tid2 & 63,
+                                     w0, w1});
+            R3D_CHAIN_MARK(D.timeline, b == 0, 7);
+            dc3_bwd<true>(D, b, lds, keep, w0, w1, w2);
+        } else {
+            if (D.phases & 1) dc3_fwd<false>(D, t, b, lds, keep);
+            R3D_CHAIN_MARK(D.timeline, b == 0, 6);
+            if (D.phases & 2) {
+                __syncthreads();
+                tail_clip_body(t, a, part, b, lg, dl, red);
+            }
+            R3D_CHAIN_MARK(D.timeline, b == 0, 7);
+            if (D.phases & 4) {
+                __syncthreads();
+                dc3_bwd<false>(D, b, lds, keep, w0, w1, w2);
+            }
         }
     } else if (D.phases & 2) {
         const int u = ((int)blockIdx.x - D.B) * 8 + wave;
diff --git a/r3d_amd/csrc/fuser_chain.hip b/r3d_amd/csrc/fuser_chain.hip
--- a/r3d_amd/csrc/fuser_chain.hip
+++ b/r3d_amd/csrc/fuser_chain.hip
@@ -383,8 +383,6 @@
     const int f0 = (row0 >> 1) + 2 * q;
     const float pos0 = A.pos[(size_t)(f0 % A.S) * H + c], pos1 = A.pos[(size_t)((f0 + 1) % A.S) * H + c];
     const float bkv0 = A.bkv[wave * 16 + li], bkv1 = A.bkv[(wave + 8) * 16 + li];
-    const int cseg = (has12 ? wave : 0) * 16 + li;
-    const float bsg = A.bseg[cseg < A.K ? cseg : A.K - 1];
     __builtin_amdgcn_sched_barrier(0);
     bf3_stage_tile(imgH, kF3P1, 0, a_in, tid);
     __syncthreads();
@@ -452,6 +450,10 @@
     }
     __syncthreads();
     R3D_CHAIN_MARK(A.timeline, wg == 0, 4);
+    int wseg = wave;
+    asm volatile("" : "+v"(wseg));
+    const int cseg = (wseg < nseg_t ? wseg : 0) * 16 + li;
+    const float bsg = A.bseg[cseg < A.K ? cseg : A.K - 1];
     acc0 = zero; acc1 = zero;
     bf3_chunk<4>(imgF, kF3P4, li, q, 0, b0, acc0, acc1);
     __builtin_amdgcn_sched_barrier(0);
@@ -929,8 +931,8 @@
 }
 
 __device__ __forceinline__ void fc3_bwd_fuser(const FcBwd& A, const int wg, float* lds) {
-    const int tid = threadIdx.x, lane = tid & 63, wave = tid >> 6;
-    const int li = lane & 15, q = lane >> 4;
+    int tid = threadIdx.x, lane = tid & 63, wave = tid >> 6;
+    int li = lane & 15, q = lane >> 4;
     unsigned short* img = reinterpret_cast<unsigned short*>(lds);
     unsigned short* imgH = img + kF3ImgH;
     unsigned short* imgV = img + kF3ImgV;
@@ -939,8 +941,8 @@
     float* redB = redA + 2 * 8 * kFcRows;
     constexpr int H = kFcH;
     const int row0 = wg * kFcRows;
-    const int c = wave * 16 + li;
-    const int f0 = (row0 >> 1) + 2 * q;
+    int c = wave * 16 + li;
+    int f0 = (row0 >> 1) + 2 * q;
     const f32x4 zero = {0.f, 0.f, 0.f, 0.f};
     R3D_CHAIN_MARK(A.timeline, wg == 0, 0);
     Bf3B b0, b1, b2;
@@ -1022,6 +1024,9 @@
     }
     __syncthreads();
     R3D_CHAIN_MARK(A.timeline, wg == 0, 3);
+    asm volatile("" : "+v"(tid));
+    lane = tid & 63; wave = tid >> 6; li = lane & 15; q = lane >> 4;
+    c = wave * 16 + li; f0 = (row0 >> 1) + 2 * q;
 #pragma unroll
     for (int t = 0; t < 4; ++t) {
         acc0 = zero; acc1 = zero;
diff --git a/r3d_amd/csrc/losses_dev.h b/r3d_amd/csrc/losses_dev.h
--- a/r3d_amd/csrc/losses_dev.h
+++ b/r3d_amd/csrc/losses_dev.h
@@ -226,9 +226,22 @@
 
 constexpr int kTLHeads = 24;
 
+struct TailGlobalIo {
+    static constexpr bool kChip = false;
+    __device__ __forceinline__ int tid() const { return threadIdx.x; }
+    __device__ __forceinline__ float x(int, int) const { return 0.f; }
+    __device__ __forceinline__ float ln(int, int) const { return 0.f; }
+    __device__ __forceinline__ float wh(int, int) const { return 0.f; }
+    __device__ __forceinline__ float bh(int) const { return 0.f; }
+    __device__ __forceinline__ void grads(int, int, float, float) const {}
+    __device__ __forceinline__ void loads_requested() const {}
+};
+
+template <class Io = TailGlobalIo>
 __device__ __forceinline__ void tail_clip_body(const r3d_tail_losses_args& t, const LossArgs& a, float* part, const int b,
-                                               float (*lg)[kTLHeads + 8], float (*dl)[kTLHeads + 8], float (*red)[4][128]) {
-    const int lane = threadIdx.x & 63, wave = threadIdx.x >> 6;
+                                               float (*lg)[kTLHeads + 8], float (*dl)[kTLHeads + 8], float (*red)[4][128],
+                                               const Io io = Io()) {
+    const int tid = io.tid(), lane = tid & 63, wave = tid >> 6;
     const int H = t.H, K = a.K, Q = a.Q, NH = t.n_head, N = a.B * a.S, BQ = a.B * a.Q;
     const int row = b * Q + wave;
     int cc[2];
@@ -237,26 +250,44 @@
     for (int e = 0; e < 2; ++e) {
         const int c = lane + 64 * e;
         cc[e] = c < H ? c : H - 1;
-        x[e] = t.x[(size_t)row * H + cc[e]];
-        g3[e] = t.g3[cc[e]]; b3[e] = t.b3[cc[e]]; gF[e] = t.gF[cc[e]]; bF[e] = t.bF[cc[e]];
+        if (Io::kChip) {
+            x[e] = io.x(wave, cc[e]);
+            g3[e] = io.ln(0, cc[e]); b3[e] = io.ln(1, cc[e]); gF[e] = io.ln(2, cc[e]); bF[e] = io.ln(3, cc[e]);
+        } else {
+            x[e] = t.x[(size_t)row * H + cc[e]];
+            g3[e] = t.g3[cc[e]]; b3[e] = t.b3[cc[e]]; gF[e] = t.gF[cc[e]]; bF[e] = t.bF[cc[e]];
+        }
     }
     float wh[kTLHeads][2];
 #pragma unroll
     for (int k = 0; k < kTLHeads; ++k) {
         const int kc = k < NH ? k : NH - 1;
 #pragma unroll
-        for (int e = 0; e < 2; ++e) wh[k][e] = t.w_head[(size_t)kc * H + cc[e]];
+        for (int e = 0; e < 2; ++e) wh[k][e] = Io::kChip ? io.wh(kc, cc[e]) : t.w_head[(size_t)kc * H + cc[e]];
     }
     float keep[2];
-#pragma unroll
-    for (int e = 0; e < 2; ++e) keep[e] = t.drop ? t.drop_scale * (float)t.drop[(size_t)row * H + cc[e]] : 1.f;
+    uint8_t keep_raw[2] = {0, 0};
+    if (Io::kChip) {
+        const uint8_t* dp = t.drop ? t.drop + (size_t)row * H : reinterpret_cast<const uint8_t*>(t.g3);
+#pragma unroll
+        for (int e = 0; e < 2; ++e) keep_raw[e] = dp[cc[e]];
+    } else {
+#pragma unroll
+        for (int e = 0; e < 2; ++e) keep[e] = t.drop ? t.drop_scale * (float)t.drop[(size_t)row * H + cc[e]] : 1.f;
+    }
     const bool small = a.S <= 64 && BQ <= 64;
     const int64_t pl_pre = a.past_label[(size_t)b * a.S + (lane < a.S ? lane : 0)];
     const int64_t tgt_first = a.target[(size_t)b * Q];
     const int64_t tgt_row = a.target[row];
     const float td_all = a.target_dur[lane < BQ ? lane : 0];
     const float td_clip = a.target_dur[(size_t)b * Q + (lane < Q ? lane : 0)];
-    const float dden_pre = a.dur_den ? *a.dur_den : 0.f;
+    const float* ddp = a.dur_den ? a.dur_den : t.g3;
+    const float dden_pre = Io::kChip ? *ddp : (a.dur_den ? *a.dur_den : 0.f);
+    io.loads_requested();
+    if (Io::kChip) {
+#pragma unroll
+        for (int e = 0; e < 2; ++e) keep[e] = t.drop ? t.drop_scale * (float)keep_raw[e] : 1.f;
+    }
     float y3[2], yF[2], m3, r3, mF, rF;
     ln2_apply(x, g3, b3, H, lane, y3, m3, r3);
     ln2_apply(y3, gF, bF, H, lane, yF, mF, rF);
@@ -274,7 +305,7 @@
 #pragma unroll
         for (int k = 0; k < kTLHeads; ++k) {
             if (k < NH) {
-                const float v = wave_sum(p[k]) + t.b_head[k];
+                const float v = wave_sum(p[k]) + (Io::kChip ? io.bh(k) : t.b_head[k]);
                 if (lane == 0) { t.out[(size_t)row * t.ld_out + k] = v; lg[wave][k] = v; }
             }
         }
@@ -387,6 +418,7 @@
             const float o = r3 * (gg[e] - u1 - xh[e] * u2);
             t.dx[(size_t)row * H + c] = o;
             t.dx2[(size_t)row * H + c] = o * keep[e];
+            io.grads(wave, c, o, o * keep[e]);
             red[wave][0][c] = agF[e]; red[wave][1][c] = abF[e]; red[wave][2][c] = ag3[e]; red[wave][3][c] = ab3[e];
         }
     }
diff --git a/r3d_amd/csrc/mha_small.h b/r3d_amd/csrc/mha_small.h
--- a/r3d_amd/csrc/mha_small.h
+++ b/r3d_amd/csrc/mha_small.h
@@ -22,11 +22,18 @@
     else __builtin_amdgcn_wave_barrier();
 }
 
-template <int DH, int LQ, bool WG>
-__device__ __forceinline__ void mha_fwd_small_unit(const MhaArgs& a, const int unit, float* lds) {
-    float* qs = lds;
-    float* sc = lds + LQ * DH;
-    float* vc = sc + LQ * 64;
+template <int DH, int LQ> struct MhaFwdRegs {
+    float4 k4[DH / 4], v4[DH / 4];
+    float qv[(LQ * DH + 63) / 64];
+    uint8_t kraw[LQ];
+    uint8_t kpm_raw;
+    int64_t lab_raw;
+};
+
+struct MhaNoSink { __device__ __forceinline__ void operator()(int, int, float) const {} };
+
+template <int DH, int LQ>
+__device__ __forceinline__ void mha_fwd_small_load(const MhaArgs& a, const int unit, MhaFwdRegs<DH, LQ>& R) {
     const int b = unit / a.heads, h = unit % a.heads;
     const int lane = threadIdx.x & 63, Lk = a.Lk;
     const int jc = lane < Lk ? lane : Lk - 1;
@@ -34,27 +41,41 @@
     const float4* kr = reinterpret_cast<const float4*>(a.k + ((size_t)b * Lk + jc) * a.ldk + h * DH);
     const float4* vr = reinterpret_cast<const float4*>(a.v + ((size_t)b * Lk + jc) * a.ldv + h * DH);
     const size_t pbase = ((size_t)(b * a.heads + h) * LQ) * Lk;
-    float4 k4[DH / 4], v4[DH / 4];
-#pragma unroll
-    for (int t = 0; t < DH / 4; ++t) { k4[t] = kr[t]; v4[t] = vr[t]; }
-    float qv[(LQ * DH + 63) / 64];
+#pragma unroll
+    for (int t = 0; t < DH / 4; ++t) { R.k4[t] = kr[t]; R.v4[t] = vr[t]; }
 #pragma unroll
     for (int t = 0; t < (LQ * DH + 63) / 64; ++t) {
         const int e = lane + 64 * t, ec = e < LQ * DH ? e : LQ * DH - 1;
-        qv[t] = qb[(size_t)(ec / DH) * a.ldq + (ec % DH)];
+        R.qv[t] = qb[(size_t)(ec / DH) * a.ldq + (ec % DH)];
     }
     const bool has_drop = a.drop != nullptr, has_kpm = a.kpm != nullptr, has_lab = a.key_label != nullptr;
     const uint8_t* dp = has_drop ? a.drop + pbase + jc : reinterpret_cast<const uint8_t*>(kr);
     const size_t dst_ = has_drop ? (size_t)Lk : 0;
-    uint8_t kraw[LQ];
-#pragma unroll
-    for (int i = 0; i < LQ; ++i) kraw[i] = dp[(size_t)i * dst_];
-    const uint8_t kpm_raw = *(has_kpm ? a.kpm + (size_t)b * Lk + jc : reinterpret_cast<const uint8_t*>(kr));
-    const int64_t lab_raw = *(has_lab ? a.key_label + (size_t)b * Lk + jc : reinterpret_cast<const int64_t*>(kr));
-#pragma unroll
-    for (int t = 0; t < (LQ * DH + 63) / 64; ++t) {
-        const int e = lane + 64 * t;
-        if (e < LQ * DH) qs[e] = qv[t];
+#pragma unroll
+    for (int i = 0; i < LQ; ++i) R.kraw[i] = dp[(size_t)i * dst_];
+    R.kpm_raw = *(has_kpm ? a.kpm + (size_t)b * Lk + jc : reinterpret_cast<const uint8_t*>(kr));
+    R.lab_raw = *(has_lab ? a.key_label + (size_t)b * Lk + jc : reinterpret_cast<const int64_t*>(kr));
+}
+
+template <int DH, int LQ, bool WG, class Sink = MhaNoSink>
+__device__ __forceinline__ void mha_fwd_small_compute(const MhaArgs& a, const int unit, float* lds, const MhaFwdRegs<DH, LQ>& R,
+                                                      const Sink sink = Sink()) {
+    float* qs = lds;
+    float* sc = lds + LQ * DH;
+    float* vc = sc + LQ * 64;
+    const int b = unit / a.heads, h = unit % a.heads;
+    const int lane = threadIdx.x & 63, Lk = a.Lk;
+    const size_t pbase = ((size_t)(b * a.heads + h) * LQ) * Lk;
+    const bool has_drop = a.drop != nullptr, has_kpm = a.kpm != nullptr, has_lab = a.key_label != nullptr;
+    const float4 (&k4)[DH / 4] = R.k4;
+    const float4 (&v4)[DH / 4] = R.v4;
+    const uint8_t (&kraw)[LQ] = R.kraw;
+    const uint8_t kpm_raw = R.kpm_raw;
+    const int64_t lab_raw = R.lab_raw;
+#pragma unroll
+    for (int t = 0; t < (LQ * DH + 63) / 64; ++t) {
+        const int e = lane + 64 * t;
+        if (e < LQ * DH) qs[e] = R.qv[t];
     }
 #pragma unroll
     for (int t = 0; t < DH / 4; ++t) {
@@ -92,50 +113,77 @@
             float s = 0.f;
             for (int r = 0; r < Lk; ++r) s += sc[i * 64 + r] * vc[r * (DH + 1) + d];
             a.o[((size_t)b * LQ + i) * a.ldo + h * DH + d] = s;
-        }
-    }
+            sink(i, h * DH + d, s);
+        }
+    }
+}
+
+template <int DH, int LQ, bool WG>
+__device__ __forceinline__ void mha_fwd_small_unit(const MhaArgs& a, const int unit, float* lds) {
+    MhaFwdRegs<DH, LQ> R;
+    mha_fwd_small_load<DH, LQ>(a, unit, R);
+    mha_fwd_small_compute<DH, LQ, WG>(a, unit, lds, R);
 }
 
 constexpr int mha_small_bwd_lds_floats(int DH, int LQ) { return 2 * LQ * DH + LQ * 64 + 64 * (DH + 1); }
 
-template <int DH, int LQ, bool WG>
-__device__ __forceinline__ void mha_bwd_small_unit(const MhaArgs& a, const int unit, float* lds) {
+template <int DH, int LQ> struct MhaBwdRegs {
+    float4 k4[DH / 4], v4[DH / 4];
+    float qv[(LQ * DH + 63) / 64], dv_[(LQ * DH + 63) / 64];
+    float P[LQ];
+    uint8_t kraw[LQ];
+};
+
+template <int DH, int LQ, bool DoLds>
+__device__ __forceinline__ void mha_bwd_small_load(const MhaArgs& a, const int unit, MhaBwdRegs<DH, LQ>& R,
+                                                   const int lane = threadIdx.x & 63) {
+    const int b = unit / a.heads, h = unit % a.heads;
+    const int Lk = a.Lk;
+    const int jc = lane < Lk ? lane : Lk - 1;
+    const float* qb = a.q + (size_t)b * LQ * a.ldq + h * DH;
+    const float4* kr = reinterpret_cast<const float4*>(a.k + ((size_t)b * Lk + jc) * a.ldk + h * DH);
+    const float4* vr = reinterpret_cast<const float4*>(a.v + ((size_t)b * Lk + jc) * a.ldv + h * DH);
+    const size_t pbase = ((size_t)(b * a.heads + h) * LQ) * Lk;
+#pragma unroll
+    for (int t = 0; t < DH / 4; ++t) { R.k4[t] = kr[t]; R.v4[t] = vr[t]; }
+#pragma unroll
+    for (int t = 0; t < (LQ * DH + 63) / 64; ++t) {
+        const int e = lane + 64 * t, ec = e < LQ * DH ? e : LQ * DH - 1;
+        R.qv[t] = qb[(size_t)(ec / DH) * a.ldq + (ec % DH)];
+        if (!DoLds) R.dv_[t] = (a.d_o + (size_t)b * LQ * a.lddo + h * DH)[(size_t)(ec / DH) * a.lddo + (ec % DH)];
+    }
+    const bool has_drop = a.drop != nullptr;
+    const uint8_t* dp = has_drop ? a.drop + pbase + jc : reinterpret_cast<const uint8_t*>(kr);
+    const size_t dst_ = has_drop ? (size_t)Lk : 0;
+#pragma unroll
+    for (int i = 0; i < LQ; ++i) {
+        R.P[i] = a.probs[pbase + (size_t)i * Lk + jc];
+        R.kraw[i] = dp[(size_t)i * dst_];
+    }
+}
+
+template <int DH, int LQ, bool WG, bool DoLds>
+__device__ __forceinline__ void mha_bwd_small_compute(const MhaArgs& a, const int unit, float* lds, const MhaBwdRegs<DH, LQ>& R,
+                                                      const float* do_tile = nullptr, const int ld_tile = 0,
+                                                      const int lane = threadIdx.x & 63) {
     float* qs = lds;
     float* dos = lds + LQ * DH;
     float* ds = dos + LQ * DH;
     float* kc = ds + LQ * 64;
     const int b = unit / a.heads, h = unit % a.heads;
-    const int lane = threadIdx.x & 63, Lk = a.Lk;
-    const int jc = lane < Lk ? lane : Lk - 1;
-    const float* qb = a.q + (size_t)b * LQ * a.ldq + h * DH;
-    const float* dob = a.d_o + (size_t)b * LQ * a.lddo + h * DH;
-    const float4* kr = reinterpret_cast<const float4*>(a.k + ((size_t)b * Lk + jc) * a.ldk + h * DH);
-    const float4* vr = reinterpret_cast<const float4*>(a.v + ((size_t)b * Lk + jc) * a.ldv + h * DH);
-    const size_t pbase = ((size_t)(b * a.heads + h) * LQ) * Lk;
-    float4 k4[DH / 4], v4[DH / 4];
-#pragma unroll
-    for (int t = 0; t < DH / 4; ++t) { k4[t] = kr[t]; v4[t] = vr[t]; }
-    float qv[(LQ * DH + 63) / 64], dv_[(LQ * DH + 63) / 64];
-#pragma unroll
-    for (int t = 0; t < (LQ * DH + 63) / 64; ++t) {
-        const int e = lane + 64 * t, ec = e < LQ * DH ? e : LQ * DH - 1;
-        qv[t] = qb[(size_t)(ec / DH) * a.ldq + (ec % DH)];
-        dv_[t] = dob[(size_t)(ec / DH) * a.lddo + (ec % DH)];
-    }
+    const int Lk = a.Lk;
     const bool has_drop = a.drop != nullptr;
-    const uint8_t* dp = has_drop ? a.drop + pbase + jc : reinterpret_cast<const uint8_t*>(kr);
-    const size_t dst_ = has_drop ? (size_t)Lk : 0;
-    float P[LQ];
-    uint8_t kraw[LQ];
-#pragma unroll
-    for (int i = 0; i < LQ; ++i) {
-        P[i] = a.probs[pbase + (size_t)i * Lk + jc];
-        kraw[i] = dp[(size_t)i * dst_];
-    }
-#pragma unroll
-    for (int t = 0; t < (LQ * DH + 63) / 64; ++t) {
-        const int e = lane + 64 * t;
-        if (e < LQ * DH) { qs[e] = qv[t]; dos[e] = dv_[t]; }
+    const float4 (&k4)[DH / 4] = R.k4;
+    const float4 (&v4)[DH / 4] = R.v4;
+    const float (&P)[LQ] = R.P;
+    const uint8_t (&kraw)[LQ] = R.kraw;
+#pragma unroll
+    for (int t = 0; t < (LQ * DH + 63) / 64; ++t) {
+        const int e = lane + 64 * t;
+        if (e < LQ * DH) {
+            qs[e] = R.qv[t];
+            dos[e] = DoLds ? do_tile[(e / DH) * ld_tile + h * DH + (e % DH)] : R.dv_[t];
+        }
     }
 #pragma unroll
     for (int t = 0; t < DH / 4; ++t) {
@@ -193,4 +241,11 @@
     }
 }
 
-}
+template <int DH, int LQ, bool WG>
+__device__ __forceinline__ void mha_bwd_small_unit(const MhaArgs& a, const int unit, float* lds) {
+    MhaBwdRegs<DH, LQ> R;
+    mha_bwd_small_load<DH, LQ, false>(a, unit, R);
+    mha_bwd_small_compute<DH, LQ, WG, false>(a, unit, lds, R);
+}
+
+}
```

Measured after the change: 45830 (median of 6 runs). +4.1%, better.
